# loicland/superpoint_graph

Measured on NVIDIA H100. Metric: spg_train_step_edges_plus_points_per_sec, higher is better.
Workload: dtype f32

## Files before the change

include/spg_b200.h:

```cpp
#ifndef SPG_B200_H_
#define SPG_B200_H_

#include <stdint.h>

#ifdef __cplusplus
extern "C" {
#endif

typedef void* spg_stream_t;

#define SPG_OK 0
#define SPG_E_BADARG (-1)
#define SPG_E_UNSUPPORTED (-2)
#define SPG_E_ALIGN (-3)

#define SPG_F32 0
#define SPG_F64 1

int spg_version(void);
const char* spg_error_string(int code);
int spg_set_pdl(int enabled);
int spg_zero(void* ptr, int64_t bytes, spg_stream_t stream);

int spg_prof_enable(int on);
int spg_prof_reset(void);
int spg_prof_collect(void);
int spg_prof_num_kernels(void);
const char* spg_prof_kernel_name(int kernel_id);
int spg_prof_kernel_stats(int kernel_id, int64_t* launches, double* total_ms);
int64_t spg_prof_total_launches(void);


int spg_ecc_fwd(const void* x, const void* w, const int32_t* tgt_rowptr, const int32_t* idxn,
                const int32_t* idxe, void* out, int64_t n_out, int64_t n_edges, int c_in,
                int c_out, int w_is_matrix, int dtype, spg_stream_t stream);

int spg_ecc_bwd_w(const void* xs, const void* gs, int64_t x_iter_stride, int64_t g_iter_stride,
                  int n_iter, const int32_t* tgt_rowptr, const int32_t* idxn,
                  const int32_t* idxe, const int32_t* edge_tgt, void* grad_w, int64_t n_out,
                  int64_t n_edges, int c_in, int c_out, int w_is_matrix, int accumulate,
                  int dtype, spg_stream_t stream);

int spg_ecc_bwd_x(const void* w, const void* g, const int32_t* tgt_rowptr,
                  const int32_t* src_rowptr, const int32_t* src_perm, const int32_t* edge_tgt,
                  const int32_t* idxe, const void* add0, const void* add1, void* grad_x,
                  int64_t n_in, int64_t n_edges, int c_in, int c_out, int w_is_matrix,
                  int dtype, spg_stream_t stream);


int spg_crf_softmax(const float* x, const float* g, float* out, int64_t n, int C,
                    spg_stream_t stream);

int spg_crf_fwd_step(const float* u, const float* q_prev, const float* w, const int32_t* tgt_rowptr,
                     const int32_t* idxn, float* out, int64_t n, int64_t n_edges, int C,
                     int do_softmax, spg_stream_t stream);

int spg_crf_bwd_step(const float* w, const float* gp, const float* q_prev,
                     const float* du_in, float* du_out, float* gp_out, const int32_t* tgt_rowptr,
                     const int32_t* src_rowptr, const int32_t* src_perm, const int32_t* edge_tgt,
                     int64_t n, int64_t n_edges, int C, spg_stream_t stream);


#define SPG_GRU_LAYERNORM 1
#define SPG_GRU_INGATE 2
#define SPG_GRU_BIAS 4
int spg_gru_fwd(const float* x, const float* h, const float* weight_ih, const float* weight_hh,
                const float* bias_ih, const float* bias_hh, const float* ig_weight,
                const float* ig_bias, float* hy, int64_t n_rows, int hidden, int flags,
                spg_stream_t stream);
int spg_gru_bwd(const float* x, const float* h, const float* grad_hy, const float* weight_ih,
                const float* weight_hh, const float* bias_ih, const float* bias_hh,
                const float* ig_weight, const float* ig_bias, float* d_x, float* d_h,
                float* d_gi, float* d_gh, float* d_q, float* xprime, float* dpre,
                int64_t n_rows, int hidden, int flags, spg_stream_t stream);

int spg_rnn_vv_supported(int64_t n_nodes, int hidden);
int spg_rnn_vv_fwd(float* hs, float* inps, const float* w, const int32_t* tgt_rowptr,
                   const int32_t* idxn, const float* weight_ih, const float* weight_hh,
                   const float* bias_ih, const float* bias_hh, const float* ig_weight,
                   const float* ig_bias, int64_t n_nodes, int hidden, int n_repeats, int flags,
                   void* barrier_ws, spg_stream_t stream);
int spg_rnn_vv_bwd(const float* hs, const float* inps, const float* w, const float* grad_top,
                   const float* grad_cat, const int32_t* tgt_rowptr, const int32_t* src_rowptr,
                   const int32_t* src_perm, const int32_t* edge_tgt, const float* weight_ih,
                   const float* weight_hh, const float* bias_ih, const float* bias_hh,
                   const float* ig_weight, const float* ig_bias, float* grad_inp, float* d_h_ws,
                   float* grad_h0, float* d_gi, float* d_gh, float* d_q, float* xprime,
                   float* dpre, int64_t n_nodes, int hidden, int n_repeats, int flags,
                   void* barrier_ws, spg_stream_t stream);

int spg_lstm_fwd(const float* x, const float* h, const float* c, const float* weight_ih,
                 const float* weight_hh, const float* bias_ih, const float* bias_hh,
                 const float* ig_weight, const float* ig_bias, float* hy, float* cy,
                 int64_t n_rows, int hidden, int flags, spg_stream_t stream);
int spg_lstm_bwd(const float* x, const float* h, const float* c, const float* grad_hy,
                 const float* grad_cy, const float* weight_ih, const float* weight_hh,
                 const float* bias_ih, const float* bias_hh, const float* ig_weight,
                 const float* ig_bias, float* d_x, float* d_h, float* d_c, float* d_gi,
                 float* d_gh, float* d_q, float* xprime, int64_t n_rows, int hidden, int flags,
                 spg_stream_t stream);
int spg_rnn_vv_lstm_fwd(float* hs, float* cs, float* inps, const float* w,
                        const int32_t* tgt_rowptr, const int32_t* idxn, const float* weight_ih,
                        const float* weight_hh, const float* bias_ih, const float* bias_hh,
                        const float* ig_weight, const float* ig_bias, int64_t n_nodes, int hidden,
                        int n_repeats, int flags, void* barrier_ws, spg_stream_t stream);
int spg_rnn_vv_lstm_bwd(const float* hs, const float* cs, const float* inps, const float* w,
                        const float* grad_top, const float* grad_cat, const int32_t* tgt_rowptr,
                        const int32_t* src_rowptr, const int32_t* src_perm,
                        const int32_t* edge_tgt, const float* weight_ih, const float* weight_hh,
                        const float* bias_ih, const float* bias_hh, const float* ig_weight,
                        const float* ig_bias, float* grad_inp, float* d_h_ws, float* d_c_ws,
                        float* grad_h0, float* d_gi, float* d_gh, float* d_q, float* xprime,
                        int64_t n_nodes, int hidden, int n_repeats, int flags, void* barrier_ws,
                        spg_stream_t stream);

int spg_gemm(const float* A, int64_t lda, int a_kmajor, const float* B, int64_t ldb, int b_kmajor,
             const float* bias, float* C, int64_t ldc, int64_t M, int64_t N, int64_t K,
             const float* a_scale, const float* a_shift, int a_relu, const float* b_scale,
             const float* b_shift, int b_relu, int split_k, float* workspace, float* stats_ws,
             spg_stream_t stream);
int64_t spg_gemm_stats_tiles(int64_t M);
int spg_colstats_merge(float* partials, int64_t n_partials, int C, float* mean, float* var,
                       spg_stream_t stream);
int spg_colstats_merge_fold(float* partials, int64_t n_partials, int C, float* mean, float* var,
                            const float* gamma, const float* beta, float eps, float* scale,
                            float* shift, float* running_mean, float* running_var,
                            int64_t* num_batches_tracked, float momentum, int64_t M,
                            spg_stream_t stream);

int64_t spg_tc_weight_image_floats(int N, int K);
int spg_tc_pack_weights(const float* W, int64_t ldw, int transpose, int N, int K, int k_valid,
                        float* image, spg_stream_t stream);
int spg_tc_pack_weights_scaled(const float* W, int64_t ldw, const float* row_scale, int N, int K, int k_valid,
                               float* image, spg_stream_t stream);
int spg_tc_pack_weights_multi(const int64_t* table, int n_jobs, int64_t total, spg_stream_t stream);
int spg_tc_gemm_supported(int64_t M, int N, int K);
int spg_tc_gemm(const float* A, int64_t lda, const float* weight_image, const float* bias, float* C,
                int64_t ldc, int64_t M, int N, int K, const float* a_scale, const float* a_shift,
                int a_relu, spg_stream_t stream);
int spg_tc_gemm_max_partials(void);
int spg_tc_gemm_ex(const float* A, int64_t lda, const float* weight_image, const float* bias, float* C,
                   int64_t ldc, int64_t M, int N, int K,
                   const float* a_scale, const float* a_shift, int a_relu,
                   const float* a2, int64_t lda2, const float* a_mean, const float* a_var,
                   const float* a_s12, float a_eps, float* dy_out, int64_t lddy,
                   int epilogue, float* partials_ws,
                   float* mean_out, float* var_out, const float* gamma, const float* beta, float eps,
                   float* scale_out, float* shift_out, float* running_mean, float* running_var,
                   int64_t* num_batches_tracked, float momentum,
                   const float* e_y, int64_t e_ldy, const float* e_scale, const float* e_shift,
                   const float* e_mean, const float* e_var, float e_eps, int e_relu, float* e_s12,
                   spg_stream_t stream);

int spg_tc_dw_supported(int64_t M, int co, int ci);
int spg_tc_dw_ctas(int64_t M);
int spg_tc_dw(const float* dY, int64_t lddy, const float* P, int64_t ldp, const float* p_scale,
              const float* p_shift, int p_relu, float* dW, float* workspace, int64_t M, int co, int ci,
              spg_stream_t stream);
int spg_splitk_reduce(const float* partials, int split, int64_t M, int64_t N, const float* bias,
                      float* C, int64_t ldc, spg_stream_t stream);

int64_t spg_colstats_chunks(int64_t M);
int spg_bn_fold(const float* mean, const float* var, const float* gamma, const float* beta,
                float eps, float* scale, float* shift, float* running_mean, float* running_var,
                int64_t* num_batches_tracked, float momentum, int64_t M, int C,
                spg_stream_t stream);
int spg_affine_act(const float* Y, int64_t ldy, const float* scale, const float* shift, int relu,
                   float* out, int64_t ldo, int64_t M, int C, float p, const int64_t* drop_slot,
                   spg_stream_t stream);
int spg_colsum(const float* X, int64_t ldx, int64_t M, int C, float* out, float* workspace,
               spg_stream_t stream);
int spg_act_bwd_reduce(const float* G, int64_t ldg, const float* Y, int64_t ldy,
                       const float* scale, const float* shift, const float* mean,
                       const float* var, float eps, int relu, float* s12, float* workspace,
                       int64_t M, int C, float p, const int64_t* drop_slot, spg_stream_t stream);
int spg_act_bwd_apply(const float* G, int64_t ldg, const float* Y, int64_t ldy,
                      const float* scale, const float* shift, const float* mean,
                      const float* var, float eps, int relu, int has_bn, const float* s1,
                      const float* s2, float* dY, int64_t lddy, int64_t M, int C, float p,
                      const int64_t* drop_slot, spg_stream_t stream);

int spg_dropout_rng_next(int64_t* state, int64_t* slot, int64_t key_xor, spg_stream_t stream);
int spg_dropout_mask(const int64_t* slot, float p, int64_t M, int C, uint8_t* mask, spg_stream_t stream);

int spg_cloud_rows(const float* clouds, const float* T, int add_eye, float* rows, int64_t ld,
                   int64_t B, int F, int L, spg_stream_t stream);
int spg_segmax_fwd(const float* Y, int64_t ldy, const float* scale, const float* shift, int relu,
                   float* pooled, int64_t ldp, int32_t* argmax, int64_t B, int L, const int64_t* offsets,
                   int C, spg_stream_t stream);
int spg_segmax_bwd(const float* g_pooled, int64_t ldg, const int32_t* argmax, float* G,
                   int64_t ldG, int64_t B, int L, const int64_t* offsets, const int32_t* row_seg,
                   int64_t rows, int C, spg_stream_t stream);
int spg_segmax_bn_bwd(const float* g_pooled, int64_t ldg, const int32_t* argmax, const float* Y,
                      int64_t ldy, const float* scale, const float* shift, const float* mean,
                      const float* var, float eps, int relu, float* s12, float* dY, int64_t lddy,
                      float* workspace, int64_t B, int L, const int64_t* offsets, const int32_t* row_seg,
                      int64_t rows, int C, spg_stream_t stream);
int64_t spg_group_norm_partials(int64_t B);
int spg_group_norm_fwd(const float* Y, int64_t ldy, const float* gamma, const float* beta, float eps, int relu,
                       float* out, int64_t ldo, float* mean, float* rstd, int64_t B, int L,
                       const int64_t* offsets, int C, int groups, float p, const int64_t* drop_slot,
                       spg_stream_t stream);
int spg_group_norm_bwd(const float* G, int64_t ldg, const float* Y, int64_t ldy, const float* mean,
                       const float* rstd, const float* gamma, const float* beta, int relu, float* dY,
                       int64_t lddy, float* dbg, float* workspace, int64_t B, int L, const int64_t* offsets,
                       int C, int groups, float p, const int64_t* drop_slot, spg_stream_t stream);
int spg_stn_apply_bwd(const float* clouds, const float* dXrows, int64_t ld, float* dT, int64_t B,
                      int F, int L, spg_stream_t stream);
int spg_rows_scatter(const float* src, const int64_t* idx, float* dst, int64_t n_src, int C,
                     spg_stream_t stream);
int spg_rows_gather(const float* src, const int64_t* idx, float* dst, int64_t n_dst, int C,
                    spg_stream_t stream);

int spg_ce_loss(const float* logits, const int64_t* target, const float* class_weight,
                int64_t ignore_index, float* loss_out, float* d_logits, float* workspace,
                int64_t n_rows, int C, spg_stream_t stream);
int spg_clamp_adam(float* param, const float* grad, float* exp_avg, float* exp_avg_sq,
                   int64_t n, float lr, float beta1, float beta2, float eps, float weight_decay,
                   float grad_clip, float grad_scale, int64_t step, spg_stream_t stream);

int spg_clamp_adam_dev(float* param, const float* grad, float* exp_avg, float* exp_avg_sq, int64_t n,
                       float lr, float beta1, float beta2, float eps, float weight_decay,
                       float grad_clip, float grad_scale, int64_t* step_counter,
                       spg_stream_t stream);

int spg_cloud_build(const float* points, int64_t ldp, const int64_t* sp_start,
                    const int32_t* sp_count, const int32_t* sample_idx, const int32_t* columns,
                    int n_attribs, int n_points, int normalize, const double* xform,
                    const float* jitter, float jitter_sigma, float jitter_clip, int64_t seed,
                    float* clouds, float* diameters, int64_t n_clouds, spg_stream_t stream);
int spg_graph_build_workspace(int64_t n_out, int64_t n_in, int64_t n_edges, int64_t* bytes);
int spg_graph_build(const int64_t* idxn, const int64_t* degs, int64_t n_out, int64_t n_in, int64_t n_edges,
                    int32_t* idxn32, int32_t* tgt_rowptr, int32_t* edge_tgt, int32_t* src_rowptr,
                    int32_t* src_perm, int32_t* status, void* workspace, int64_t workspace_bytes,
                    spg_stream_t stream);
int spg_confusion_count(const float* logits, int64_t ld_logits, const int64_t* label_mode,
                        const int64_t* label_vec, int64_t ld_vec, int64_t* confusion,
                        int64_t* counters, int64_t* pred_out, int64_t n_nodes, int n_classes,
                        spg_stream_t stream);
int spg_allreduce_flag_words(int world);
int64_t spg_allreduce_stage_floats(int64_t n);
int spg_allreduce_clamp_adam(const float* grad, float* const* peer_stage, uint32_t* const* peer_flags, int rank,
                             int world, float* param, float* exp_avg, float* exp_avg_sq, int64_t n, float lr,
                             float beta1, float beta2, float eps, float weight_decay, float grad_clip,
                             float grad_scale, int64_t* step_counter, uint32_t* local_state, spg_stream_t stream);
int spg_pointnet_fused_supported(int n_features, int n_points, int n_layers, const int32_t* widths);
int64_t spg_pointnet_fused_image_rows(int n_features, int n_layers, const int32_t* widths);
int spg_pointnet_fused_eval(const float* clouds, int64_t n_clouds, int n_features, int n_points, const float* T,
                            int add_eye, const float* weight_image, const float* bias, int n_layers,
                            const int32_t* widths, float* pooled, int64_t ldp, spg_stream_t stream);
int64_t spg_pointnet_fused_bf16_image_rows(int n_features, int n_layers, const int32_t* widths);
int spg_tc_pack_weights_bf16(const float* W, int64_t ldw, const float* row_scale, int N, int K, int k_valid,
                             void* image, spg_stream_t stream);
int spg_pointnet_fused_eval_bf16(const float* clouds, int64_t n_clouds, int n_features, int n_points, const float* T,
                                 int add_eye, const void* weight_image, const float* bias, int n_layers,
                                 const int32_t* widths, float* pooled, int64_t ldp, spg_stream_t stream);
int spg_rows_to_clouds(const float* rows, int64_t ld, float* clouds, int64_t B, int F, int L,
                       spg_stream_t stream);
int spg_rows_xy_transform(const float* rows_in, const float* T, int add_eye, const int32_t* row_seg,
                          float* rows_out, int64_t P, int64_t ld, spg_stream_t stream);
int spg_rows_xy_transform_bwd(const float* rows_in, int64_t ld, const float* d_rows_out, int64_t ld_d,
                              const int64_t* offsets, float* dT, int64_t B, spg_stream_t stream);
int spg_labels_to_points(const int64_t* labels_red, const int64_t* comp_ptr, const int64_t* point_ids,
                         int64_t n_components, uint8_t* labels_full, int64_t n_ver, spg_stream_t stream);
int spg_nn1_interpolate(const float* xyz_ref, int64_t n_ref, const float* xyz_query, int64_t n_query,
                        const int64_t* labels_ref, int64_t* labels_out, int32_t* nn_index_out,
                        spg_stream_t stream);

int spg_lp_sort_workspace(int64_t n, int64_t* bytes);
int spg_lp_incidence(const int64_t* src, const int64_t* tgt, int64_t n_ver, int64_t n_edges, int32_t* rowptr,
                     int32_t* entry, int32_t* keys_tmp, int32_t* keys_sorted, int32_t* vals_tmp, void* workspace,
                     int64_t workspace_bytes, spg_stream_t stream);
int spg_lp_dist_fwd(const float* emb, int64_t n_ver, int D, const int64_t* src, const int64_t* tgt, int64_t n_edges,
                    int dist_type, float* diff, float* coef, spg_stream_t stream);
int spg_lp_dist_bwd(const float* emb, int64_t n_ver, int D, const int64_t* src, const int64_t* tgt, int64_t n_edges,
                    int dist_type, const float* coef, const float* gdiff, const int32_t* rowptr, const int32_t* entry,
                    float* gemb, spg_stream_t stream);
int64_t spg_lp_loss_partials(void);
int spg_lp_loss_fwd(const float* diff, const float* weights, const uint8_t* is_transition, int64_t n_edges,
                    int intra, int inter, int dist_type, double* partials, float* loss, spg_stream_t stream);
int spg_lp_loss_bwd(const float* diff, const float* weights, const uint8_t* is_transition, int64_t n_edges,
                    int intra, int inter, int dist_type, const float* gloss, float* gdiff, spg_stream_t stream);
int spg_lp_xpart(const int64_t* src, const int64_t* tgt, const uint8_t* is_transition,
                 const int64_t* pred_in_component, int64_t n_ver, int64_t n_edges, double transition_factor,
                 float* weights, int32_t* in_component_x, int32_t* comp_size, int32_t* n_comp, int32_t* parent,
                 int32_t* is_root, int32_t* root_rank, uint64_t* keys_tmp, uint64_t* keys_sorted, int32_t* vals_tmp,
                 int32_t* vals_sorted, void* workspace, int64_t workspace_bytes, spg_stream_t stream);
int spg_lp_seal(const int64_t* src, const int64_t* tgt, const uint8_t* is_transition, const int64_t* pred_in_component,
                const int64_t* objects, int64_t n_ver, int64_t n_edges, int64_t n_comp, double transition_factor,
                float* weights, int32_t* w_per_component, int32_t* size_tmp, int32_t* maxfreq_tmp, uint64_t* keys_tmp,
                uint64_t* keys_sorted, void* workspace, int64_t workspace_bytes, spg_stream_t stream);
int spg_lp_fill_weights(const uint8_t* is_transition, int64_t n_edges, float w_other, float w_transition,
                        float* weights, spg_stream_t stream);
int spg_lp_count(const uint8_t* truth, const uint8_t* pred, int64_t n, int64_t* counts, spg_stream_t stream);
int spg_lp_edge_weight(const float* diff, int64_t n_edges, double threshold, double* edge_weight,
                       spg_stream_t stream);
int spg_lp_relax(uint8_t* relaxed, const int64_t* src, const int64_t* tgt, int64_t n_ver, int64_t n_edges,
                 int tolerance, uint8_t* vertex_mark, int32_t* hit, int32_t* status, spg_stream_t stream);
int spg_lp_perfect_prediction(const int64_t* comp_ptr, const int64_t* point_ids, int64_t n_comp,
                              const int64_t* labels, int64_t ld_labels, int n_classes, int64_t n_ver, int64_t* pred,
                              spg_stream_t stream);

int spg_lp_augment(const float* xyz, const float* rgb, int64_t n_ver, const float* rot, int64_t ref_index,
                   const float* noise_xyz, const float* noise_rgb, int device_noise, int rgb_jitter, float sigma,
                   float clip, int64_t seed, int64_t file_pos, float* xyz_out, float* rgb_out, spg_stream_t stream);
int spg_lp_subgraph_workspace(int64_t n_ver, int64_t n_edges, int64_t* bytes);
int spg_lp_subgraph_select(const uint8_t* mask, const int32_t* objects, int64_t n_ver, const int32_t* src,
                           const int32_t* tgt, int64_t n_edges, int32_t* new_index, int32_t* selected,
                           int32_t* edge_pos, uint32_t* object_max, void* workspace, int64_t workspace_bytes,
                           spg_stream_t stream);
int spg_lp_subgraph_edges(const int32_t* src, const int32_t* tgt, const uint8_t* is_transition, int64_t n_edges,
                          const int32_t* new_index, const int32_t* edge_pos, int64_t vertex_offset, int64_t* src_out,
                          int64_t* tgt_out, uint8_t* is_transition_out, spg_stream_t stream);
int spg_lp_object_offsets(const uint32_t* object_max, const int64_t* counts, int64_t n_files, int64_t* offsets,
                          spg_stream_t stream);
int spg_lp_local_clouds(const float* xyz, const float* rgb, int rgb_scale, const int32_t* local_geometry,
                        int64_t ld_geometry, int k, const int32_t* selected, int64_t n_sel, const float* elevation,
                        const float* xyn, const int32_t* labels, int64_t n_label_cols, const int32_t* objects,
                        const int64_t* object_offset, int use_rgb, int global_flags, float* clouds,
                        float* clouds_global, int64_t ld_global, float* xyz_out, int64_t* labels_out,
                        int64_t* objects_out, spg_stream_t stream);

int spg_knn_max_k(void);
int spg_knn_workspace(int64_t n, int64_t* bytes);
int spg_knn_bounds(const float* xyz, int64_t n, uint32_t* words, spg_stream_t stream);
int spg_knn_grid(const float* xyz, int64_t n, double ox, double oy, double oz, double cell, int64_t dim_x,
                 int64_t dim_y, int64_t dim_z, void* workspace, int64_t workspace_bytes, int32_t* n_cells,
                 spg_stream_t stream);
int spg_knn_query(int64_t n, int k, int k1, double ox, double oy, double oz, double cell, int64_t dim_x,
                  int64_t dim_y, int64_t dim_z, const void* workspace, int64_t workspace_bytes, int64_t* source,
                  int64_t* target, float* distances, int64_t* target2, spg_stream_t stream);
int spg_geof(const float* xyz, int64_t n, const int64_t* target, int k, float* geof, uint32_t* status,
             spg_stream_t stream);

#ifdef __cplusplus
}
#endif
#endif
```

superpoint_graph_b200/csrc/common.cuh:

```cuda
#pragma once
#include <cuda_runtime.h>
#include <stdint.h>

#include "../../include/spg_b200.h"

namespace spg {

enum KernelId {
    K_ECC_VV_FWD = 0,
    K_ECC_MAT_FWD,
    K_ECC_GEN_FWD,
    K_ECC_VV_BWD_W,
    K_ECC_MAT_BWD_W,
    K_ECC_GEN_BWD_W,
    K_ECC_VV_BWD_X,
    K_ECC_MAT_BWD_X,
    K_ECC_GEN_BWD_X,
    K_GRU_FWD,
    K_GRU_BWD,
    K_GEMM,
    K_GEMM_SPLITK_REDUCE,
    K_COLSTATS_FINAL,
    K_BN_FOLD,
    K_AFFINE_ACT,
    K_COLSUM_PARTIAL,
    K_COLSUM_FINAL,
    K_ACT_BWD_REDUCE,
    K_ACT_BWD_REDUCE_FINAL,
    K_ACT_BWD_APPLY,
    K_CLOUD_ROWS,
    K_SEGMAX_FWD,
    K_SEGMAX_BWD,
    K_STN_APPLY_BWD,
    K_ROWS_SCATTER,
    K_ROWS_GATHER,
    K_CE_LOSS,
    K_CE_LOSS_FINAL,
    K_CLAMP_ADAM,
    K_TC_GEMM,
    K_TC_PACK,
    K_TC_DW,
    K_RNN_FWD,
    K_RNN_BWD,
    K_CLOUD_BUILD,
    K_CONFUSION,
    K_TC_MERGE,
    K_POINTNET_FUSED,
    K_GRAPH_BUILD,
    K_DROPOUT_RNG_NEXT,
    K_DROPOUT_FWD,
    K_DROPOUT_MASK,
    K_DROPOUT_BWD_REDUCE,
    K_DROPOUT_BWD_REDUCE_FINAL,
    K_DROPOUT_BWD_APPLY,
    K_CRF_FWD,
    K_CRF_BWD,
    K_CRF_SOFTMAX,
    K_LSTM_FWD,
    K_LSTM_BWD,
    K_RNN_LSTM_FWD,
    K_RNN_LSTM_BWD,
    K_GN_FWD,
    K_GN_BWD,
    K_GN_BWD_FINAL,
    K_LP_INCIDENCE,
    K_LP_DIST_FWD,
    K_LP_DIST_BWD,
    K_LP_LOSS_FWD,
    K_LP_LOSS_BWD,
    K_LP_CC,
    K_LP_XPART,
    K_LP_SEAL,
    K_LP_WEIGHTS,
    K_LP_RELAX,
    K_LP_METRICS,
    K_LP_AUGMENT,
    K_LP_SUBGRAPH,
    K_LP_LOCAL_CLOUDS,
    K_GEO_BOUNDS,
    K_GEO_GRID,
    K_GEO_KNN,
    K_GEO_GEOF,
    K_COUNT
};

struct LaunchScope {
    int kid;
    cudaStream_t stream;
    int slot;
    LaunchScope(int kernel_id, cudaStream_t s);
    ~LaunchScope();
};

inline int launch_status() { return (int)cudaGetLastError(); }

constexpr int kNumSMs = 132;

__host__ __device__ inline int64_t ceil_div64(int64_t a, int64_t b) { return (a + b - 1) / b; }

__device__ __forceinline__ float warp_sum(float v) {
#pragma unroll
    for (int o = 16; o > 0; o >>= 1) v += __shfl_xor_sync(0xffffffffu, v, o);
    return v;
}

__device__ __forceinline__ float4 ld_stream4(const float4* p) { return __ldcs(p); }
__device__ __forceinline__ void st_stream4(float4* p, float4 v) { __stcs(p, v); }

__device__ __forceinline__ float sigmoidf_(float v) { return 1.f / (1.f + expf(-v)); }


__device__ __forceinline__ float relu_bwd(float g, float y, float sc, float sh) {
    return fmaf(y, sc, sh) > 0.f ? g : 0.f;
}

__device__ __forceinline__ float bn_bwd(float g, float y, float sc, float mu, float rstd, float m1, float m2) {
    return sc * (g - m1 - (y - mu) * rstd * m2);
}

struct FoldArgs {
    const float *gamma, *beta;
    float *scale, *shift, *rmean, *rvar;
    long long* nbt;
    float eps, momentum, unbias;
    int enabled;
};

inline FoldArgs fold_args(const float* gamma, const float* beta, float eps, float* scale, float* shift,
                          float* rmean, float* rvar, int64_t* nbt, float momentum, int64_t M) {
    FoldArgs f;
    f.gamma = gamma; f.beta = beta; f.scale = scale; f.shift = shift;
    f.rmean = rmean; f.rvar = rvar; f.nbt = (long long*)nbt;
    f.eps = eps; f.momentum = momentum;
    f.unbias = M > 1 ? (float)((double)M / (double)(M - 1)) : 1.f;
    f.enabled = scale != nullptr;
    return f;
}

__device__ __forceinline__ void bn_fold_col(const FoldArgs& f, int c, float mu, float var) {
    const float rstd = 1.f / sqrtf(var + f.eps);
    const float sc = (f.gamma ? f.gamma[c] : 1.f) * rstd;
    f.scale[c] = sc;
    f.shift[c] = (f.beta ? f.beta[c] : 0.f) - mu * sc;
    if (f.rmean) f.rmean[c] = (1.f - f.momentum) * f.rmean[c] + f.momentum * mu;
    if (f.rvar) f.rvar[c] = (1.f - f.momentum) * f.rvar[c] + f.momentum * var * f.unbias;
    if (c == 0 && f.nbt) f.nbt[0] += 1;
}

int colsum_merge(int kid, const float* ws, int64_t chunks, int C, float* out, cudaStream_t s);

}

#define SPG_PDL_ENTRY()                                          \
    do {                                                         \
        asm volatile("griddepcontrol.wait;" ::: "memory");       \
        asm volatile("griddepcontrol.launch_dependents;" :::);   \
    } while (0)

namespace spg {
bool pdl_enabled(int kernel_id);

template <typename... KArgs, typename... Args>
inline void launch_kernel(int kid, void (*kernel)(KArgs...), dim3 grid, dim3 block, size_t smem, cudaStream_t s,
                          Args&&... args) {
    cudaLaunchConfig_t cfg = {};
    cfg.gridDim = grid;
    cfg.blockDim = block;
    cfg.dynamicSmemBytes = smem;
    cfg.stream = s;
    cudaLaunchAttribute at[1];
    at[0].id = cudaLaunchAttributeProgrammaticStreamSerialization;
    at[0].val.programmaticStreamSerializationAllowed = 1;
    cfg.attrs = at;
    cfg.numAttrs = pdl_enabled(kid) ? 1 : 0;
    cudaLaunchKernelEx(&cfg, kernel, static_cast<KArgs>(args)...);
}
}

#define SPG_LAUNCH(kid, stream_, kernel, grid, block, smem, ...)                                  \
    do {                                                                                           \
        ::spg::LaunchScope _scope((kid), (stream_));                                               \
        ::spg::launch_kernel((kid), kernel, dim3(grid), dim3(block), (size_t)(smem), (stream_), __VA_ARGS__); \
    } while (0)
```

superpoint_graph_b200/csrc/pointnet.cu:

```cuda
#include <float.h>

#include "common.cuh"
#include "segs.cuh"

namespace spg {

constexpr int kPtChunk = 128;

__global__ void __launch_bounds__(kPtChunk)
cloud_rows_kernel(const float* __restrict__ clouds, const float* __restrict__ T, int add_eye,
                  float* __restrict__ rows, int64_t ld, int F, int L) {
    SPG_PDL_ENTRY();
    extern __shared__ float tile[];
    const int64_t b = blockIdx.x;
    const int l0 = blockIdx.y * kPtChunk;
    const int nl = min(kPtChunk, L - l0);
    const float* src = clouds + b * (int64_t)F * L;
    for (int f = 0; f < F; ++f)
        for (int l = threadIdx.x; l < nl; l += kPtChunk)
            tile[f * (kPtChunk + 1) + l] = src[(int64_t)f * L + l0 + l];
    __syncthreads();
    if (T && F >= 2) {
        const float eye = add_eye ? 1.f : 0.f;
        const float t00 = T[b * 4 + 0] + eye, t01 = T[b * 4 + 1], t10 = T[b * 4 + 2],
                    t11 = T[b * 4 + 3] + eye;
        for (int l = threadIdx.x; l < nl; l += kPtChunk) {
            const float x0 = tile[l], x1 = tile[(kPtChunk + 1) + l];
            tile[l] = fmaf(x0, t00, x1 * t10);
            tile[(kPtChunk + 1) + l] = fmaf(x0, t01, x1 * t11);
        }
        __syncthreads();
    }
    float* dst = rows + (b * L + l0) * ld;
    const int64_t total = (int64_t)nl * ld;
    for (int64_t i = threadIdx.x; i < total; i += kPtChunk) {
        const int l = (int)(i / ld), f = (int)(i % ld);
        dst[i] = f < F ? tile[f * (kPtChunk + 1) + l] : 0.f;
    }
}

template <class Segs>
__global__ void __launch_bounds__(256)
segmax_fwd_kernel(const float* __restrict__ Y, int64_t ldy, const float* __restrict__ scale,
                  const float* __restrict__ shift, int relu, float* __restrict__ pooled,
                  int64_t ldp, int* __restrict__ argmax, Segs segs, int C) {
    SPG_PDL_ENTRY();
    __shared__ float s_v[8][32];
    __shared__ int s_i[8][32];
    const int x = threadIdx.x & 31, y = threadIdx.x >> 5;
    const int c = blockIdx.x * 32 + x;
    const int64_t b = blockIdx.y;
    const int64_t r0 = segs.begin(b);
    const int L = (int)(segs.end(b) - r0);
    float best = -FLT_MAX;
    int bi = 0;
    if (c < C) {
        const float sc = scale ? scale[c] : 1.f, sh = shift ? shift[c] : 0.f;
        const float* src = Y + r0 * ldy + c;
        for (int l = y; l < L; l += 8) {
            float v = fmaf(__ldg(src + (int64_t)l * ldy), sc, sh);
            if (relu) v = fmaxf(v, 0.f);
            if (v > best || l == y) {
                best = v;
                bi = l;
            }
        }
    }
    s_v[y][x] = best;
    s_i[y][x] = (y < L) ? bi : -1;
    __syncthreads();
    if (y == 0 && c < C) {
        float bv = s_v[0][x];
        int bidx = s_i[0][x];
        for (int j = 1; j < 8; ++j) {
            const float v = s_v[j][x];
            const int i = s_i[j][x];
            if (i >= 0 && (v > bv || (v == bv && i < bidx))) {
                bv = v;
                bidx = i;
            }
        }
        pooled[b * ldp + c] = (Segs::kMayBeEmpty && bidx < 0) ? 0.f : bv;
        argmax[b * C + c] = bidx;
    }
}

template <class Segs>
__global__ void __launch_bounds__(256)
segmax_fwd_v4_kernel(const float* __restrict__ Y, int64_t ldy, const float* __restrict__ scale,
                     const float* __restrict__ shift, int relu, float* __restrict__ pooled,
                     int64_t ldp, int* __restrict__ argmax, Segs segs, int C) {
    SPG_PDL_ENTRY();
    __shared__ float4 s_v[8][32];
    __shared__ int4 s_i[8][32];
    const int x = threadIdx.x & 31, y = threadIdx.x >> 5;
    const int c = (blockIdx.x * 32 + x) * 4;
    const int64_t b = blockIdx.y;
    const int64_t r0 = segs.begin(b);
    const int L = (int)(segs.end(b) - r0);
    float best[4] = {-FLT_MAX, -FLT_MAX, -FLT_MAX, -FLT_MAX};
    int bi[4] = {-1, -1, -1, -1};
    if (c < C) {
        float sc[4] = {1.f, 1.f, 1.f, 1.f}, sh[4] = {0.f, 0.f, 0.f, 0.f};
#pragma unroll
        for (int j = 0; j < 4; ++j) {
            if (scale) sc[j] = scale[c + j];
            if (shift) sh[j] = shift[c + j];
        }
        const float* src = Y + r0 * ldy + c;
#pragma unroll 4
        for (int l = y; l < L; l += 8) {
            const float4 q = __ldg(reinterpret_cast<const float4*>(src + (int64_t)l * ldy));
            const float v[4] = {q.x, q.y, q.z, q.w};
#pragma unroll
            for (int j = 0; j < 4; ++j) {
                float t = fmaf(v[j], sc[j], sh[j]);
                if (relu) t = fmaxf(t, 0.f);
                if (bi[j] < 0 || t > best[j]) {
                    best[j] = t;
                    bi[j] = l;
                }
            }
        }
    }
    s_v[y][x] = make_float4(best[0], best[1], best[2], best[3]);
    s_i[y][x] = make_int4(bi[0], bi[1], bi[2], bi[3]);
    __syncthreads();
    if (y == 0 && c < C) {
        for (int j = 1; j < 8; ++j) {
            const float4 vq = s_v[j][x];
            const int4 iq = s_i[j][x];
            const float v[4] = {vq.x, vq.y, vq.z, vq.w};
            const int i[4] = {iq.x, iq.y, iq.z, iq.w};
#pragma unroll
            for (int k = 0; k < 4; ++k) {
                if (i[k] >= 0 && (bi[k] < 0 || v[k] > best[k] || (v[k] == best[k] && i[k] < bi[k]))) {
                    best[k] = v[k];
                    bi[k] = i[k];
                }
            }
        }
#pragma unroll
        for (int k = 0; k < 4; ++k) pooled[b * ldp + c + k] = (Segs::kMayBeEmpty && bi[k] < 0) ? 0.f : best[k];
        *reinterpret_cast<int4*>(argmax + b * C + c) = make_int4(bi[0], bi[1], bi[2], bi[3]);
    }
}

template <class Segs>
__global__ void __launch_bounds__(256)
segmax_bwd_kernel(const float* __restrict__ gp, int64_t ldg, const int* __restrict__ argmax,
                  float* __restrict__ G, int64_t ldG, int64_t rows, Segs segs, int C) {
    SPG_PDL_ENTRY();
    const int x = threadIdx.x & 31, y = threadIdx.x >> 5;
    const int c = blockIdx.x * 32 + x;
    if (c >= C) return;
    for (int64_t r = (int64_t)blockIdx.y * 8 + y; r < rows; r += (int64_t)gridDim.y * 8) {
        const int64_t b = segs.seg_of(r);
        const int l = (int)(r - segs.begin(b));
        G[r * ldG + c] = (argmax[b * C + c] == l) ? gp[b * ldg + c] : 0.f;
    }
}

__global__ void __launch_bounds__(128)
stn_apply_bwd_kernel(const float* __restrict__ clouds, const float* __restrict__ dX, int64_t ld,
                     float* __restrict__ dT, int F, int L) {
    SPG_PDL_ENTRY();
    __shared__ float red[4][4];
    const int64_t b = blockIdx.x;
    const float* xy = clouds + b * (int64_t)F * L;
    float a00 = 0.f, a01 = 0.f, a10 = 0.f, a11 = 0.f;
    for (int l = threadIdx.x; l < L; l += 128) {
        const float x0 = xy[l], x1 = xy[L + l];
        const float d0 = dX[(b * L + l) * ld], d1 = dX[(b * L + l) * ld + 1];
        a00 = fmaf(x0, d0, a00);
        a01 = fmaf(x0, d1, a01);
        a10 = fmaf(x1, d0, a10);
        a11 = fmaf(x1, d1, a11);
    }
    a00 = warp_sum(a00);
    a01 = warp_sum(a01);
    a10 = warp_sum(a10);
    a11 = warp_sum(a11);
    const int w = threadIdx.x >> 5;
    if ((threadIdx.x & 31) == 0) {
        red[w][0] = a00;
        red[w][1] = a01;
        red[w][2] = a10;
        red[w][3] = a11;
    }
    __syncthreads();
    if (threadIdx.x < 4)
        dT[b * 4 + threadIdx.x] = red[0][threadIdx.x] + red[1][threadIdx.x] + red[2][threadIdx.x] +
                                  red[3][threadIdx.x];
}

template <class Segs>
__global__ void __launch_bounds__(256)
segmax_bn_bwd_reduce_kernel(const float* __restrict__ gp, int64_t ldg, const int* __restrict__ argmax,
                            const float* __restrict__ Y, int64_t ldy, const float* __restrict__ scale,
                            const float* __restrict__ shift, const float* __restrict__ mean,
                            const float* __restrict__ var, float eps, int relu,
                            float* __restrict__ ws, int64_t B, Segs segs, int C) {
    SPG_PDL_ENTRY();
    __shared__ float s1[8][32], s2[8][32];
    const int x = threadIdx.x & 31, y = threadIdx.x >> 5;
    const int c = blockIdx.x * 32 + x;
    const int64_t b0 = (int64_t)blockIdx.y * 256, b1 = min(B, b0 + 256);
    float a1 = 0.f, a2 = 0.f;
    if (c < C) {
        const float sc = scale[c], sh = shift[c], mu = mean[c];
        const float rstd = 1.f / sqrtf(var[c] + eps);
        for (int64_t b = b0 + y; b < b1; b += 8) {
            const int l = argmax[b * C + c];
            if (Segs::kMayBeEmpty && l < 0) continue;
            const float yv = __ldg(Y + (segs.begin(b) + l) * ldy + c);
            float g = __ldg(gp + b * ldg + c);
            if (relu) g = relu_bwd(g, yv, sc, sh);
            a1 += g;
            a2 = fmaf(g, (yv - mu) * rstd, a2);
        }
    }
    s1[y][x] = a1;
    s2[y][x] = a2;
    __syncthreads();
    if (y == 0 && c < C) {
        float t1 = 0.f, t2 = 0.f;
        for (int j = 0; j < 8; ++j) {
            t1 += s1[j][x];
            t2 += s2[j][x];
        }
        ws[((int64_t)blockIdx.y * 2) * C + c] = t1;
        ws[((int64_t)blockIdx.y * 2 + 1) * C + c] = t2;
    }
}

template <class Segs>
__global__ void __launch_bounds__(256)
segmax_bn_bwd_apply_kernel(const float* __restrict__ gp, int64_t ldg, const int* __restrict__ argmax,
                           const float* __restrict__ Y, int64_t ldy, const float* __restrict__ scale,
                           const float* __restrict__ shift, const float* __restrict__ mean,
                           const float* __restrict__ var, float eps, int relu,
                           const float* __restrict__ s1, const float* __restrict__ s2,
                           float* __restrict__ dY, int64_t lddy, int64_t M, Segs segs, int C) {
    SPG_PDL_ENTRY();
    const int x = threadIdx.x & 31, y = threadIdx.x >> 5;
    const int c = (blockIdx.x * 32 + x) * 4;
    if (c >= C) return;
    float sc[4], sh[4], mu[4], rs[4], m1[4], m2[4];
#pragma unroll
    for (int j = 0; j < 4; ++j) {
        sc[j] = scale[c + j];
        sh[j] = shift[c + j];
        mu[j] = mean[c + j];
        rs[j] = 1.f / sqrtf(var[c + j] + eps);
        m1[j] = s1[c + j] / (float)M;
        m2[j] = s2[c + j] / (float)M;
    }
#pragma unroll 2
    for (int64_t r = (int64_t)blockIdx.y * 8 + y; r < M; r += (int64_t)gridDim.y * 8) {
        const int64_t b = segs.seg_of(r);
        const int l = (int)(r - segs.begin(b));
        const float4 yq = __ldg(reinterpret_cast<const float4*>(Y + r * ldy + c));
        const int4 am = __ldg(reinterpret_cast<const int4*>(argmax + b * C + c));
        const float* gr = gp + b * ldg + c;
        const float gv[4] = {__ldg(gr), __ldg(gr + 1), __ldg(gr + 2), __ldg(gr + 3)};
        const float yv[4] = {yq.x, yq.y, yq.z, yq.w};
        const int aq[4] = {am.x, am.y, am.z, am.w};
        float d[4];
#pragma unroll
        for (int j = 0; j < 4; ++j) {
            float g = (aq[j] == l) ? gv[j] : 0.f;
            if (relu) g = relu_bwd(g, yv[j], sc[j], sh[j]);
            d[j] = bn_bwd(g, yv[j], sc[j], mu[j], rs[j], m1[j], m2[j]);
        }
        *reinterpret_cast<float4*>(dY + r * lddy + c) = make_float4(d[0], d[1], d[2], d[3]);
    }
}

__global__ void rows_scatter_kernel(const float* __restrict__ src, const int64_t* __restrict__ idx,
                                    float* __restrict__ dst, int64_t n, int C) {
    SPG_PDL_ENTRY();
    const int64_t i = (int64_t)blockIdx.x * blockDim.x + threadIdx.x;
    if (i >= n * C) return;
    const int64_t r = i / C;
    dst[idx[r] * C + (i % C)] = src[i];
}

__global__ void rows_gather_kernel(const float* __restrict__ src, const int64_t* __restrict__ idx,
                                   float* __restrict__ dst, int64_t n, int C) {
    SPG_PDL_ENTRY();
    const int64_t i = (int64_t)blockIdx.x * blockDim.x + threadIdx.x;
    if (i >= n * C) return;
    const int64_t r = i / C;
    dst[i] = src[idx[r] * C + (i % C)];
}

__global__ void __launch_bounds__(kPtChunk)
rows_to_clouds_kernel(const float* __restrict__ rows, int64_t ld, float* __restrict__ clouds, int F, int L) {
    SPG_PDL_ENTRY();
    extern __shared__ float tile[];
    const int64_t b = blockIdx.x;
    const int l0 = blockIdx.y * kPtChunk;
    const int nl = min(kPtChunk, L - l0);
    const float* src = rows + (b * L + l0) * ld;
    for (int64_t i = threadIdx.x; i < (int64_t)nl * F; i += kPtChunk) {
        const int l = (int)(i / F), f = (int)(i % F);
        tile[f * (kPtChunk + 1) + l] = src[(int64_t)l * ld + f];
    }
    __syncthreads();
    float* dst = clouds + b * (int64_t)F * L;
    for (int f = 0; f < F; ++f)
        for (int l = threadIdx.x; l < nl; l += kPtChunk) dst[(int64_t)f * L + l0 + l] = tile[f * (kPtChunk + 1) + l];
}

__global__ void __launch_bounds__(256)
rows_xy_transform_kernel(const float* __restrict__ in, const float* __restrict__ T, int add_eye,
                         const int32_t* __restrict__ row_seg, float* __restrict__ out, int64_t P,
                         int64_t ld) {
    SPG_PDL_ENTRY();
    const int64_t i = (int64_t)blockIdx.x * blockDim.x + threadIdx.x;
    if (i >= P * ld) return;
    const int64_t r = i / ld;
    const int f = (int)(i % ld);
    float v = in[i];
    if (f < 2) {
        const int64_t b = row_seg[r];
        const float eye = add_eye ? 1.f : 0.f;
        const float x0 = in[r * ld], x1 = in[r * ld + 1];
        v = f == 0 ? fmaf(x0, T[b * 4 + 0] + eye, x1 * T[b * 4 + 2])
                   : fmaf(x0, T[b * 4 + 1], x1 * (T[b * 4 + 3] + eye));
    }
    out[i] = v;
}

__global__ void __launch_bounds__(256)
rows_xy_transform_bwd_kernel(const float* __restrict__ in, int64_t ld, const float* __restrict__ dOut,
                             int64_t ldd, const int64_t* __restrict__ offsets, float* __restrict__ dT,
                             int64_t B) {
    SPG_PDL_ENTRY();
    const int lane = threadIdx.x & 31;
    const int64_t b = ((int64_t)blockIdx.x * blockDim.x + threadIdx.x) >> 5;
    if (b >= B) return;
    float a00 = 0.f, a01 = 0.f, a10 = 0.f, a11 = 0.f;
    for (int64_t r = offsets[b] + lane; r < offsets[b + 1]; r += 32) {
        const float x0 = in[r * ld], x1 = in[r * ld + 1], d0 = dOut[r * ldd], d1 = dOut[r * ldd + 1];
        a00 = fmaf(x0, d0, a00);
        a01 = fmaf(x0, d1, a01);
        a10 = fmaf(x1, d0, a10);
        a11 = fmaf(x1, d1, a11);
    }
    a00 = warp_sum(a00);
    a01 = warp_sum(a01);
    a10 = warp_sum(a10);
    a11 = warp_sum(a11);
    if (lane == 0) {
        dT[b * 4 + 0] = a00;
        dT[b * 4 + 1] = a01;
        dT[b * 4 + 2] = a10;
        dT[b * 4 + 3] = a11;
    }
}

}

using namespace spg;

extern "C" {

int spg_cloud_rows(const float* clouds, const float* T, int add_eye, float* rows, int64_t ld,
                   int64_t B, int F, int L, spg_stream_t stream) {
    if (B < 0 || F <= 0 || L <= 0 || ld < F) return SPG_E_BADARG;
    if (B == 0) return SPG_OK;
    if (!clouds || !rows) return SPG_E_BADARG;
    if (F > 256 || B > 2147483647ll) return SPG_E_UNSUPPORTED;
    const size_t smem = sizeof(float) * (size_t)F * (kPtChunk + 1);
    if (smem > 200 * 1024) return SPG_E_UNSUPPORTED;
    if (smem > 48 * 1024) {
        cudaError_t e = cudaFuncSetAttribute(cloud_rows_kernel,
                                             cudaFuncAttributeMaxDynamicSharedMemorySize, (int)smem);
        if (e != cudaSuccess) return (int)e;
    }
    dim3 grid((unsigned)B, (unsigned)ceil_div64(L, kPtChunk));
    SPG_LAUNCH(K_CLOUD_ROWS, (cudaStream_t)stream, cloud_rows_kernel, grid, kPtChunk, smem, clouds,
               T, add_eye, rows, ld, F, L);
    return launch_status();
}

int spg_segmax_fwd(const float* Y, int64_t ldy, const float* scale, const float* shift, int relu,
                   float* pooled, int64_t ldp, int32_t* argmax, int64_t B, int L, const int64_t* offsets,
                   int C, spg_stream_t stream) {
    if (B < 0 || (!offsets && L <= 0) || C <= 0 || ldy < C || ldp < C) return SPG_E_BADARG;
    if (B == 0) return SPG_OK;
    if (!Y || !pooled || !argmax) return SPG_E_BADARG;
    if (B > 65535ll * 32768) return SPG_E_UNSUPPORTED;
    cudaStream_t s = (cudaStream_t)stream;
    const int64_t max_by = 65535;
    const bool vec = (C & 3) == 0 && (ldy & 3) == 0 && ((uintptr_t)Y & 15) == 0 &&
                     ((uintptr_t)argmax & 15) == 0;
    for (int64_t b0 = 0; b0 < B; b0 += max_by) {
        const int64_t nb = min(max_by, B - b0);
        const float* Yb = offsets ? Y : Y + b0 * L * ldy;
        const int rc = with_segs(L, offsets ? offsets + b0 : nullptr, nullptr, [&](auto segs) {
            if (vec) {
                dim3 grid((unsigned)ceil_div64(C, 128), (unsigned)nb);
                SPG_LAUNCH(K_SEGMAX_FWD, s, segmax_fwd_v4_kernel<decltype(segs)>, grid, 256, 0, Yb, ldy,
                           scale, shift, relu, pooled + b0 * ldp, ldp, argmax + b0 * C, segs, C);
            } else {
                dim3 grid((unsigned)ceil_div64(C, 32), (unsigned)nb);
                SPG_LAUNCH(K_SEGMAX_FWD, s, segmax_fwd_kernel<decltype(segs)>, grid, 256, 0, Yb, ldy,
                           scale, shift, relu, pooled + b0 * ldp, ldp, argmax + b0 * C, segs, C);
            }
            return launch_status();
        });
        if (rc) return rc;
    }
    return SPG_OK;
}

int spg_segmax_bwd(const float* g_pooled, int64_t ldg, const int32_t* argmax, float* G,
                   int64_t ldG, int64_t B, int L, const int64_t* offsets, const int32_t* row_seg,
                   int64_t rows, int C, spg_stream_t stream) {
    if (B < 0 || rows < 0 || C <= 0 || ldg < C || ldG < C) return SPG_E_BADARG;
    if (offsets ? !row_seg : (L <= 0 || rows != B * L)) return SPG_E_BADARG;
    if (rows == 0) return SPG_OK;
    if (!g_pooled || !argmax || !G) return SPG_E_BADARG;
    int64_t gy = ceil_div64(rows, 64);
    if (gy > 8 * kNumSMs) gy = 8 * kNumSMs;
    dim3 grid((unsigned)ceil_div64(C, 32), (unsigned)gy);
    return with_segs(L, offsets, row_seg, [&](auto segs) {
        SPG_LAUNCH(K_SEGMAX_BWD, (cudaStream_t)stream, segmax_bwd_kernel<decltype(segs)>, grid, 256, 0,
                   g_pooled, ldg, argmax, G, ldG, rows, segs, C);
        return launch_status();
    });
}

int spg_segmax_bn_bwd(const float* g_pooled, int64_t ldg, const int32_t* argmax, const float* Y,
                      int64_t ldy, const float* scale, const float* shift, const float* mean,
                      const float* var, float eps, int relu, float* s12, float* dY, int64_t lddy,
                      float* workspace, int64_t B, int L, const int64_t* offsets, const int32_t* row_seg,
                      int64_t rows, int C, spg_stream_t stream) {
    if (B <= 0 || rows <= 0 || C <= 0 || !g_pooled || !argmax || !Y || !scale || !shift || !mean || !var ||
        !s12 || !dY || !workspace)
        return SPG_E_BADARG;
    if (offsets ? !row_seg : (L <= 0 || rows != B * L)) return SPG_E_BADARG;
    if ((C & 3) || (ldy & 3) || (lddy & 3)) return SPG_E_UNSUPPORTED;
    if (((uintptr_t)argmax | (uintptr_t)Y | (uintptr_t)dY) & 15) return SPG_E_ALIGN;
    cudaStream_t s = (cudaStream_t)stream;
    const int64_t chunks = ceil_div64(B, 256);
    if (chunks > 65535) return SPG_E_UNSUPPORTED;
    return with_segs(L, offsets, row_seg, [&](auto segs) {
        dim3 g1((unsigned)ceil_div64(C, 32), (unsigned)chunks);
        SPG_LAUNCH(K_SEGMAX_BWD, s, segmax_bn_bwd_reduce_kernel<decltype(segs)>, g1, 256, 0, g_pooled, ldg,
                   argmax, Y, ldy, scale, shift, mean, var, eps, relu, workspace, B, segs, C);
        int rc = launch_status();
        if (rc) return rc;
        rc = colsum_merge(K_SEGMAX_BWD, workspace, chunks, 2 * C, s12, s);
        if (rc) return rc;
        int64_t gy = ceil_div64(rows, 32);
        if (gy > 16 * kNumSMs) gy = 16 * kNumSMs;
        dim3 g2((unsigned)ceil_div64(C, 128), (unsigned)gy);
        SPG_LAUNCH(K_SEGMAX_BWD, s, segmax_bn_bwd_apply_kernel<decltype(segs)>, g2, 256, 0, g_pooled, ldg,
                   argmax, Y, ldy, scale, shift, mean, var, eps, relu, s12, s12 + C, dY, lddy, rows, segs, C);
        return launch_status();
    });
}

int spg_stn_apply_bwd(const float* clouds, const float* dXrows, int64_t ld, float* dT, int64_t B,
                      int F, int L, spg_stream_t stream) {
    if (B < 0 || F < 2 || L <= 0 || ld < 2) return SPG_E_BADARG;
    if (B == 0) return SPG_OK;
    if (!clouds || !dXrows || !dT) return SPG_E_BADARG;
    if (B > 2147483647ll) return SPG_E_UNSUPPORTED;
    SPG_LAUNCH(K_STN_APPLY_BWD, (cudaStream_t)stream, stn_apply_bwd_kernel, (unsigned)B, 128, 0,
               clouds, dXrows, ld, dT, F, L);
    return launch_status();
}

int spg_rows_scatter(const float* src, const int64_t* idx, float* dst, int64_t n_src, int C,
                     spg_stream_t stream) {
    if (n_src < 0 || C <= 0) return SPG_E_BADARG;
    if (n_src == 0) return SPG_OK;
    if (!src || !idx || !dst) return SPG_E_BADARG;
    SPG_LAUNCH(K_ROWS_SCATTER, (cudaStream_t)stream, rows_scatter_kernel,
               (unsigned)ceil_div64(n_src * C, 256), 256, 0, src, idx, dst, n_src, C);
    return launch_status();
}

int spg_rows_gather(const float* src, const int64_t* idx, float* dst, int64_t n_dst, int C,
                    spg_stream_t stream) {
    if (n_dst < 0 || C <= 0) return SPG_E_BADARG;
    if (n_dst == 0) return SPG_OK;
    if (!src || !idx || !dst) return SPG_E_BADARG;
    SPG_LAUNCH(K_ROWS_GATHER, (cudaStream_t)stream, rows_gather_kernel,
               (unsigned)ceil_div64(n_dst * C, 256), 256, 0, src, idx, dst, n_dst, C);
    return launch_status();
}

int spg_rows_to_clouds(const float* rows, int64_t ld, float* clouds, int64_t B, int F, int L,
                       spg_stream_t stream) {
    if (B < 0 || F <= 0 || L <= 0 || ld < F) return SPG_E_BADARG;
    if (B == 0) return SPG_OK;
    if (!rows || !clouds) return SPG_E_BADARG;
    const size_t smem = sizeof(float) * (size_t)F * (kPtChunk + 1);
    if (smem > 48 * 1024 || B > 2147483647ll) return SPG_E_UNSUPPORTED;
    dim3 grid((unsigned)B, (unsigned)ceil_div64(L, kPtChunk));
    SPG_LAUNCH(K_CLOUD_ROWS, (cudaStream_t)stream, rows_to_clouds_kernel, grid, kPtChunk, smem, rows, ld, clouds, F,
               L);
    return launch_status();
}

int spg_rows_xy_transform(const float* rows_in, const float* T, int add_eye, const int32_t* row_seg,
                          float* rows_out, int64_t P, int64_t ld, spg_stream_t stream) {
    if (P < 0 || ld < 2) return SPG_E_BADARG;
    if (P == 0) return SPG_OK;
    if (!rows_in || !T || !row_seg || !rows_out) return SPG_E_BADARG;
    SPG_LAUNCH(K_CLOUD_ROWS, (cudaStream_t)stream, rows_xy_transform_kernel, (unsigned)ceil_div64(P * ld, 256),
               256, 0, rows_in, T, add_eye, row_seg, rows_out, P, ld);
    return launch_status();
}

int spg_rows_xy_transform_bwd(const float* rows_in, int64_t ld, const float* d_rows_out, int64_t ld_d,
                              const int64_t* offsets, float* dT, int64_t B, spg_stream_t stream) {
    if (B < 0 || ld < 2 || ld_d < 2) return SPG_E_BADARG;
    if (B == 0) return SPG_OK;
    if (!rows_in || !d_rows_out || !offsets || !dT) return SPG_E_BADARG;
    SPG_LAUNCH(K_STN_APPLY_BWD, (cudaStream_t)stream, rows_xy_transform_bwd_kernel,
               (unsigned)ceil_div64(B * 32, 256), 256, 0, rows_in, ld, d_rows_out, ld_d, offsets, dT, B);
    return launch_status();
}

}
```

superpoint_graph_b200/csrc/tc_dw.cu:

```cuda
#include "common.cuh"
#include "tc_common.cuh"

#include <type_traits>

namespace spg {

constexpr int DW_CONS_WARPS = 8, DW_PROD_WARPS = 4;
constexpr int DW_PROD_THREADS = DW_PROD_WARPS * 32;
constexpr int DW_THREADS = (DW_CONS_WARPS + DW_PROD_WARPS) * 32;
constexpr int DW_PTS = 32;
constexpr int DW_KSTEPS = DW_PTS / 8;
constexpr int DW_STAGES = 4;
constexpr int DW_SMEM_LIMIT = 232448;
constexpr int DW_STATIC_SMEM = 2048;

template <int CO, int CI>
struct DwCfg {
    static constexpr int WM = CO >= 128 ? CO / 2 : 64;
    static constexpr int WN = CO >= 128 ? CI : CI / 2;
    static constexpr int MSUB = WM / 64;
    static constexpr int B_BYTES = CI * DW_PTS * 4;
    static constexpr int STAGE_BYTES = 2 * B_BYTES;
    static constexpr int SMEM = DW_STAGES * STAGE_BYTES + 1024;
    static_assert(SMEM + DW_STATIC_SMEM <= DW_SMEM_LIMIT, "ring");
    static constexpr int B_F4 = CI * DW_PTS / 4 / DW_PROD_THREADS;
    static constexpr bool REG_SPLIT = WM * WN > 128 * 64;
    static constexpr int CONS_REGS = 224, PROD_REGS = 56;
    static constexpr int PF_FIT = REG_SPLIT ? 1 : 24 / B_F4;
    static constexpr int PF = PF_FIT < 1 ? 1 : (PF_FIT > 4 ? 4 : PF_FIT);
    static constexpr int HL = WN * MSUB <= 64 ? 4 : 2;
    static constexpr int RAW = MSUB == 1 ? 2 * DW_KSTEPS : 2;
    static_assert(DW_KSTEPS % HL == 0 && (DW_KSTEPS % RAW == 0 || RAW == 2 * DW_KSTEPS), "A fragment rings");
};

struct DwArgs {
    const float* dY;
    int64_t lddy;
    const float* P;
    int64_t ldp;
    const float *p_scale, *p_shift;
    int p_relu;
    float* partial;
    int64_t M;
    int64_t pts_per_cta;
};

template <int CO, int CI>
__global__ void __launch_bounds__(DW_THREADS, 1) tc_dw_kernel(const DwArgs p) {
    using Cfg = DwCfg<CO, CI>;
    constexpr int WM = Cfg::WM, WN = Cfg::WN, MSUB = Cfg::MSUB;
    constexpr int B_BYTES = Cfg::B_BYTES, STAGE_BYTES = Cfg::STAGE_BYTES;
    constexpr int PF = Cfg::PF, B_F4 = Cfg::B_F4, HL = Cfg::HL, RAW = Cfg::RAW;
    static_assert(CO % 64 == 0 && CI % 32 == 0 && CI <= 128 && CO <= 256, "shape");

    extern __shared__ __align__(1024) uint8_t smem_raw[];
    uint8_t* smem = reinterpret_cast<uint8_t*>((reinterpret_cast<uintptr_t>(smem_raw) + 1023) & ~(uintptr_t)1023);
    __shared__ __align__(8) uint64_t bars[2 * DW_STAGES];
    __shared__ __align__(16) float sc_s[128], sh_s[128];
    static_assert(sizeof(bars) + sizeof(sc_s) + sizeof(sh_s) <= DW_STATIC_SMEM, "static shared memory");

    const int t = threadIdx.x;
    const int warp = t >> 5, lane = t & 31;
    const uint32_t bars_u32 = smem_u32(&bars[0]);
    auto bar_full = [&](int s) { return bars_u32 + 8u * (uint32_t)s; };
    auto bar_empty = [&](int s) { return bars_u32 + 8u * (uint32_t)(DW_STAGES + s); };
    if (t == 0) {
#pragma unroll
        for (int s = 0; s < DW_STAGES; ++s) {
            mbar_init(bar_full(s), DW_PROD_WARPS);
            mbar_init(bar_empty(s), DW_CONS_WARPS);
        }
        asm volatile("fence.mbarrier_init.release.cluster;" ::: "memory");
    }
    SPG_PDL_ENTRY();

    const int64_t m_beg = (int64_t)blockIdx.x * p.pts_per_cta;
    const int64_t m_end = min(p.M, m_beg + p.pts_per_cta);
    const int nchunks = m_beg < m_end ? (int)((m_end - m_beg + DW_PTS - 1) / DW_PTS) : 0;

    const int ptid = t - DW_CONS_WARPS * 32;
    const int pt = (ptid >> 5) * 8 + (lane & 7), c40 = lane >> 3;
    float4 q[PF][B_F4];
    auto load_chunk = [&](int ch, float4 (&dst)[B_F4]) {
        const int64_t row = m_beg + (int64_t)ch * DW_PTS + pt;
        const bool ok = row < m_end;
        const float4* gb = reinterpret_cast<const float4*>(p.P + row * p.ldp) + c40;
#pragma unroll
        for (int j = 0; j < B_F4; ++j) dst[j] = ok ? __ldg(gb + 4 * j) : make_float4(0.f, 0.f, 0.f, 0.f);
    };
    const int g = warp >> 2, wl = warp & 3;
    const int a_co = (CO >= 128 ? g * WM : 0) + (wl * 8 + (lane >> 2)) * 2 * MSUB;
    float a_raw[RAW][MSUB][4];
    auto load_a = [&](int kstep, float (&dst)[MSUB][4]) {
        const int64_t i0 = m_beg + (int64_t)kstep * 8 + (lane & 3);
        const bool ok0 = i0 < m_end, ok1 = i0 + 4 < m_end;
        const float* y0 = p.dY + i0 * p.lddy + a_co;
        const float* y1 = y0 + 4 * p.lddy;
        if constexpr (MSUB == 1) {
            const float2 v0 = ok0 ? __ldg(reinterpret_cast<const float2*>(y0)) : make_float2(0.f, 0.f);
            const float2 v1 = ok1 ? __ldg(reinterpret_cast<const float2*>(y1)) : make_float2(0.f, 0.f);
            dst[0][0] = v0.x; dst[0][1] = v0.y; dst[0][2] = v1.x; dst[0][3] = v1.y;
        } else {
            static_assert(MSUB == 2, "A fragment loads");
            const float4 v0 = ok0 ? __ldg(reinterpret_cast<const float4*>(y0)) : make_float4(0.f, 0.f, 0.f, 0.f);
            const float4 v1 = ok1 ? __ldg(reinterpret_cast<const float4*>(y1)) : make_float4(0.f, 0.f, 0.f, 0.f);
            dst[0][0] = v0.x; dst[0][1] = v0.y; dst[1][0] = v0.z; dst[1][1] = v0.w;
            dst[0][2] = v1.x; dst[0][3] = v1.y; dst[1][2] = v1.z; dst[1][3] = v1.w;
        }
    };
    if (ptid >= 0) {
#pragma unroll
        for (int d = 0; d < PF; ++d) load_chunk(d, q[d]);
    } else {
#pragma unroll
        for (int j = 0; j < RAW; ++j) load_a(j, a_raw[j]);
    }
    if (t < CI) {
        sc_s[t] = p.p_scale ? p.p_scale[t] : 1.f;
        sh_s[t] = p.p_shift ? p.p_shift[t] : 0.f;
    }
    __syncthreads();

    if (warp >= DW_CONS_WARPS) {
        if constexpr (Cfg::REG_SPLIT) asm volatile("setmaxnreg.dec.sync.aligned.u32 %0;" ::"n"(Cfg::PROD_REGS));
        const bool pro = p.p_scale || p.p_shift || p.p_relu;
        uint32_t soff[4];
#pragma unroll
        for (int e = 0; e < 4; ++e) soff[e] = sw128_off(4 * c40 + e, pt >> 2) + (uint32_t)(pt & 3) * 4u;
        auto st_shared = [](uint32_t addr, uint32_t v) {
            asm volatile("st.shared.b32 [%0], %1;" ::"r"(addr), "r"(v) : "memory");
        };
        const uint32_t smem_u = smem_u32(smem);
        int ch = 0, s = 0;
        uint32_t use = 0;
        auto produce = [&](float4 (&cur)[B_F4]) {
            if (use > 0) mbar_wait(bar_empty(s), (use - 1) & 1);
            const uint32_t stage = smem_u + (uint32_t)s * STAGE_BYTES;
            const bool affine = pro && m_beg + (int64_t)ch * DW_PTS + pt < m_end;
#pragma unroll
            for (int j = 0; j < B_F4; ++j) {
                float4 v = cur[j];
                if (affine) {
                    const float4 sc = *reinterpret_cast<const float4*>(sc_s + (c40 + 4 * j) * 4);
                    const float4 sh = *reinterpret_cast<const float4*>(sh_s + (c40 + 4 * j) * 4);
                    v.x = fmaf(v.x, sc.x, sh.x);
                    v.y = fmaf(v.y, sc.y, sh.y);
                    v.z = fmaf(v.z, sc.z, sh.z);
                    v.w = fmaf(v.w, sc.w, sh.w);
                    if (p.p_relu) {
                        v.x = fmaxf(v.x, 0.f);
                        v.y = fmaxf(v.y, 0.f);
                        v.z = fmaxf(v.z, 0.f);
                        v.w = fmaxf(v.w, 0.f);
                    }
                }
                const float vv[4] = {v.x, v.y, v.z, v.w};
#pragma unroll
                for (int e = 0; e < 4; ++e) {
                    const uint32_t addr = stage + soff[e] + 2048u * (uint32_t)j;
                    const uint32_t hi = to_tf32(vv[e]);
                    st_shared(addr, hi);
                    st_shared(addr + B_BYTES, to_tf32(vv[e] - __uint_as_float(hi)));
                }
            }
            load_chunk(ch + PF, cur);
            asm volatile("fence.proxy.async.shared::cta;" ::: "memory");
            __syncwarp();
            if (lane == 0) mbar_arrive(bar_full(s));
            ++ch;
            if (++s == DW_STAGES) {
                s = 0;
                ++use;
            }
        };
        while (ch < nchunks) {
#pragma unroll
            for (int u = 0; u < PF; ++u) {
                produce(q[u]);
                if (ch >= nchunks) break;
            }
        }
    } else {
        if constexpr (Cfg::REG_SPLIT) asm volatile("setmaxnreg.inc.sync.aligned.u32 %0;" ::"n"(Cfg::CONS_REGS));
        float acc[MSUB][WN / 2];
#pragma unroll
        for (int m = 0; m < MSUB; ++m)
#pragma unroll
            for (int i = 0; i < WN / 2; ++i) acc[m][i] = 0.f;
        uint32_t a_hi[HL][MSUB][4], a_lo[HL][MSUB][4];
#pragma unroll
        for (int m = 0; m < MSUB; ++m) wg_reg_fence(acc[m]);
        const int col_g = CO >= 128 ? 0 : g * WN;
        const uint32_t smem_u = smem_u32(smem);

        int s = 0, s_prev = 0;
        uint32_t phase = 0;
        auto consume = [&](int ch, auto par) {
            constexpr int PAR = decltype(par)::value;
            mbar_wait(bar_full(s), phase);
            const uint32_t bh = smem_u + (uint32_t)s * STAGE_BYTES + (uint32_t)col_g * 128u, bl = bh + B_BYTES;
#pragma unroll
            for (int kb = 0; kb < DW_KSTEPS; ++kb) {
                const int h = kb % HL, r = (PAR * DW_KSTEPS + kb) % RAW;
                wg_wait<HL - 1>();
#pragma unroll
                for (int m = 0; m < MSUB; ++m) {
                    wg_reg_fence(a_hi[h][m]);
                    wg_reg_fence(a_lo[h][m]);
                }
                if (kb == HL - 1 && ch > 0) {
                    __syncwarp();
                    if (lane == 0) mbar_arrive(bar_empty(s_prev));
                }
#pragma unroll
                for (int m = 0; m < MSUB; ++m)
#pragma unroll
                    for (int e = 0; e < 4; ++e) {
                        const float v = a_raw[r][m][e];
                        const uint32_t hi = to_tf32(v);
                        a_hi[h][m][e] = hi;
                        a_lo[h][m][e] = to_tf32(v - __uint_as_float(hi));
                    }
                load_a(ch * DW_KSTEPS + kb + RAW, a_raw[r]);
                wg_fence();
                const uint64_t dbh = wg_desc_k_sw128(bh + kb * 32), dbl = wg_desc_k_sw128(bl + kb * 32);
#pragma unroll
                for (int m = 0; m < MSUB; ++m) {
                    wgmma_tf32<WN>(acc[m], a_hi[h][m], dbh, 1u);
                    wgmma_tf32<WN>(acc[m], a_lo[h][m], dbh, 1u);
                    wgmma_tf32<WN>(acc[m], a_hi[h][m], dbl, 1u);
                }
                wg_commit();
            }
            s_prev = s;
            if (++s == DW_STAGES) {
                s = 0;
                phase ^= 1u;
            }
        };
        if constexpr (RAW > DW_KSTEPS) {
            for (int ch = 0; ch < nchunks; ch += 2) {
                consume(ch, std::integral_constant<int, 0>());
                if (ch + 1 < nchunks) consume(ch + 1, std::integral_constant<int, 1>());
            }
        } else {
            for (int ch = 0; ch < nchunks; ++ch) consume(ch, std::integral_constant<int, 0>());
        }
        wg_wait<0>();
#pragma unroll
        for (int m = 0; m < MSUB; ++m) wg_reg_fence(acc[m]);
#pragma unroll
        for (int h = 0; h < HL; ++h)
#pragma unroll
            for (int m = 0; m < MSUB; ++m) {
                wg_reg_fence(a_hi[h][m]);
                wg_reg_fence(a_lo[h][m]);
            }

        float* out = p.partial + (int64_t)blockIdx.x * CO * CI;
        const int cq = 2 * (lane & 3);
#pragma unroll
        for (int m = 0; m < MSUB; ++m) {
            const int row = a_co + 2 * m;
#pragma unroll
            for (int j = 0; j < WN / 8; ++j) {
                const int col = col_g + 8 * j + cq;
                *reinterpret_cast<float2*>(out + (int64_t)row * CI + col) =
                    make_float2(acc[m][4 * j], acc[m][4 * j + 1]);
                *reinterpret_cast<float2*>(out + (int64_t)(row + 1) * CI + col) =
                    make_float2(acc[m][4 * j + 2], acc[m][4 * j + 3]);
            }
        }
    }
}

template <int CO, int CI>
static int launch_dw(const DwArgs& a, int ctas, cudaStream_t s) {
    constexpr int smem = DwCfg<CO, CI>::SMEM;
    cudaError_t e = cudaFuncSetAttribute(tc_dw_kernel<CO, CI>, cudaFuncAttributeMaxDynamicSharedMemorySize, smem);
    if (e != cudaSuccess) return (int)e;
    SPG_LAUNCH(K_TC_DW, s, (tc_dw_kernel<CO, CI>), (unsigned)ctas, DW_THREADS, smem, a);
    return launch_status();
}

}

using namespace spg;

extern "C" {

int spg_tc_dw_supported(int64_t M, int co, int ci) {
    const bool co_ok = (co == 64 || co == 128 || co == 256);
    const bool ci_ok = (ci == 32 || ci == 64 || ci == 128);
    return (M >= DW_PTS && co_ok && ci_ok) ? 1 : 0;
}

int spg_tc_dw_ctas(int64_t M) {
    int64_t chunks = ceil_div64(M, DW_PTS);
    int64_t ctas = chunks < kNumSMs ? chunks : kNumSMs;
    return (int)(ctas < 1 ? 1 : ctas);
}

int spg_tc_dw(const float* dY, int64_t lddy, const float* P, int64_t ldp, const float* p_scale,
              const float* p_shift, int p_relu, float* dW, float* workspace, int64_t M, int co, int ci,
              spg_stream_t stream) {
    if (!dY || !P || !dW || !workspace || M <= 0) return SPG_E_BADARG;
    if (!spg_tc_dw_supported(M, co, ci)) return SPG_E_UNSUPPORTED;
    if ((lddy & 3) || (ldp & 3) || lddy < co || ldp < ci) return SPG_E_ALIGN;
    if (((uintptr_t)dY | (uintptr_t)P | (uintptr_t)workspace | (uintptr_t)p_scale | (uintptr_t)p_shift) & 15)
        return SPG_E_ALIGN;
    const int ctas = spg_tc_dw_ctas(M);
    DwArgs a;
    a.dY = dY; a.lddy = lddy; a.P = P; a.ldp = ldp; a.p_scale = p_scale; a.p_shift = p_shift;
    a.p_relu = p_relu; a.partial = workspace; a.M = M;
    cudaStream_t s = (cudaStream_t)stream;
    a.pts_per_cta = ceil_div64(ceil_div64(M, ctas), DW_PTS) * DW_PTS;
    int rc;
#define SPG_DW_CASE(CO_, CI_) \
    if (co == CO_ && ci == CI_) rc = launch_dw<CO_, CI_>(a, ctas, s); else
    SPG_DW_CASE(64, 32) SPG_DW_CASE(64, 64) SPG_DW_CASE(64, 128) SPG_DW_CASE(128, 32)
    SPG_DW_CASE(128, 64) SPG_DW_CASE(128, 128) SPG_DW_CASE(256, 32) SPG_DW_CASE(256, 64)
    SPG_DW_CASE(256, 128) rc = SPG_E_UNSUPPORTED;
#undef SPG_DW_CASE
    if (rc) return rc;
    return spg_splitk_reduce(workspace, ctas, co, ci, nullptr, dW, ci, stream);
}

}
```

superpoint_graph_b200/csrc/tc_gemm2.cu:

```cuda
#include <cuda.h>
#include <stdlib.h>

#include <mutex>

#include "common.cuh"
#include "tc_common.cuh"

namespace spg {

constexpr int T2_BM = 128;
constexpr int T2_KC = 32;
constexpr int T2_MAX_STAGES = 4;
constexpr int T2_EPI_WARPS = 8, T2_PROD_WARPS = 8;
constexpr int T2_THREADS = (T2_EPI_WARPS + T2_PROD_WARPS) * 32;
constexpr int T2_A_BYTES = T2_BM * T2_KC * 4;
constexpr int T2_STAGE_BYTES = 2 * T2_A_BYTES;
constexpr int T2_HALF_A_BYTES = T2_A_BYTES / 2;
constexpr int T2_HALF_STAGE_BYTES = 2 * T2_HALF_A_BYTES;

enum { PRO_AFFINE = 0, PRO_BNBWD = 1 };
enum { EPI_NONE = 0, EPI_STATS = 1, EPI_BNRED = 2 };

struct Tc2Args {
    const float* A;
    int64_t lda;
    const float* A2;
    int64_t lda2;
    const float* bias;
    float* C;
    int64_t ldc;
    int64_t M;
    int N, K;
    const float *a_scale, *a_shift;
    int a_relu;
    const float *a_mean, *a_var, *a_s12;
    float a_eps;
    float* dy_out;
    int64_t lddy;
    int epi;
    float* part;
    float *mean_out, *var_out;
    FoldArgs fold;
    const float* e_y;
    int64_t e_ldy;
    const float *e_scale, *e_shift, *e_mean, *e_var;
    float e_eps;
    int e_relu;
    float* e_s12;
    int nstages;
};

constexpr int T2_TURN_BAR = 1;
constexpr int T2_TURN_THREADS = 2 * 128;
__device__ __forceinline__ void turn_wait(int id) {
    asm volatile("bar.sync %0, %1;" ::"r"(id), "n"(T2_TURN_THREADS) : "memory");
}
__device__ __forceinline__ void turn_pass(int id) {
    asm volatile("bar.arrive %0, %1;" ::"r"(id), "n"(T2_TURN_THREADS) : "memory");
}

__device__ __forceinline__ void st_global2(float* ptr, float2 v, bool pred) {
    asm volatile(
        "{\n\t.reg .pred p;\n\tsetp.ne.b32 p, %3, 0;\n\t@p st.global.v2.f32 [%0], {%1, %2};\n\t}" ::"l"(ptr),
        "f"(v.x), "f"(v.y), "r"((int)pred));
}
__device__ __forceinline__ void st_global4(float* ptr, float4 v, bool pred) {
    asm volatile(
        "{\n\t.reg .pred p;\n\tsetp.ne.b32 p, %5, 0;\n\t@p st.global.v4.f32 [%0], {%1, %2, %3, %4};\n\t}" ::"l"(ptr),
        "f"(v.x), "f"(v.y), "f"(v.z), "f"(v.w), "r"((int)pred));
}

__device__ __forceinline__ float reduce_scatter8(const float (&v)[8], int r) {
    const bool b0 = r & 1, b1 = r & 2, b2 = r & 4;
    float w[4], x[2];
#pragma unroll
    for (int i = 0; i < 4; ++i) {
        const float keep = b0 ? v[i + 4] : v[i], send = b0 ? v[i] : v[i + 4];
        w[i] = keep + __shfl_xor_sync(0xffffffffu, send, 4);
    }
#pragma unroll
    for (int i = 0; i < 2; ++i) {
        const float keep = b1 ? w[i + 2] : w[i], send = b1 ? w[i] : w[i + 2];
        x[i] = keep + __shfl_xor_sync(0xffffffffu, send, 8);
    }
    const float keep = b2 ? x[1] : x[0], send = b2 ? x[0] : x[1];
    return keep + __shfl_xor_sync(0xffffffffu, send, 16);
}

__device__ __forceinline__ void tma_load_2d(uint32_t dst, const CUtensorMap* map, int x, int y, uint32_t bar) {
    asm volatile(
        "cp.async.bulk.tensor.2d.shared::cluster.global.mbarrier::complete_tx::bytes [%0], [%1, {%2, %3}], [%4];"
        ::"r"(dst), "l"(map), "r"(x), "r"(y), "r"(bar)
        : "memory");
}

template <int NS, int PRO>
__global__ void __launch_bounds__(T2_THREADS, 1)
tc_gemm2_kernel(const Tc2Args p, const __grid_constant__ CUtensorMap wmap) {
    extern __shared__ __align__(1024) uint8_t smem_raw[];
    uint8_t* smem = smem_raw;
    if ((smem_u32(smem_raw) & 1023u) != 0u) __trap();
    __shared__ __align__(8) uint64_t bars[4 * T2_MAX_STAGES + 1];

    const int t = threadIdx.x;
    const int warp = t >> 5, lane = t & 31;
    const int nk = p.K / T2_KC;
    const int n0 = blockIdx.y * NS;
    const int64_t tiles = (p.M + T2_BM - 1) / T2_BM;
    const int nst = p.nstages;
    auto ring = [&](int h) { return smem_u32(smem) + (uint32_t)(h * nst) * T2_HALF_STAGE_BYTES; };
    uint8_t* wres = smem + (size_t)nst * T2_STAGE_BYTES;

    const uint32_t bars_u32 = smem_u32(&bars[0]);
    auto bar_full = [&](int h, int s) { return bars_u32 + 8u * (uint32_t)(h * T2_MAX_STAGES + s); };
    auto bar_empty = [&](int h, int s) { return bars_u32 + 8u * (uint32_t)((2 + h) * T2_MAX_STAGES + s); };
    const uint32_t bar_w = bars_u32 + 8u * (4 * T2_MAX_STAGES);

    if (t == 0) {
#pragma unroll
        for (int h = 0; h < 2; ++h)
#pragma unroll
            for (int s = 0; s < T2_MAX_STAGES; ++s) {
                mbar_init(bar_full(h, s), T2_PROD_WARPS / 2);
                mbar_init(bar_empty(h, s), T2_EPI_WARPS / 2);
            }
        mbar_init(bar_w, 1);
        asm volatile("fence.mbarrier_init.release.cluster;" ::: "memory");
        asm volatile("prefetch.tensormap [%0];" ::"l"(&wmap) : "memory");
    }
    SPG_PDL_ENTRY();
    if (t == 0) {
        mbar_expect_tx(bar_w, (uint32_t)(nk * 2 * NS * T2_KC * 4));
        const uint32_t wres_u = smem_u32(wres);
        for (int blk = 0; blk < nk * 2; ++blk)
            tma_load_2d(wres_u + (uint32_t)blk * (NS * T2_KC * 4), &wmap, 0, blk * p.N + n0, bar_w);
    }
    constexpr int PF = PRO == PRO_BNBWD ? 2 : 4;
    constexpr int NOPS = PRO == PRO_BNBWD ? 2 : 1;
    float4 q[PF][NOPS][4];
    const int pt = t - T2_EPI_WARPS * 32;
    const int ph = pt >> 7, pq = pt & 127;
    auto load = [&](int64_t tile, int kc, float4 (&dst)[NOPS][4]) {
        const int64_t m0 = tile * T2_BM;
#pragma unroll
        for (int j = 0; j < 4; ++j) {
            const int row = ph * 64 + (pq >> 3) + 16 * j, c16 = pq & 7;
            const bool ok = tile < tiles && m0 + row < p.M;
            dst[0][j] = ok ? __ldg(reinterpret_cast<const float4*>(p.A + (m0 + row) * p.lda + kc * T2_KC + c16 * 4))
                           : make_float4(0.f, 0.f, 0.f, 0.f);
            if (PRO == PRO_BNBWD)
                dst[NOPS - 1][j] =
                    ok ? __ldg(reinterpret_cast<const float4*>(p.A2 + (m0 + row) * p.lda2 + kc * T2_KC + c16 * 4))
                       : make_float4(0.f, 0.f, 0.f, 0.f);
        }
    };
    auto advance = [&](int64_t& tl, int& k) {
        if (++k == nk) {
            k = 0;
            tl += gridDim.x;
        }
    };
    int64_t ltile = blockIdx.x;
    int lkc = 0;
    if (pt >= 0) {
#pragma unroll
        for (int d = 0; d < PF - 1; ++d) {
            load(ltile, lkc, q[d]);
            advance(ltile, lkc);
        }
    }
    float* sc_s = reinterpret_cast<float*>(wres + (size_t)nk * 2 * NS * T2_KC * 4);
    float* sh_s = sc_s + p.K;
    float* cy_s = sh_s + p.K;
    float* c0_s = cy_s + p.K;
    float* bias_s = c0_s + p.K;
    float* ev_s = bias_s + NS;
    float* acc_s = ev_s + 4 * NS;
    for (int i = t; i < p.K; i += T2_THREADS) {
        const float sc = p.a_scale ? p.a_scale[i] : 1.f;
        sc_s[i] = sc;
        sh_s[i] = p.a_shift ? p.a_shift[i] : 0.f;
        if (PRO == PRO_BNBWD) {
            const float mu = p.a_mean[i], rstd = 1.f / sqrtf(p.a_var[i] + p.a_eps);
            const float m1 = p.a_s12[i] / (float)p.M, m2 = p.a_s12[p.K + i] / (float)p.M;
            cy_s[i] = -sc * rstd * m2;
            c0_s[i] = sc * (rstd * m2 * mu - m1);
        }
    }
    for (int i = t; i < NS; i += T2_THREADS) {
        bias_s[i] = p.bias ? p.bias[n0 + i] : 0.f;
        if (p.epi == EPI_BNRED) {
            ev_s[i] = p.e_scale ? p.e_scale[n0 + i] : 1.f;
            ev_s[NS + i] = p.e_shift ? p.e_shift[n0 + i] : 0.f;
            ev_s[2 * NS + i] = p.e_mean[n0 + i];
            ev_s[3 * NS + i] = 1.f / sqrtf(p.e_var[n0 + i] + p.e_eps);
        }
    }
    for (int i = t; i < T2_EPI_WARPS * NS * 4; i += T2_THREADS) acc_s[i] = 0.f;
    __syncthreads();

    if (warp >= T2_EPI_WARPS) {
        const bool pro = PRO == PRO_BNBWD || p.a_scale || p.a_shift || p.a_relu;
        int64_t tile = blockIdx.x;
        int kc = 0;
        uint32_t it = 0;
        const int c16 = pq & 7;
        uint32_t soff[4];
#pragma unroll
        for (int j = 0; j < 4; ++j) soff[j] = sw128_off((pq >> 3) + 16 * j, c16);
        const uint32_t ring_u = ring(ph);
        const bool side_store = PRO == PRO_BNBWD && p.dy_out != nullptr && blockIdx.y == 0;
        auto st_shared4 = [](uint32_t addr, uint4 v) {
            asm volatile("st.shared.v4.b32 [%0], {%1, %2, %3, %4};" ::"r"(addr), "r"(v.x), "r"(v.y),
                         "r"(v.z), "r"(v.w)
                         : "memory");
        };
        auto consume = [&](float4 (&cur)[NOPS][4], float4 (&far)[NOPS][4]) {
            const int s = it % nst;
            const uint32_t use = it / nst;
            load(ltile, lkc, far);
            advance(ltile, lkc);
            const int col = kc * T2_KC + c16 * 4;
            const float4 sc = *reinterpret_cast<const float4*>(sc_s + col);
            const float4 sh = *reinterpret_cast<const float4*>(sh_s + col);
            float4 cy = make_float4(0.f, 0.f, 0.f, 0.f), c0 = cy;
            if (PRO == PRO_BNBWD) {
                cy = *reinterpret_cast<const float4*>(cy_s + col);
                c0 = *reinterpret_cast<const float4*>(c0_s + col);
            }
            if (use > 0) mbar_wait(bar_empty(ph, s), (use - 1) & 1);
            const uint32_t stage = ring_u + (uint32_t)s * T2_HALF_STAGE_BYTES;
            const int64_t m0 = tile * T2_BM + ph * 64;
#pragma unroll
            for (int j = 0; j < 4; ++j) {
                float4 v = cur[0][j];
                const int64_t row = m0 + (pq >> 3) + 16 * j;
                if (pro && row < p.M) {
                    if (PRO == PRO_BNBWD) {
                        const float4 y = cur[NOPS - 1][j];
                        if (p.a_relu) {
                            if (!(fmaf(y.x, sc.x, sh.x) > 0.f)) v.x = 0.f;
                            if (!(fmaf(y.y, sc.y, sh.y) > 0.f)) v.y = 0.f;
                            if (!(fmaf(y.z, sc.z, sh.z) > 0.f)) v.z = 0.f;
                            if (!(fmaf(y.w, sc.w, sh.w) > 0.f)) v.w = 0.f;
                        }
                        v.x = fmaf(sc.x, v.x, fmaf(cy.x, y.x, c0.x));
                        v.y = fmaf(sc.y, v.y, fmaf(cy.y, y.y, c0.y));
                        v.z = fmaf(sc.z, v.z, fmaf(cy.z, y.z, c0.z));
                        v.w = fmaf(sc.w, v.w, fmaf(cy.w, y.w, c0.w));
                        st_global4(p.dy_out + row * p.lddy + col, v, side_store);
                    } else {
                        v.x = fmaf(v.x, sc.x, sh.x);
                        v.y = fmaf(v.y, sc.y, sh.y);
                        v.z = fmaf(v.z, sc.z, sh.z);
                        v.w = fmaf(v.w, sc.w, sh.w);
                        if (p.a_relu) {
                            v.x = fmaxf(v.x, 0.f);
                            v.y = fmaxf(v.y, 0.f);
                            v.z = fmaxf(v.z, 0.f);
                            v.w = fmaxf(v.w, 0.f);
                        }
                    }
                }
                uint4 hi, lo;
                hi.x = to_tf32(v.x);
                hi.y = to_tf32(v.y);
                hi.z = to_tf32(v.z);
                hi.w = to_tf32(v.w);
                lo.x = to_tf32(v.x - __uint_as_float(hi.x));
                lo.y = to_tf32(v.y - __uint_as_float(hi.y));
                lo.z = to_tf32(v.z - __uint_as_float(hi.z));
                lo.w = to_tf32(v.w - __uint_as_float(hi.w));
                st_shared4(stage + soff[j], hi);
                st_shared4(stage + T2_HALF_A_BYTES + soff[j], lo);
            }
            asm volatile("fence.proxy.async.shared::cta;" ::: "memory");
            __syncwarp();
            if (lane == 0) mbar_arrive(bar_full(ph, s));
            advance(tile, kc);
            ++it;
        };
        while (tile < tiles) {
#pragma unroll
            for (int u = 0; u < PF; ++u) {
                consume(q[u], q[(u + PF - 1) % PF]);
                if (tile >= tiles) break;
            }
        }
    } else {
        const int g = warp >> 2, wl = warp & 3;
        const int r = lane >> 2, cq = 2 * (lane & 3);
        float* acc_w = acc_s + warp * (NS * 4);
        const uint32_t wres_u32 = smem_u32(wres);
        const uint32_t ring_u = ring(g);
        float acc[NS / 2];
        float n_w = 0.f;
        uint32_t it = 0;
        mbar_wait(bar_w, 0);
        for (int64_t tile = blockIdx.x; tile < tiles; tile += gridDim.x) {
            if (g == 1 || tile != blockIdx.x) turn_wait(T2_TURN_BAR + g);
            for (int kc = 0; kc < nk; ++kc, ++it) {
                const int s = it % nst;
                mbar_wait(bar_full(g, s), (it / nst) & 1);
                const uint32_t a_hi = ring_u + (uint32_t)s * T2_HALF_STAGE_BYTES;
                const uint32_t a_lo = a_hi + T2_HALF_A_BYTES;
                const uint32_t b_hi = wres_u32 + (uint32_t)(kc * 2) * (NS * T2_KC * 4);
                const uint32_t b_lo = b_hi + NS * T2_KC * 4;
                wg_reg_fence(acc);
                wg_fence();
#pragma unroll
                for (int ks = 0; ks < T2_KC / 8; ++ks) {
                    const uint32_t ko = ks * 32;
                    const uint64_t dah = wg_desc_k_sw128(a_hi + ko), dal = wg_desc_k_sw128(a_lo + ko);
                    const uint64_t dbh = wg_desc_k_sw128(b_hi + ko), dbl = wg_desc_k_sw128(b_lo + ko);
                    wgmma_tf32<NS>(acc, dah, dbh, (kc | ks) ? 1u : 0u);
                    wgmma_tf32<NS>(acc, dal, dbh, 1u);
                    wgmma_tf32<NS>(acc, dah, dbl, 1u);
                }
                wg_commit();
                wg_wait<0>();
                wg_reg_fence(acc);
                __syncwarp();
                if (lane == 0) mbar_arrive(bar_empty(g, s));
            }
            if (g == 0 || tile + gridDim.x < tiles) turn_pass(T2_TURN_BAR + (g ^ 1));
            const int64_t row0 = tile * T2_BM + g * 64 + wl * 16;
            const int nv = (int)max((int64_t)0, min((int64_t)16, p.M - row0));
            const bool va = r < nv, vb = r + 8 < nv;
            float* ca = p.C + (row0 + r) * p.ldc + n0;
            float* cb = ca + 8 * p.ldc;
            const bool have_pivot = n_w > 0.f;
            if (p.epi == EPI_STATS) __syncwarp();
            const bool reduce = p.epi == EPI_BNRED || (p.epi == EPI_STATS && nv > 0);
            const int vr = 4 * (r & 1) + 2 * ((r >> 1) & 1) + (r >> 2);
            constexpr int YB = NS == 128 ? 2 : 4;
#pragma unroll
            for (int j1 = 0; j1 < NS / 8; j1 += YB) {
                float2 ya[YB], yb[YB];
                if (p.epi == EPI_BNRED) {
#pragma unroll
                    for (int u = 0; u < YB; ++u) {
                        const int64_t col = n0 + 8 * (j1 + u) + cq;
                        ya[u] = va ? __ldg(reinterpret_cast<const float2*>(p.e_y + (row0 + r) * p.e_ldy + col))
                                   : make_float2(0.f, 0.f);
                        yb[u] = vb ? __ldg(reinterpret_cast<const float2*>(p.e_y + (row0 + r + 8) * p.e_ldy + col))
                                   : make_float2(0.f, 0.f);
                    }
                }
#pragma unroll
                for (int j0 = j1; j0 < j1 + YB; j0 += 2) {
                    float v[8];
                    float piv[4];
#pragma unroll
                    for (int u = 0; u < 2; ++u) {
                        const int j = j0 + u;
                        const int c = 8 * j + cq;
                        const float2 oa = make_float2(acc[4 * j] + bias_s[c], acc[4 * j + 1] + bias_s[c + 1]);
                        const float2 ob = make_float2(acc[4 * j + 2] + bias_s[c], acc[4 * j + 3] + bias_s[c + 1]);
                        st_global2(ca + c, oa, va);
                        st_global2(cb + c, ob, vb);
#pragma unroll
                        for (int e = 0; e < 2; ++e) {
                            const int k = 2 * u + e;
                            if (p.epi == EPI_BNRED) {
                                const float esc = ev_s[c + e], esh = ev_s[NS + c + e];
                                const float emu = ev_s[2 * NS + c + e], ers = ev_s[3 * NS + c + e];
                                const float2 y0p = ya[j - j1], y1p = yb[j - j1];
                                const float y0 = e ? y0p.y : y0p.x, y1 = e ? y1p.y : y1p.x;
                                float g0 = va ? (e ? oa.y : oa.x) : 0.f, g1 = vb ? (e ? ob.y : ob.x) : 0.f;
                                if (p.e_relu) {
                                    if (!(fmaf(y0, esc, esh) > 0.f)) g0 = 0.f;
                                    if (!(fmaf(y1, esc, esh) > 0.f)) g1 = 0.f;
                                }
                                v[2 * k] = g0 + g1;
                                v[2 * k + 1] = fmaf(g1, (y1 - emu) * ers, g0 * ((y0 - emu) * ers));
                            } else if (p.epi == EPI_STATS && nv > 0) {
                                const float x0 = e ? oa.y : oa.x, x1 = e ? ob.y : ob.x;
                                const float first = __shfl_sync(0xffffffffu, x0, lane & 3);
                                piv[k] = have_pivot ? acc_w[(c + e) * 4 + 3] : first;
                                const float d0 = va ? x0 - piv[k] : 0.f;
                                const float d1 = vb ? x1 - piv[k] : 0.f;
                                v[2 * k] = d0 + d1;
                                v[2 * k + 1] = fmaf(d1, d1, d0 * d0);
                            }
                        }
                    }
                    if (reduce) {
                        const float sum = reduce_scatter8(v, r);
                        const int k = vr >> 1;
                        acc_w[(8 * (j0 + (k >> 1)) + cq + (k & 1)) * 4 + (p.epi == EPI_STATS) + (vr & 1)] += sum;
                        if (p.epi == EPI_STATS && r == 0 && !have_pivot) {
#pragma unroll
                            for (int q = 0; q < 4; ++q) acc_w[(8 * (j0 + (q >> 1)) + cq + (q & 1)) * 4 + 3] = piv[q];
                        }
                    }
                }
            }
            if (p.epi == EPI_STATS && nv > 0) n_w += (float)nv;
        }
        if (p.epi == EPI_STATS && r == 0) {
#pragma unroll
            for (int j = 0; j < NS / 8; ++j) {
                acc_w[(8 * j + cq) * 4] = n_w;
                acc_w[(8 * j + cq + 1) * 4] = n_w;
            }
        }
    }

    __syncthreads();
    if (p.epi == EPI_NONE) return;

    if (t < NS) {
        if (p.epi == EPI_STATS) {
            double n = 0.0, mean = 0.0, m2 = 0.0;
#pragma unroll
            for (int wq = 0; wq < T2_EPI_WARPS; ++wq) {
                const float* o = acc_s + wq * (NS * 4) + t * 4;
                const double nb = (double)o[0];
                if (nb > 0.0) {
                    const double mb = (double)o[3] + (double)o[1] / nb;
                    const double qb = fmax((double)o[2] - (double)o[1] * (double)o[1] / nb, 0.0);
                    const double tot = n + nb, delta = mb - mean;
                    m2 += qb + delta * delta * n * nb / tot;
                    mean += delta * nb / tot;
                    n = tot;
                }
            }
            float* o = p.part + ((int64_t)blockIdx.x * p.N + n0 + t) * 3;
            o[0] = (float)n;
            o[1] = (float)mean;
            o[2] = (float)m2;
        } else {
            float a1 = 0.f, a2 = 0.f;
#pragma unroll
            for (int wq = 0; wq < T2_EPI_WARPS; ++wq) {
                a1 += acc_s[wq * (NS * 4) + t * 4];
                a2 += acc_s[wq * (NS * 4) + t * 4 + 1];
            }
            float* o = p.part + ((int64_t)blockIdx.x * p.N + n0 + t) * 2;
            o[0] = a1;
            o[1] = a2;
        }
    }
}

__global__ void __launch_bounds__(256) tc_merge_kernel(const Tc2Args p, int P) {
    SPG_PDL_ENTRY();
    const int warp = threadIdx.x >> 5, lane = threadIdx.x & 31;
    const int c = blockIdx.x * 8 + warp;
    if (c >= p.N) return;
    {
        if (p.epi == EPI_STATS) {
            double sn = 0.0, snm = 0.0;
            float pn[5], pm[5], pq[5];
#pragma unroll
            for (int u = 0; u < 5; ++u) {
                const int k = lane + 32 * u;
                pn[u] = pm[u] = pq[u] = 0.f;
                if (k < P) {
                    const float* o = p.part + ((int64_t)k * p.N + c) * 3;
                    pn[u] = __ldcg(o);
                    pm[u] = __ldcg(o + 1);
                    pq[u] = __ldcg(o + 2);
                }
                sn += (double)pn[u];
                snm += (double)pn[u] * (double)pm[u];
            }
#pragma unroll
            for (int o = 16; o > 0; o >>= 1) {
                sn += __shfl_xor_sync(0xffffffffu, sn, o);
                snm += __shfl_xor_sync(0xffffffffu, snm, o);
            }
            const double mu = sn > 0.0 ? snm / sn : 0.0;
            double qq = 0.0;
#pragma unroll
            for (int u = 0; u < 5; ++u) {
                const double d = (double)pm[u] - mu;
                qq += (double)pq[u] + (double)pn[u] * d * d;
            }
#pragma unroll
            for (int o = 16; o > 0; o >>= 1) qq += __shfl_xor_sync(0xffffffffu, qq, o);
            if (lane == 0) {
                const float mu_f = (float)mu;
                const float var_f = sn > 0.0 ? (float)(qq / sn) : 0.f;
                p.mean_out[c] = mu_f;
                p.var_out[c] = var_f;
                if (p.fold.enabled) bn_fold_col(p.fold, c, mu_f, var_f);
            }
        } else {
            double a1 = 0.0, a2 = 0.0;
            for (int k = lane; k < P; k += 32) {
                const float* o = p.part + ((int64_t)k * p.N + c) * 2;
                a1 += (double)__ldcg(o);
                a2 += (double)__ldcg(o + 1);
            }
#pragma unroll
            for (int o = 16; o > 0; o >>= 1) {
                a1 += __shfl_xor_sync(0xffffffffu, a1, o);
                a2 += __shfl_xor_sync(0xffffffffu, a2, o);
            }
            if (lane == 0) {
                p.e_s12[c] = (float)a1;
                p.e_s12[p.N + c] = (float)a2;
            }
        }
    }
}

typedef CUresult (*EncodeTiledFn)(CUtensorMap*, CUtensorMapDataType, cuuint32_t, void*, const cuuint64_t*,
                                  const cuuint64_t*, const cuuint32_t*, const cuuint32_t*,
                                  CUtensorMapInterleave, CUtensorMapSwizzle, CUtensorMapL2promotion,
                                  CUtensorMapFloatOOBfill);

static EncodeTiledFn encode_tiled() {
    static EncodeTiledFn fn = nullptr;
    static std::once_flag once;
    std::call_once(once, [] {
        void* ptr = nullptr;
        cudaDriverEntryPointQueryResult qres;
        if (cudaGetDriverEntryPoint("cuTensorMapEncodeTiled", &ptr, cudaEnableDefault, &qres) == cudaSuccess &&
            qres == cudaDriverEntryPointSuccess)
            fn = reinterpret_cast<EncodeTiledFn>(ptr);
    });
    return fn;
}

static int make_weight_map(CUtensorMap* map, const float* image, int N, int K, int NS) {
    EncodeTiledFn fn = encode_tiled();
    if (!fn) return SPG_E_UNSUPPORTED;
    const cuuint64_t dims[2] = {(cuuint64_t)T2_KC, (cuuint64_t)(K / T2_KC) * 2 * (cuuint64_t)N};
    const cuuint64_t strides[1] = {(cuuint64_t)T2_KC * 4};
    const cuuint32_t box[2] = {(cuuint32_t)T2_KC, (cuuint32_t)NS};
    const cuuint32_t estr[2] = {1, 1};
    const CUresult r = fn(map, CU_TENSOR_MAP_DATA_TYPE_FLOAT32, 2, const_cast<float*>(image), dims, strides, box,
                          estr, CU_TENSOR_MAP_INTERLEAVE_NONE, CU_TENSOR_MAP_SWIZZLE_NONE,
                          CU_TENSOR_MAP_L2_PROMOTION_L2_128B, CU_TENSOR_MAP_FLOAT_OOB_FILL_NONE);
    return r == CUDA_SUCCESS ? SPG_OK : SPG_E_BADARG;
}

static inline int fixed_smem(int NS, int K) {
    return (K / T2_KC) * 2 * NS * T2_KC * 4 + (4 * K + NS + 4 * NS + T2_EPI_WARPS * NS * 4) * 4;
}

static inline int stages_for(int NS, int K) {
    int nst = (232448 - 1024 - fixed_smem(NS, K)) / T2_STAGE_BYTES;
    return nst > T2_MAX_STAGES ? T2_MAX_STAGES : nst;
}

template <int NS, int PRO>
static int launch_tc2(Tc2Args& a, const float* image, cudaStream_t s) {
    const int slices = a.N / NS;
    const int64_t tiles = ceil_div64(a.M, T2_BM);
    int64_t gx = kNumSMs / slices;
    if (gx > tiles) gx = tiles;
    if (gx < 1) gx = 1;
    const int nst = stages_for(NS, a.K);
    if (nst < 2) return SPG_E_UNSUPPORTED;
    a.nstages = nst;
    CUtensorMap map;
    int rc = make_weight_map(&map, image, a.N, a.K, NS);
    if (rc) return rc;
    const int smem = nst * T2_STAGE_BYTES + fixed_smem(NS, a.K);
    cudaError_t e = cudaFuncSetAttribute(tc_gemm2_kernel<NS, PRO>, cudaFuncAttributeMaxDynamicSharedMemorySize, smem);
    if (e != cudaSuccess) return (int)e;
    dim3 grid((unsigned)gx, (unsigned)slices);
    SPG_LAUNCH(K_TC_GEMM, s, (tc_gemm2_kernel<NS, PRO>), grid, T2_THREADS, smem, a, map);
    rc = launch_status();
    if (rc || a.epi == EPI_NONE) return rc;
    SPG_LAUNCH(K_TC_MERGE, s, tc_merge_kernel, (unsigned)ceil_div64(a.N, 8), 256, 0, a, (int)gx);
    return launch_status();
}

static inline int pick_ns(int N, int K) {
    if (N % 128 == 0 && stages_for(128, K) >= 2) return 128;
    if (N % 64 == 0 && stages_for(64, K) >= 2) return 64;
    if (N % 32 == 0 && N <= 64 && stages_for(32, K) >= 2) return 32;
    return 0;
}

}

using namespace spg;

extern "C" {

int spg_tc_gemm_supported(int64_t M, int N, int K) {
    return (M > 0 && N > 0 && N <= 256 && K >= T2_KC && K % T2_KC == 0 && pick_ns(N, K) != 0) ? 1 : 0;
}

int spg_tc_gemm_max_partials(void) { return kNumSMs; }

int spg_tc_gemm_ex(const float* A, int64_t lda, const float* weight_image, const float* bias, float* C,
                   int64_t ldc, int64_t M, int N, int K,
                   const float* a_scale, const float* a_shift, int a_relu,
                   const float* a2, int64_t lda2, const float* a_mean, const float* a_var,
                   const float* a_s12, float a_eps, float* dy_out, int64_t lddy,
                   int epilogue, float* partials_ws,
                   float* mean_out, float* var_out, const float* gamma, const float* beta, float eps,
                   float* scale_out, float* shift_out, float* running_mean, float* running_var,
                   int64_t* num_batches_tracked, float momentum,
                   const float* e_y, int64_t e_ldy, const float* e_scale, const float* e_shift,
                   const float* e_mean, const float* e_var, float e_eps, int e_relu, float* e_s12,
                   spg_stream_t stream) {
    if (M < 0 || !A || !weight_image || !C) return SPG_E_BADARG;
    if (M == 0) return SPG_OK;
    if (!spg_tc_gemm_supported(M, N, K)) return SPG_E_UNSUPPORTED;
    if ((lda & 3) || (ldc & 3) || lda < K || ldc < N) return SPG_E_ALIGN;
    if (((uintptr_t)A | (uintptr_t)C | (uintptr_t)weight_image | (uintptr_t)a2 | (uintptr_t)dy_out |
         (uintptr_t)e_y) & 15)
        return SPG_E_ALIGN;
    if (ceil_div64(M, T2_BM) > 2147483647ll) return SPG_E_UNSUPPORTED;
    Tc2Args a;
    a.A = A; a.lda = lda; a.A2 = a2; a.lda2 = lda2; a.bias = bias; a.C = C; a.ldc = ldc; a.M = M;
    a.N = N; a.K = K; a.a_scale = a_scale; a.a_shift = a_shift; a.a_relu = a_relu;
    a.a_mean = a_mean; a.a_var = a_var; a.a_s12 = a_s12; a.a_eps = a_eps;
    a.dy_out = dy_out; a.lddy = lddy;
    a.epi = epilogue; a.part = partials_ws;
    a.mean_out = mean_out; a.var_out = var_out;
    a.fold = fold_args(gamma, beta, eps, scale_out, shift_out, running_mean, running_var, num_batches_tracked,
                       momentum, M);
    a.e_y = e_y; a.e_ldy = e_ldy; a.e_scale = e_scale; a.e_shift = e_shift; a.e_mean = e_mean;
    a.e_var = e_var; a.e_eps = e_eps; a.e_relu = e_relu; a.e_s12 = e_s12; a.nstages = 0;
    const bool bnbwd = a2 != nullptr;
    if (bnbwd && (!a_scale || !a_shift || !a_mean || !a_var || !a_s12 || (lda2 & 3) || lda2 < K))
        return SPG_E_BADARG;
    if (dy_out && (!bnbwd || (lddy & 3) || lddy < K)) return SPG_E_BADARG;
    if (epilogue == EPI_STATS) {
        if (!partials_ws || !mean_out || !var_out) return SPG_E_BADARG;
        if (a.fold.enabled && !shift_out) return SPG_E_BADARG;
    } else if (epilogue == EPI_BNRED) {
        if (!partials_ws || !e_y || !e_mean || !e_var || !e_s12 || (e_ldy & 3) || e_ldy < N) return SPG_E_BADARG;
    } else if (epilogue != EPI_NONE) {
        return SPG_E_BADARG;
    }
    cudaStream_t s = (cudaStream_t)stream;
    const int ns = pick_ns(N, K);
#define SPG_TC2_CASE(NS_)                                                                  \
    if (ns == NS_) return bnbwd ? launch_tc2<NS_, PRO_BNBWD>(a, weight_image, s)          \
                                : launch_tc2<NS_, PRO_AFFINE>(a, weight_image, s);
    SPG_TC2_CASE(128)
    SPG_TC2_CASE(64)
    SPG_TC2_CASE(32)
#undef SPG_TC2_CASE
    return SPG_E_UNSUPPORTED;
}

int spg_tc_gemm(const float* A, int64_t lda, const float* weight_image, const float* bias, float* C,
                int64_t ldc, int64_t M, int N, int K, const float* a_scale, const float* a_shift,
                int a_relu, spg_stream_t stream) {
    return spg_tc_gemm_ex(A, lda, weight_image, bias, C, ldc, M, N, K, a_scale, a_shift, a_relu, nullptr, 0,
                          nullptr, nullptr, nullptr, 0.f, nullptr, 0, EPI_NONE, nullptr, nullptr, nullptr,
                          nullptr, nullptr, 0.f, nullptr, nullptr, nullptr, nullptr, nullptr, 0.f, nullptr, 0,
                          nullptr, nullptr, nullptr, nullptr, 0.f, 0, nullptr, stream);
}

}
```

superpoint_graph_b200/dense.py:

```python
import torch
import torch.nn as nn

from . import ops


class LayerSpec(object):

    __slots__ = ("w", "b", "gamma", "beta", "bn", "relu", "cin", "cout", "drop", "gn")

    def __init__(self, w, b, gamma, beta, bn, relu, cin, cout, drop=0.0, gn=None):
        self.w, self.b, self.gamma, self.beta = w, b, gamma, beta
        self.bn, self.relu, self.cin, self.cout = bn, relu, cin, cout
        self.drop = drop
        self.gn = gn


def parse_sequential(seq, training, params=None):
    specs = []
    params = [] if params is None else params
    mods = list(seq.children()) if isinstance(seq, nn.Sequential) else list(seq)
    i = 0
    while i < len(mods):
        m = mods[i]
        if isinstance(m, nn.Conv1d):
            if m.kernel_size != (1,) or m.stride != (1,) or m.padding != (0,) or m.groups != 1:
                raise NotImplementedError("only 1x1 Conv1d layers are on the SPG path")
            cout, cin = m.weight.shape[0], m.weight.shape[1]
        elif isinstance(m, nn.Linear):
            cout, cin = m.weight.shape
        elif isinstance(m, nn.Dropout):
            if training and m.p > 0:
                raise NotImplementedError(
                    "training-mode dropout is supported only directly after a layer's activation, in the "
                    "order Linear|Conv1d, [BatchNorm1d], [ReLU], Dropout (got %r at position %d)" % (m, i))
            i += 1
            continue
        else:
            raise NotImplementedError("unsupported module in fused chain: %r" % (m,))
        w = len(params)
        params.append(m.weight)
        b = None
        if m.bias is not None:
            b = len(params)
            params.append(m.bias)
        i += 1
        bn, gn, gamma, beta, relu = None, None, None, None, False
        if i < len(mods) and isinstance(mods[i], nn.BatchNorm1d):
            bn = mods[i]
            if bn.affine:
                gamma = len(params)
                params.append(bn.weight)
                beta = len(params)
                params.append(bn.bias)
            i += 1
        elif i < len(mods) and isinstance(mods[i], nn.GroupNorm):
            gn = mods[i]
            if not gn.affine:
                raise NotImplementedError("GroupNorm(affine=False) is not on the fused path (no PointNet of the "
                                          "reference builds one)")
            gamma = len(params)
            params.append(gn.weight)
            beta = len(params)
            params.append(gn.bias)
            i += 1
        if i < len(mods) and isinstance(mods[i], nn.ReLU):
            relu = True
            i += 1
        drop = 0.0
        if i < len(mods) and isinstance(mods[i], nn.Dropout):
            if training and mods[i].p > 0:
                drop = float(mods[i].p)
            i += 1
        specs.append(LayerSpec(w, b, gamma, beta, bn, relu, cin, cout, drop, gn))
    return specs, params


class Deferred(object):

    __slots__ = ("raw", "ld", "C", "scale", "shift", "relu", "drop")

    def __init__(self, raw, ld, C, scale=None, shift=None, relu=False):
        self.raw, self.ld, self.C = raw, ld, C
        self.scale, self.shift, self.relu = scale, shift, relu
        self.drop = None

    @property
    def pending(self):
        return self.scale is not None or self.shift is not None or self.relu

    def aff(self):
        return (self.scale, self.shift, self.relu) if self.pending else None

    def materialise(self, M):
        if not self.pending and self.ld == self.C:
            return self.raw
        return ops.affine_act(self.raw, self.ld, M, self.C, self.scale, self.shift, self.relu)


_ZEROS = {}


def _zeros(n, device):
    key = (n, device.index)
    z = _ZEROS.get(key)
    if z is None:
        z = torch.zeros(n, dtype=torch.float32, device=device)
        _ZEROS[key] = z
    return z


def _padded_k(cin, ld):
    kp = (cin + 31) // 32 * 32
    return kp if kp <= ld else cin


def _w2d(w):
    return w.view(w.shape[0], w.shape[1]) if w.dim() == 3 else w


def chain_forward(inp, M, specs, params, training, saved=None, bn_repeats=1, seg=None):
    cur = inp
    for sp in specs:
        W = _w2d(params[sp.w])
        bias = params[sp.b] if sp.b is not None else None
        bn = sp.bn
        batch_stats = bn is not None and (training or not bn.track_running_stats)
        fold = None
        if batch_stats:
            rm = rv = nbt = None
            mom = 0.0
            if training and bn.track_running_stats:
                rm, rv, nbt = bn.running_mean, bn.running_var, bn.num_batches_tracked
                if bn.momentum is None:
                    raise NotImplementedError("BatchNorm momentum=None (cumulative average)")
                mom = bn.momentum
                if bn_repeats != 1:
                    mom = 1.0 - (1.0 - mom) ** bn_repeats
            fold = (params[sp.gamma] if sp.gamma is not None else None,
                    params[sp.beta] if sp.beta is not None else None, bn.eps, rm, rv, nbt, mom)
        kpad = _padded_k(sp.cin, cur.ld)
        if ops.tc_supported(M, sp.cout, kpad, cur.ld, sp.cout) and (kpad == sp.cin or not cur.pending):
            res = ops.tc_gemm(cur.raw, cur.ld, W, sp.cin, False, M, sp.cout, kpad, bias=bias,
                              a_aff=cur.aff(), stats=batch_stats, k_valid=sp.cin, fold=fold)
        else:
            res = ops.gemm(cur.raw, cur.ld, True, W, sp.cin, True, M, sp.cout, sp.cin, bias=bias,
                           a_aff=cur.aff(), stats=batch_stats, fold=fold)
        mean = var = scale = shift = None
        y = res
        if bn is not None:
            gamma = params[sp.gamma] if sp.gamma is not None else None
            beta = params[sp.beta] if sp.beta is not None else None
            if batch_stats:
                y, mean, var, scale, shift = res
                if bn_repeats != 1 and fold[5] is not None:
                    fold[5].add_(bn_repeats - 1)
            else:
                mean, var = bn.running_mean, bn.running_var
                scale, shift = ops.bn_fold(mean, var, gamma, beta, bn.eps)
        if sp.gn is not None:
            drop = (sp.drop, ops.dropout_slot(y.device)) if (sp.drop > 0 and training) else None
            a, mean, var = ops.group_norm_fwd(y, sp.cout, ops.row_segs(M) if seg is None else seg, sp.cout,
                                              sp.gn.num_groups, params[sp.gamma], params[sp.beta], sp.gn.eps,
                                              sp.relu, drop=drop)
            nxt = Deferred(y, sp.cout, sp.cout)
            nxt.drop = drop
            act = Deferred(a, sp.cout, sp.cout)
        else:
            nxt = act = Deferred(y, sp.cout, sp.cout, scale, shift, sp.relu)
            if sp.drop > 0 and training:
                nxt.drop = (sp.drop, ops.dropout_slot(y.device))
                act = Deferred(ops.affine_act(y, sp.cout, M, sp.cout, scale, shift, sp.relu, drop=nxt.drop),
                               sp.cout, sp.cout)
        if saved is not None:
            saved.append((cur, nxt, mean, var))
        cur = act
    return cur


def _accumulate_grad(prm, g):
    if prm.requires_grad:
        prm.grad = g if prm.grad is None else prm.grad + g


def chain_backward(G, ldg, M, specs, params, saved, need_input_grad, grads, own_g=False, pooled=None, seg=None):
    red = None
    for li in range(len(specs) - 1, -1, -1):
        sp = specs[li]
        cur, nxt, mean, var = saved[li]
        C = sp.cout
        Wp = params[sp.w]
        want_dx = li > 0 or need_input_grad
        drop = nxt.drop
        fused_pool = (pooled is not None and li == len(specs) - 1 and sp.bn is not None
                      and mean is not None and C % 4 == 0 and drop is None)
        if G is None and not fused_pool:
            gp, ldgp, argmax, seg = pooled
            G, ldg, own_g = ops.segmax_bwd(gp, ldgp, argmax, seg, C), C, True
        lazy = None
        dY, ldy = None, C
        if fused_pool:
            gp, ldgp, argmax, seg = pooled
            s1, s2, dY = ops.segmax_bn_bwd(gp, ldgp, argmax, nxt.raw, nxt.ld, nxt.scale, nxt.shift,
                                           mean, var, sp.bn.eps, nxt.relu, seg, C)
            if sp.gamma is not None:
                grads[sp.gamma] = s2
                grads[sp.beta] = s1
        elif sp.gn is not None:
            dY, grads[sp.gamma], grads[sp.beta] = ops.group_norm_bwd(
                G, ldg, nxt.raw, nxt.ld, mean, var, params[sp.gamma], params[sp.beta],
                ops.row_segs(M) if seg is None else seg, C, sp.gn.num_groups, sp.relu, drop=drop)
        elif sp.bn is not None:
            eps = sp.bn.eps
            assert drop is None or red is None
            s12 = red if red is not None else ops.act_bwd_reduce(
                G, ldg, nxt.raw, nxt.ld, nxt.scale, nxt.shift, mean, var, eps, nxt.relu, M, C, drop=drop)
            s1, s2 = s12[:C], s12[C:]
            if sp.gamma is not None:
                grads[sp.gamma] = s2
                grads[sp.beta] = s1
            if (ops.USE_FUSED_BNBWD[0] and want_dx and ldg % 4 == 0 and nxt.ld % 4 == 0 and mean is not None
                    and drop is None and ops.tc_supported(M, sp.cin, sp.cout, ldg, sp.cin)):
                lazy = (nxt.raw, nxt.ld, nxt.scale, nxt.shift, nxt.relu, mean, var, s12, eps, True)
            else:
                out = G if (own_g and ldg == C) else None
                dY = ops.act_bwd_apply(G, ldg, nxt.raw, nxt.ld, nxt.scale, nxt.shift, mean, var, eps,
                                       nxt.relu, True, s1, s2, M, C, out=out, ldo=C, drop=drop)
        elif sp.relu or drop is not None:
            out = G if (own_g and ldg == C) else None
            dY = ops.act_bwd_apply(G, ldg, nxt.raw if sp.relu else None, nxt.ld, None, None, None, None, 0.0,
                                   sp.relu, False, None, None, M, C, out=out, ldo=C, drop=drop)
        else:
            dY, ldy = G, ldg
        red = None

        def weight_grads(dY, ldy, cur=cur, nxt=nxt, mean=mean, sp=sp, Wp=Wp, C=C):
            kpad = _padded_k(sp.cin, cur.ld)
            if ops.tc_dw_supported(M, sp.cout, kpad, ldy, cur.ld) and (kpad == sp.cin or not cur.pending):
                dW = ops.tc_dw(dY, ldy, cur.raw, cur.ld, M, sp.cout, kpad, p_aff=cur.aff())
                if kpad != sp.cin:
                    dW = dW[:, :sp.cin].contiguous()
            else:
                dW = ops.gemm(dY, ldy, False, cur.raw, cur.ld, False, sp.cout, sp.cin, M, b_aff=cur.aff())
            db = None
            if sp.b is not None:
                if sp.bn is not None and nxt.scale is not None and mean is not None:
                    db = _zeros(C, dY.device)
                else:
                    db = ops.colsum(dY, ldy, M, C)
            return dW.view(Wp.shape), db

        def run_weight_grads(dY, ldy):
            side = ops.SIDE[0]
            if side is None:
                grads[sp.w], db = weight_grads(dY, ldy)
                if sp.b is not None:
                    grads[sp.b] = db
            else:
                with side.fork(dY, saved[li]):
                    dW, db = weight_grads(dY, ldy)
                    _accumulate_grad(Wp, dW)
                    if sp.b is not None:
                        if db is _ZEROS.get((C, dY.device.index)):
                            db = db.clone()
                        _accumulate_grad(params[sp.b], db)

        if lazy is None:
            run_weight_grads(dY, ldy)
        Gn = None
        if want_dx:
            if lazy is not None or ops.tc_supported(M, sp.cin, sp.cout, ldy, sp.cin):
                bnred = None
                if (ops.USE_FUSED_BNBWD[0] and li > 0 and specs[li - 1].bn is not None
                        and saved[li - 1][2] is not None and saved[li - 1][1].drop is None and cur.ld % 4 == 0):
                    bnred = (cur.raw, cur.ld, cur.scale, cur.shift, saved[li - 1][2], saved[li - 1][3],
                             specs[li - 1].bn.eps, cur.relu)
                res = ops.tc_gemm(G if lazy is not None else dY, ldg if lazy is not None else ldy,
                                  _w2d(Wp), sp.cin, True, M, sp.cin, sp.cout, bnbwd=lazy, bnred=bnred)
                res = list(res) if isinstance(res, tuple) else [res]
                Gn = res.pop(0)
                if lazy is not None:
                    dY, ldy = res.pop(0), C
                if bnred is not None:
                    red = res.pop(0)
            else:
                Gn = ops.gemm(dY, ldy, True, _w2d(Wp), sp.cin, False, M, sp.cin, sp.cout)
        elif lazy is not None:
            raise AssertionError
        if lazy is not None:
            run_weight_grads(dY, ldy)
        if want_dx:
            G, ldg, own_g = Gn, sp.cin, True
        else:
            G = None
    return G


def pack_jobs(specs, params, M, ld_in, need_input_grad):
    jobs = []
    ld = ld_in
    for li, sp in enumerate(specs):
        W = _w2d(params[sp.w])
        kpad = _padded_k(sp.cin, ld)
        if ops.tc_supported(M, sp.cout, kpad, ld, sp.cout):
            jobs.append((W, sp.cin, False, sp.cout, kpad, sp.cin))
        if (li > 0 or need_input_grad) and ops.tc_supported(M, sp.cin, sp.cout, sp.cout, sp.cin):
            jobs.append((W, sp.cin, True, sp.cin, sp.cout, sp.cout))
        ld = sp.cout
    return jobs


class ChainFunction(torch.autograd.Function):

    @staticmethod
    def forward(ctx, x, specs, training, *params):
        x = x.contiguous()
        M, K = x.shape
        saved = [] if training else None
        out = chain_forward(Deferred(x, K, K), M, specs, params, training, saved)
        y = out.materialise(M)
        ctx.specs, ctx.saved, ctx.M = specs, saved, M
        ctx.nparams = len(params)
        ctx.params = params
        return y

    @staticmethod
    def backward(ctx, gy):
        if ctx.saved is None:
            raise RuntimeError("backward through an eval-mode forward is not supported "
                               "(the reference never does it: learning/main.py:229-311)")
        gy = gy.contiguous()
        grads = [None] * ctx.nparams
        gx = chain_backward(gy, gy.shape[1], ctx.M, ctx.specs, ctx.params, ctx.saved,
                            ctx.needs_input_grad[0], grads)
        ctx.saved = None
        return (gx, None, None) + tuple(grads)


def run_sequential(seq, x, training):
    specs, params = parse_sequential(seq, training)
    return ChainFunction.apply(x, specs, training, *params)
```

superpoint_graph_b200/ops.py:

```python
import os

import numpy as np
import torch

from . import _lib

F32, F64 = 0, 1
GRU_LAYERNORM, GRU_INGATE, GRU_BIAS = 1, 2, 4


def _need_cuda(*tensors):
    for t in tensors:
        if t is not None and not t.is_cuda:
            raise RuntimeError(
                "superpoint_graph_b200 ops run on sm_90a CUDA tensors only (got a CPU tensor); "
                "there is no CPU fallback")


def _dt(t):
    if t.dtype == torch.float32:
        return F32
    if t.dtype == torch.float64:
        return F64
    raise TypeError("unsupported dtype %s" % t.dtype)


def _c(t):
    return t if t.is_contiguous() else t.contiguous()


_workspaces = {}
_retired_workspaces = []


def workspace(nfloats, device, slot=0):
    key = (device.index, _lib.current_stream(), slot)
    buf = _workspaces.get(key)
    if buf is None or buf.numel() < nfloats:
        grow = 0 if buf is None else 2 * buf.numel()
        if buf is not None:
            _retired_workspaces.append(buf)
        buf = torch.empty(max(int(nfloats), grow, 1 << 16), dtype=torch.float32, device=device)
        _workspaces[key] = buf
    return buf


def zero_(t):
    _need_cuda(t)
    assert t.is_contiguous()
    _lib.call("spg_zero", t, t.numel() * t.element_size(), _lib.current_stream())
    return t


class EccGraph(object):

    def __init__(self, idxn, idxe, degs, n_in=None):
        idxn_np = idxn.detach().cpu().numpy().astype(np.int64, copy=False)
        degs_np = degs.detach().cpu().numpy().astype(np.int64, copy=False)
        self.n_out = int(degs_np.shape[0])
        self.n_edges = int(idxn_np.shape[0])
        if int(degs_np.sum()) != self.n_edges:
            raise ValueError("sum(degs)=%d does not match the number of edges %d"
                             % (int(degs_np.sum()), self.n_edges))
        if n_in is None:
            n_in = max(self.n_out, int(idxn_np.max()) + 1 if self.n_edges else 0)
        self.n_in = int(n_in)
        if self.n_edges and (idxn_np.min() < 0 or idxn_np.max() >= self.n_in):
            raise ValueError("idxn out of range")
        host = build_csr_host(idxn_np, degs_np, self.n_in)
        self.host = host
        self.idxe_host = None if idxe is None else idxe.detach().cpu().numpy().astype(np.int32)
        self._dev = {}

    GRAPH_FIELDS = ("tgt_rowptr", "idxn", "edge_tgt", "src_rowptr", "src_perm")

    @classmethod
    def from_device(cls, idxn, degs, n_in=None, check=True, idxe=None):
        _need_cuda(idxn, degs)
        g = cls.__new__(cls)
        g.n_out, g.n_edges = int(degs.numel()), int(idxn.numel())
        g.n_in = int(n_in if n_in is not None else g.n_out)
        g.host, g.idxe_host = None, None
        dev = graph_build_alloc(g.n_out, g.n_in, g.n_edges, idxn.device)
        graph_build_into(dev, idxn, degs, g.n_in)
        if idxe is not None:
            dev["idxe"] = idxe.to(device=idxn.device, dtype=torch.int32)
        if check:
            st = int(dev["status"].item())
            if st:
                raise ValueError("graph build rejected the arrays (status %d: 1 = idxn out of range, "
                                 "2 = bad degree, 4 = sum(degs) != number of edges)" % st)
        g._dev = {(idxn.device.type, idxn.device.index): dev}
        return g

    def to(self, device):
        device = torch.device(device)
        key = (device.type, device.index)
        if key not in self._dev:
            if self.host is None:
                raise RuntimeError("this graph was built on %s; it has no host copy to move" % (list(self._dev),))
            d = {k: torch.from_numpy(v).to(device) for k, v in self.host.items()}
            d["idxe"] = None if self.idxe_host is None else torch.from_numpy(self.idxe_host).to(device)
            self._dev[key] = d
        return self._dev[key]


def graph_build_alloc(n_out, n_in, n_edges, device):
    nbytes = torch.zeros(1, dtype=torch.int64)
    _lib.call("spg_graph_build_workspace", n_out, n_in, n_edges, nbytes)
    i32 = dict(dtype=torch.int32, device=device)
    return {"tgt_rowptr": torch.empty(n_out + 1, **i32), "idxn": torch.empty(n_edges, **i32),
            "edge_tgt": torch.empty(n_edges, **i32), "src_rowptr": torch.empty(n_in + 1, **i32),
            "src_perm": torch.empty(n_edges, **i32), "idxe": None, "status": torch.zeros(1, **i32),
            "_ws": torch.empty(int(nbytes[0]) + 256, dtype=torch.uint8, device=device)}


def graph_build_into(dev, idxn, degs, n_in):
    _need_cuda(idxn, degs)
    assert idxn.dtype == torch.int64 and degs.dtype == torch.int64 and idxn.is_contiguous() and degs.is_contiguous()
    ws = dev["_ws"]
    off = (-ws.data_ptr()) % 256
    _lib.call("spg_graph_build", idxn, degs, degs.numel(), int(n_in), idxn.numel(), dev["idxn"], dev["tgt_rowptr"],
              dev["edge_tgt"], dev["src_rowptr"], dev["src_perm"], dev["status"], ws.data_ptr() + off,
              ws.numel() - off, _lib.current_stream())


def build_csr_host(idxn, degs, n_in):
    n_edges = idxn.shape[0]
    tgt_rowptr = np.zeros(degs.shape[0] + 1, dtype=np.int64)
    np.cumsum(degs, out=tgt_rowptr[1:])
    edge_tgt = np.repeat(np.arange(degs.shape[0], dtype=np.int64), degs)
    src_perm = np.argsort(idxn, kind="stable")
    src_counts = np.bincount(idxn, minlength=n_in) if n_edges else np.zeros(n_in, dtype=np.int64)
    src_rowptr = np.zeros(n_in + 1, dtype=np.int64)
    np.cumsum(src_counts, out=src_rowptr[1:])
    if n_edges >= 2 ** 31 or n_in >= 2 ** 31:
        raise ValueError("graph too large for int32 indices")
    return {
        "tgt_rowptr": tgt_rowptr.astype(np.int32),
        "idxn": idxn.astype(np.int32),
        "edge_tgt": edge_tgt.astype(np.int32),
        "src_rowptr": src_rowptr.astype(np.int32),
        "src_perm": src_perm.astype(np.int32),
    }


def ecc_fwd(x, w, graph, c_out, out=None):
    _need_cuda(x, w)
    x, w = _c(x), _c(w)
    g = graph.to(x.device)
    is_mat = int(w.dim() == 3)
    c_in = x.shape[1]
    if x.shape[0] != graph.n_in:
        raise ValueError("input has %d rows, graph has %d nodes" % (x.shape[0], graph.n_in))
    n_w = g["idxe"].max().item() + 1 if g["idxe"] is not None else graph.n_edges
    if w.shape[0] < n_w:
        raise ValueError("weights has %d rows, graph needs %d" % (w.shape[0], n_w))
    if out is None:
        out = torch.empty((graph.n_out, c_out), dtype=x.dtype, device=x.device)
    _lib.call("spg_ecc_fwd", x, w, g["tgt_rowptr"], g["idxn"], g["idxe"], out, graph.n_out,
              graph.n_edges, c_in, c_out, is_mat, _dt(x), _lib.current_stream())
    return out


def ecc_bwd_w(xs, gs, graph, w_shape, n_iter=1, out=None, accumulate=False):
    _need_cuda(xs, gs)
    xs, gs = _c(xs), _c(gs)
    g = graph.to(xs.device)
    is_mat = int(len(w_shape) == 3)
    c_in, c_out = xs.shape[-1], gs.shape[-1]
    if out is None:
        if g["idxe"] is not None:
            out = torch.zeros(w_shape, dtype=xs.dtype, device=xs.device)
        else:
            out = torch.empty(w_shape, dtype=xs.dtype, device=xs.device)
    x_stride = xs.shape[-2] * c_in if xs.dim() == 3 else 0
    g_stride = gs.shape[-2] * c_out if gs.dim() == 3 else 0
    _lib.call("spg_ecc_bwd_w", xs, gs, x_stride, g_stride, n_iter, g["tgt_rowptr"], g["idxn"],
              g["idxe"], g["edge_tgt"], out, graph.n_out, graph.n_edges, c_in, c_out, is_mat,
              int(accumulate), _dt(xs), _lib.current_stream())
    return out


def ecc_bwd_x(w, g_out, graph, c_in, add0=None, add1=None):
    _need_cuda(w, g_out, add0, add1)
    w, g_out = _c(w), _c(g_out)
    add0 = None if add0 is None else _c(add0)
    add1 = None if add1 is None else _c(add1)
    g = graph.to(w.device)
    is_mat = int(w.dim() == 3)
    c_out = g_out.shape[1]
    gx = torch.empty((graph.n_in, c_in), dtype=w.dtype, device=w.device)
    _lib.call("spg_ecc_bwd_x", w, g_out, g["tgt_rowptr"], g["src_rowptr"], g["src_perm"],
              g["edge_tgt"], g["idxe"], add0, add1, gx, graph.n_in, graph.n_edges, c_in, c_out,
              is_mat, _dt(w), _lib.current_stream())
    return gx


CRF_MAX_C = 32


def _crf_graph(graph, n, device):
    if graph.idxe_host is not None or graph.n_in != n or graph.n_out != n:
        raise ValueError("the CRF kernels need a square graph of %d nodes without idxe" % n)
    return graph.to(device)


def crf_softmax(x, g=None, out=None):
    _need_cuda(x, g)
    x = _c(x)
    n, C = x.shape
    if out is None:
        out = torch.empty_like(x)
    _lib.call("spg_crf_softmax", x, None if g is None else _c(g), out, n, C, _lib.current_stream())
    return out


def crf_fwd_step(u, q_prev, w, graph, out, softmax):
    _need_cuda(u, q_prev, w, out)
    n, C = u.shape
    g = _crf_graph(graph, n, u.device)
    _lib.call("spg_crf_fwd_step", u, q_prev, w, g["tgt_rowptr"], g["idxn"], out, n, graph.n_edges, C,
              int(softmax), _lib.current_stream())
    return out


def crf_bwd_step(w, gp, q_prev, du_in, du_out, gp_out, graph):
    _need_cuda(w, gp, q_prev, du_in, du_out, gp_out)
    n, C = q_prev.shape
    g = _crf_graph(graph, n, w.device)
    _lib.call("spg_crf_bwd_step", w, gp, q_prev, du_in, du_out, gp_out, g["tgt_rowptr"], g["src_rowptr"],
              g["src_perm"], g["edge_tgt"], n, graph.n_edges, C, _lib.current_stream())
    return du_out


def gru_fwd(x, h, w_ih, w_hh, b_ih, b_hh, w_ig, b_ig, flags, out=None):
    _need_cuda(x, h, w_ih, w_hh)
    x, h = _c(x), _c(h)
    n, H = h.shape
    assert x.shape == h.shape and w_ih.shape == (3 * H, H) and w_hh.shape == (3 * H, H)
    if out is None:
        out = torch.empty_like(h)
    _lib.call("spg_gru_fwd", x, h, _c(w_ih), _c(w_hh), b_ih, b_hh,
              None if w_ig is None else _c(w_ig), b_ig, out, n, H, flags, _lib.current_stream())
    return out


def gru_bwd(x, h, gy, w_ih, w_hh, b_ih, b_hh, w_ig, b_ig, flags, d_gi, d_gh, d_q, xprime, dpre,
            d_x=None, d_h=None):
    _need_cuda(x, h, gy)
    x, h, gy = _c(x), _c(h), _c(gy)
    n, H = h.shape
    if d_x is None:
        d_x = torch.empty_like(h)
    if d_h is None:
        d_h = torch.empty_like(h)
    _lib.call("spg_gru_bwd", x, h, gy, _c(w_ih), _c(w_hh), b_ih, b_hh,
              None if w_ig is None else _c(w_ig), b_ig, d_x, d_h, d_gi, d_gh, d_q, xprime, dpre,
              n, H, flags, _lib.current_stream())
    return d_x, d_h


def lstm_fwd(x, h, c, w_ih, w_hh, b_ih, b_hh, w_ig, b_ig, flags, out=None, out_c=None):
    _need_cuda(x, h, c, w_ih, w_hh)
    x, h, c = _c(x), _c(h), _c(c)
    n, H = h.shape
    assert x.shape == h.shape == c.shape and w_ih.shape == (4 * H, H) and w_hh.shape == (4 * H, H)
    if out is None:
        out = torch.empty_like(h)
    if out_c is None:
        out_c = torch.empty_like(h)
    _lib.call("spg_lstm_fwd", x, h, c, _c(w_ih), _c(w_hh), b_ih, b_hh,
              None if w_ig is None else _c(w_ig), b_ig, out, out_c, n, H, flags, _lib.current_stream())
    return out, out_c


def lstm_bwd(x, h, c, gy, gc, w_ih, w_hh, b_ih, b_hh, w_ig, b_ig, flags, d_gi, d_gh, d_q, xprime,
             d_x=None, d_h=None, d_c=None):
    _need_cuda(x, h, c, gy, gc)
    x, h, c, gy = _c(x), _c(h), _c(c), _c(gy)
    n, H = h.shape
    d_x = torch.empty_like(h) if d_x is None else d_x
    d_h = torch.empty_like(h) if d_h is None else d_h
    d_c = torch.empty_like(h) if d_c is None else d_c
    _lib.call("spg_lstm_bwd", x, h, c, gy, None if gc is None else _c(gc), _c(w_ih), _c(w_hh), b_ih, b_hh,
              None if w_ig is None else _c(w_ig), b_ig, d_x, d_h, d_c, d_gi, d_gh, d_q, xprime,
              n, H, flags, _lib.current_stream())
    return d_x, d_h, d_c


def rnn_vv_supported(weights, graph, n, H):
    return (USE_FUSED_RNN[0] and weights.dim() == 2 and weights.dtype == torch.float32
            and graph.idxe_host is None and graph.n_in == n and graph.n_out == n
            and bool(_lib.lib().spg_rnn_vv_supported(n, H)))


def rnn_vv_fwd(hs, inps, weights, graph, cell, flags, cs=None):
    _need_cuda(hs, inps, weights, cs)
    R, n, H = inps.shape
    g = graph.to(hs.device)
    w_ih, w_hh, b_ih, b_hh, w_ig, b_ig = cell
    bar = torch.empty(4, dtype=torch.int32, device=hs.device)
    w = (_c(weights), g["tgt_rowptr"], g["idxn"], _c(w_ih), _c(w_hh), b_ih, b_hh,
         None if w_ig is None else _c(w_ig), b_ig, n, H, R, flags, bar, _lib.current_stream())
    if cs is None:
        _lib.call("spg_rnn_vv_fwd", hs, inps, *w)
    else:
        _lib.call("spg_rnn_vv_lstm_fwd", hs, cs, inps, *w)


def rnn_vv_bwd(hs, inps, weights, graph, cell, flags, gtop, gcat, ginp, d_gi, d_gh, d_q, xp, dpre, cs=None):
    _need_cuda(hs, inps, weights, gtop, cs)
    R, n, H = inps.shape
    g = graph.to(hs.device)
    w_ih, w_hh, b_ih, b_hh, w_ig, b_ig = cell
    bar = torch.empty(4, dtype=torch.int32, device=hs.device)
    dh = torch.empty((n, H), dtype=torch.float32, device=hs.device)
    gh0 = torch.empty((n, H), dtype=torch.float32, device=hs.device)
    head = (_c(weights), gtop, gcat, g["tgt_rowptr"], g["src_rowptr"], g["src_perm"], g["edge_tgt"],
            _c(w_ih), _c(w_hh), b_ih, b_hh, None if w_ig is None else _c(w_ig), b_ig, ginp, dh)
    tail = (n, H, R, flags, bar, _lib.current_stream())
    if cs is None:
        _lib.call("spg_rnn_vv_bwd", hs, inps, *head, gh0, d_gi, d_gh, d_q, xp, dpre, *tail)
    else:
        dc = torch.empty((n, H), dtype=torch.float32, device=hs.device)
        _lib.call("spg_rnn_vv_lstm_bwd", hs, cs, inps, *head, dc, gh0, d_gi, d_gh, d_q, xp, *tail)
    return gh0


GEMM_TRACE = None
GEMM_FLOPS = [0]


def _auto_split(M, N, K):
    tiles = ((M + 127) // 128) * ((N + 63) // 64)
    if tiles >= 132 or K < 256:
        return 1
    split = min((2 * 132 + tiles - 1) // tiles, max(1, K // 64))
    return max(1, split)


def _merge_stats(sws, tiles, N, M, dev, fold):
    mean = torch.empty(N, dtype=torch.float32, device=dev)
    var = torch.empty(N, dtype=torch.float32, device=dev)
    if fold is None:
        _lib.call("spg_colstats_merge", sws, tiles, N, mean, var, _lib.current_stream())
        return mean, var
    gamma, beta, eps, rm, rv, nbt, mom = fold
    scale = torch.empty(N, dtype=torch.float32, device=dev)
    shift = torch.empty(N, dtype=torch.float32, device=dev)
    _lib.call("spg_colstats_merge_fold", sws, tiles, N, mean, var, gamma, beta, float(eps), scale, shift,
              rm, rv, nbt, float(mom), int(M), _lib.current_stream())
    return mean, var, scale, shift


def gemm(A, lda, a_kmajor, B, ldb, b_kmajor, M, N, K, bias=None, out=None, ldc=None,
         a_aff=None, b_aff=None, split_k=None, stats=False, fold=None):
    _need_cuda(A, B)
    dev = A.device
    if out is None:
        out = torch.empty((M, N), dtype=torch.float32, device=dev)
        ldc = N
    elif ldc is None:
        ldc = out.stride(0)
    a_s, a_t, a_r = a_aff if a_aff is not None else (None, None, False)
    b_s, b_t, b_r = b_aff if b_aff is not None else (None, None, False)
    GEMM_FLOPS[0] += 2 * M * N * K
    if GEMM_TRACE is not None:
        ev0 = torch.cuda.Event(enable_timing=True)
        ev0.record()
    if split_k is None:
        split_k = 1 if stats else _auto_split(M, N, K)
    ws = workspace(split_k * M * N, dev) if split_k > 1 else None
    tiles = (M + 127) // 128
    sws = workspace((tiles + tiles // 256 + 2) * N * 3, dev, slot=1) if stats else None
    _lib.call("spg_gemm", A, lda, int(a_kmajor), B, ldb, int(b_kmajor), bias, out, ldc, M, N, K,
              a_s, a_t, int(bool(a_r)), b_s, b_t, int(bool(b_r)), split_k, ws, sws,
              _lib.current_stream())
    if GEMM_TRACE is not None:
        ev1 = torch.cuda.Event(enable_timing=True)
        ev1.record()
        GEMM_TRACE.append(("M=%d N=%d K=%d a%d b%d split=%d" % (M, N, K, int(a_kmajor), int(b_kmajor), split_k),
                           ev0, ev1))
    if stats:
        return (out,) + _merge_stats(sws, tiles, N, M, dev, fold)
    return out


USE_TC = [os.environ.get("SPG_TC", "1") != "0"]
USE_FUSED_RNN = [os.environ.get("SPG_FUSED_RNN", "1") != "0"]
USE_FUSED_BNBWD = [os.environ.get("SPG_FUSED_BNBWD", "1") != "0"]
USE_FUSED_EVAL = [os.environ.get("SPG_FUSED_EVAL", "1") != "0"]
def set_pdl(mode):
    if "SPG_PDL" not in os.environ:
        _lib.call("spg_set_pdl", int(mode))


USE_SIDE_STREAM = [os.environ.get("SPG_SIDE_STREAM", "1") != "0"]


def tc_supported(M, N, K, lda=0, ldc=0):
    return (USE_TC[0] and M >= 512 and lda % 4 == 0 and ldc % 4 == 0
            and bool(_lib.lib().spg_tc_gemm_supported(int(M), int(N), int(K))))


PACK_CACHE = {}
_PACK_TABLES = {}
PACK_LEARN = [None]


def prepack(jobs):
    if not jobs:
        return
    keys = tuple((W.data_ptr(), int(ldw), int(bool(tr)), int(N), int(K), int(kv)) for W, ldw, tr, N, K, kv in jobs)
    ent = _PACK_TABLES.get(keys)
    dev = jobs[0][0].device
    if ent is None:
        rows, imgs, total = [], [], 0
        for (ptr, ldw, tr, N, K, kv) in keys:
            img = torch.empty(2 * N * K, dtype=torch.float32, device=dev)
            imgs.append(img)
            rows.append([ptr, ldw, tr, N, K, kv, img.data_ptr(), total])
            total += N * K
        table = torch.tensor(rows, dtype=torch.int64).to(dev)
        ent = _PACK_TABLES[keys] = (table, imgs, total)
    table, imgs, total = ent
    _lib.call("spg_tc_pack_weights_multi", table, len(keys), total, _lib.current_stream())
    for k, img in zip(keys, imgs):
        PACK_CACHE[k] = img


def _weight_image(W, ldw, transpose, N, K, kv, dev):
    key = (W.data_ptr(), int(ldw), int(bool(transpose)), int(N), int(K), int(kv))
    img = PACK_CACHE.get(key)
    if img is None:
        img = torch.empty(2 * N * K, dtype=torch.float32, device=dev)
        _lib.call("spg_tc_pack_weights", W, ldw, int(bool(transpose)), N, K, kv, img, _lib.current_stream())
        if PACK_LEARN[0] is not None:
            PACK_LEARN[0][key] = (W, int(ldw), bool(transpose), int(N), int(K), kv)
    return img


def tc_gemm(A, lda, W, ldw, transpose, M, N, K, bias=None, a_aff=None, stats=False, k_valid=None,
            fold=None, bnbwd=None, bnred=None):
    _need_cuda(A, W)
    dev = A.device
    kv = int(K if k_valid is None else k_valid)
    img = _weight_image(W, ldw, transpose, N, K, kv, dev)
    out = torch.empty((M, N), dtype=torch.float32, device=dev)
    a_s, a_t, a_r = a_aff if a_aff is not None else (None, None, False)
    a2 = a_mean = a_var = a_s12 = dy = None
    lda2 = lddy = 0
    a_eps = 0.0
    if bnbwd is not None:
        a2, lda2, a_s, a_t, a_r, a_mean, a_var, a_s12, a_eps, want_dy = bnbwd
        if want_dy:
            dy = torch.empty((M, K), dtype=torch.float32, device=dev)
            lddy = K
    epi, ws = 0, None
    mean = var = scale = shift = gamma = beta = rm = rv = nbt = None
    eps = mom = 0.0
    e = (None, 0, None, None, None, None, 0.0, False)
    s12 = None
    if stats:
        epi = 1
        mean = torch.empty(N, dtype=torch.float32, device=dev)
        var = torch.empty(N, dtype=torch.float32, device=dev)
        if fold is not None:
            gamma, beta, eps, rm, rv, nbt, mom = fold
            scale = torch.empty(N, dtype=torch.float32, device=dev)
            shift = torch.empty(N, dtype=torch.float32, device=dev)
    elif bnred is not None:
        epi = 2
        e = bnred
        s12 = torch.empty(2 * N, dtype=torch.float32, device=dev)
    if epi:
        ws = workspace(MAX_TC_PARTIALS[0] * N * 3, dev, slot=1)
    GEMM_FLOPS[0] += 2 * M * N * K
    TC_FLOPS[0] += 2 * M * N * K
    _lib.call("spg_tc_gemm_ex", A, lda, img, bias, out, N, M, N, K, a_s, a_t, int(bool(a_r)),
              a2, lda2, a_mean, a_var, a_s12, float(a_eps), dy, lddy, epi, ws,
              mean, var, gamma, beta, float(eps), scale, shift, rm, rv, nbt, float(mom),
              e[0], e[1], e[2], e[3], e[4], e[5], float(e[6]), int(bool(e[7])), s12,
              _lib.current_stream())
    res = [out]
    if stats:
        res += [mean, var] + ([scale, shift] if fold is not None else [])
    if dy is not None:
        res.append(dy)
    if s12 is not None:
        res.append(s12)
    return res[0] if len(res) == 1 else tuple(res)


MAX_TC_PARTIALS = [132]

TC_FLOPS = [0]
DW_FLOPS = [0]


def tc_dw_supported(M, co, ci, lddy, ldp):
    return (USE_TC[0] and M >= 2048 and lddy % 4 == 0 and ldp % 4 == 0
            and bool(_lib.lib().spg_tc_dw_supported(int(M), int(co), int(ci))))


def tc_dw(dY, lddy, P, ldp, M, co, ci, p_aff=None):
    _need_cuda(dY, P)
    dev = dY.device
    ctas = int(_lib.lib().spg_tc_dw_ctas(int(M)))
    ws = workspace(ctas * co * ci, dev)
    out = torch.empty((co, ci), dtype=torch.float32, device=dev)
    p_s, p_t, p_r = p_aff if p_aff is not None else (None, None, False)
    GEMM_FLOPS[0] += 2 * M * co * ci
    DW_FLOPS[0] += 2 * M * co * ci
    _lib.call("spg_tc_dw", dY, lddy, P, ldp, p_s, p_t, int(bool(p_r)), out, ws, M, co, ci,
              _lib.current_stream())
    return out


def _chunks(M):
    return max(1, (M + 255) // 256)


def bn_fold(mean, var, gamma, beta, eps, running_mean=None, running_var=None, momentum=0.1, M=0,
            num_batches_tracked=None):
    _need_cuda(mean, var)
    C = mean.numel()
    scale = torch.empty(C, dtype=torch.float32, device=mean.device)
    shift = torch.empty(C, dtype=torch.float32, device=mean.device)
    _lib.call("spg_bn_fold", mean, var, gamma, beta, float(eps), scale, shift, running_mean,
              running_var, num_batches_tracked, float(momentum), int(M), C, _lib.current_stream())
    return scale, shift


def _drop(drop):
    if drop is None:
        return 0.0, None
    _need_cuda(drop[1])
    return float(drop[0]), drop[1]


def affine_act(Y, ldy, M, C, scale=None, shift=None, relu=False, out=None, ldo=None, drop=None):
    _need_cuda(Y)
    if out is None:
        out = torch.empty((M, C), dtype=torch.float32, device=Y.device)
        ldo = C
    _lib.call("spg_affine_act", Y, ldy, scale, shift, int(bool(relu)), out, ldo, M, C, *_drop(drop),
              _lib.current_stream())
    return out


def colsum(X, ldx, M, C):
    _need_cuda(X)
    out = torch.empty(C, dtype=torch.float32, device=X.device)
    ws = workspace(C * _chunks(M), X.device)
    _lib.call("spg_colsum", X, ldx, M, C, out, ws, _lib.current_stream())
    return out


def act_bwd_reduce(G, ldg, Y, ldy, scale, shift, mean, var, eps, relu, M, C, drop=None):
    _need_cuda(G, Y)
    s12 = torch.empty(2 * C, dtype=torch.float32, device=G.device)
    ws = workspace(2 * C * _chunks(M), G.device)
    _lib.call("spg_act_bwd_reduce", G, ldg, Y, ldy, scale, shift, mean, var, float(eps),
              int(bool(relu)), s12, ws, M, C, *_drop(drop), _lib.current_stream())
    return s12


def act_bwd_apply(G, ldg, Y, ldy, scale, shift, mean, var, eps, relu, has_bn, s1, s2, M, C,
                  out=None, ldo=None, drop=None):
    _need_cuda(G)
    if out is None:
        out = torch.empty((M, C), dtype=torch.float32, device=G.device)
        ldo = C
    _lib.call("spg_act_bwd_apply", G, ldg, Y, ldy, scale, shift, mean, var, float(eps),
              int(bool(relu)), int(bool(has_bn)), s1, s2, out, ldo, M, C, *_drop(drop),
              _lib.current_stream())
    return out


_DROPOUT_RNG = {}
DROPOUT_KEY_XOR = {}


def _device(device):
    if device is None:
        return torch.device("cuda", torch.cuda.current_device())
    device = torch.device(device)
    return torch.device("cuda", device.index if device.index is not None else torch.cuda.current_device())


def dropout_rng_state(device=None, create=True):
    dev = _device(device)
    st = _DROPOUT_RNG.get(dev.index)
    if st is None and create:
        seed = int(torch.randint(-2 ** 63, 2 ** 63 - 1, (1,), dtype=torch.int64))
        st = torch.tensor([seed, 0], dtype=torch.int64).to(dev)
        _DROPOUT_RNG[dev.index] = st
    return st


def _int64(v):
    v = int(v) & (2 ** 64 - 1)
    return v - 2 ** 64 if v >= 2 ** 63 else v


def dropout_manual_seed(seed, device=None):
    dev = _device(device)
    st = _DROPOUT_RNG.get(dev.index)
    if st is None:
        _DROPOUT_RNG[dev.index] = torch.tensor([_int64(seed), 0], dtype=torch.int64).to(dev)
    else:
        st[0].fill_(_int64(seed))
        st[1].zero_()


def dropout_slot(device):
    dev = _device(device)
    st = dropout_rng_state(dev)
    slot = torch.empty(2, dtype=torch.int64, device=dev)
    _lib.call("spg_dropout_rng_next", st, slot, _int64(DROPOUT_KEY_XOR.get(dev.index, 0)), _lib.current_stream())
    return slot


def dropout_fwd(Y, ldy, M, C, scale, shift, relu, p, slot):
    return affine_act(Y, ldy, M, C, scale, shift, relu, drop=(p, slot))


def dropout_mask(slot, p, M, C):
    _need_cuda(slot)
    mask = torch.empty((M, C), dtype=torch.uint8, device=slot.device)
    _lib.call("spg_dropout_mask", _c(slot), float(p), M, C, mask, _lib.current_stream())
    return mask


def cloud_rows(clouds, T, ld, add_eye=False):
    _need_cuda(clouds, T)
    clouds = _c(clouds)
    B, F, L = clouds.shape
    rows = torch.empty((B * L, ld), dtype=torch.float32, device=clouds.device)
    _lib.call("spg_cloud_rows", clouds, None if T is None else _c(T), int(bool(add_eye)), rows, ld,
              B, F, L, _lib.current_stream())
    return rows


def rows_to_clouds(rows, ld, B, F, L):
    _need_cuda(rows)
    out = torch.empty((B, F, L), dtype=torch.float32, device=rows.device)
    _lib.call("spg_rows_to_clouds", rows, ld, out, B, F, L, _lib.current_stream())
    return out


def _seg_rows(seg):
    B, L, offsets, row_seg = seg
    if offsets is None:
        return B * L
    assert offsets.dtype == torch.int64 and offsets.is_contiguous() and row_seg.dtype == torch.int32
    return row_seg.numel()


def segmax_fwd(Y, ldy, seg, C, scale, shift, relu, pooled, ldp):
    B, L, offsets, _ = seg
    _need_cuda(Y, pooled, offsets)
    assert offsets is None or (offsets.dtype == torch.int64 and offsets.is_contiguous())
    argmax = torch.empty((B, C), dtype=torch.int32, device=Y.device)
    _lib.call("spg_segmax_fwd", Y, ldy, scale, shift, int(bool(relu)), pooled, ldp, argmax, B, L, offsets, C,
              _lib.current_stream())
    return argmax


def segmax_bwd(g_pooled, ldg, argmax, seg, C):
    _need_cuda(g_pooled, argmax)
    B, L, offsets, row_seg = seg
    M = _seg_rows(seg)
    G = torch.empty((M, C), dtype=torch.float32, device=g_pooled.device)
    _lib.call("spg_segmax_bwd", g_pooled, ldg, argmax, G, C, B, L, offsets, row_seg, M, C, _lib.current_stream())
    return G


def segmax_bn_bwd(g_pooled, ldg, argmax, Y, ldy, scale, shift, mean, var, eps, relu, seg, C):
    _need_cuda(g_pooled, argmax, Y)
    dev = Y.device
    B, L, offsets, row_seg = seg
    M = _seg_rows(seg)
    s12 = torch.empty(2 * C, dtype=torch.float32, device=dev)
    dY = torch.empty((M, C), dtype=torch.float32, device=dev)
    ws = workspace(2 * C * ((B + 255) // 256), dev)
    _lib.call("spg_segmax_bn_bwd", g_pooled, ldg, argmax, Y, ldy, scale, shift, mean, var, float(eps),
              int(bool(relu)), s12, dY, C, ws, B, L, offsets, row_seg, M, C, _lib.current_stream())
    return s12[:C], s12[C:], dY


def row_segs(M):
    return (M, 1, None, None)


def group_norm_fwd(Y, ldy, seg, C, groups, gamma, beta, eps, relu, drop=None, out=None, ldo=None):
    B, L, offsets, _ = seg
    _need_cuda(Y, gamma, beta, offsets)
    M = _seg_rows(seg)
    dev = Y.device
    if out is None:
        out = torch.empty((M, C), dtype=torch.float32, device=dev)
        ldo = C
    mean = torch.empty((B, groups, 2), dtype=torch.float32, device=dev)
    rstd = torch.empty((B, groups), dtype=torch.float32, device=dev)
    _lib.call("spg_group_norm_fwd", Y, ldy, _c(gamma), _c(beta), float(eps), int(bool(relu)), out, ldo, mean, rstd,
              B, L, offsets, C, groups, *_drop(drop), _lib.current_stream())
    return out, mean, rstd


def group_norm_bwd(G, ldg, Y, ldy, mean, rstd, gamma, beta, seg, C, groups, relu, drop=None):
    B, L, offsets, _ = seg
    _need_cuda(G, Y, gamma, beta, offsets)
    M = _seg_rows(seg)
    dev = G.device
    dY = torch.empty((M, C), dtype=torch.float32, device=dev)
    dbg = torch.empty(2 * C, dtype=torch.float32, device=dev)
    ws = workspace(2 * C * int(_lib.lib().spg_group_norm_partials(int(B))), dev)
    _lib.call("spg_group_norm_bwd", G, ldg, Y, ldy, mean, rstd, _c(gamma), _c(beta), int(bool(relu)), dY, C, dbg,
              ws, B, L, offsets, C, groups, *_drop(drop), _lib.current_stream())
    return dY, dbg[C:], dbg[:C]


def stn_apply_bwd(clouds, dXrows, ld):
    _need_cuda(clouds, dXrows)
    clouds = _c(clouds)
    B, F, L = clouds.shape
    dT = torch.empty((B, 4), dtype=torch.float32, device=clouds.device)
    _lib.call("spg_stn_apply_bwd", clouds, dXrows, ld, dT, B, F, L, _lib.current_stream())
    return dT


def rows_scatter(src, idx, n_rows_out):
    _need_cuda(src, idx)
    src = _c(src)
    n, C = src.shape
    dst = torch.empty((n_rows_out, C), dtype=torch.float32, device=src.device)
    zero_(dst)
    _lib.call("spg_rows_scatter", src, idx, dst, n, C, _lib.current_stream())
    return dst


def rows_gather(src, idx):
    _need_cuda(src, idx)
    src = _c(src)
    n = idx.numel()
    C = src.shape[1]
    dst = torch.empty((n, C), dtype=torch.float32, device=src.device)
    _lib.call("spg_rows_gather", src, idx, dst, n, C, _lib.current_stream())
    return dst


def ce_loss(logits, target, class_weight=None, ignore_index=-100, need_grad=True):
    _need_cuda(logits, target, class_weight)
    logits = _c(logits)
    n, C = logits.shape
    loss = torch.empty(1, dtype=torch.float32, device=logits.device)
    d_logits = torch.empty_like(logits) if need_grad else None
    ws = torch.empty(2, dtype=torch.float64, device=logits.device)
    _lib.call("spg_ce_loss", logits, _c(target), class_weight, int(ignore_index), loss, d_logits,
              ws, n, C, _lib.current_stream())
    return loss, d_logits


def clamp_adam_(param, grad, exp_avg, exp_avg_sq, step, lr, beta1=0.9, beta2=0.999, eps=1e-8,
                weight_decay=0.0, grad_clip=0.0, grad_scale=1.0):
    _need_cuda(param, grad, exp_avg, exp_avg_sq)
    _lib.call("spg_clamp_adam", param, grad, exp_avg, exp_avg_sq, param.numel(), float(lr),
              float(beta1), float(beta2), float(eps), float(weight_decay), float(grad_clip),
              float(grad_scale), int(step), _lib.current_stream())


def clamp_adam_dev_(param, grad, exp_avg, exp_avg_sq, step_counter, lr, beta1=0.9, beta2=0.999,
                    eps=1e-8, weight_decay=0.0, grad_clip=0.0, grad_scale=1.0):
    _need_cuda(param, grad, exp_avg, exp_avg_sq, step_counter)
    _lib.call("spg_clamp_adam_dev", param, grad, exp_avg, exp_avg_sq, param.numel(), float(lr),
              float(beta1), float(beta2), float(eps), float(weight_decay), float(grad_clip),
              float(grad_scale), step_counter, _lib.current_stream())


class FusedAllreduce(object):

    def __init__(self, n, device, group):
        import torch.distributed as dist
        import torch.distributed._symmetric_memory as symm_mem
        self.world = dist.get_world_size(group)
        self.rank = dist.get_rank(group)
        self.grad = torch.zeros(n, dtype=torch.float32, device=device)
        self.stage = symm_mem.empty(int(_lib.lib().spg_allreduce_stage_floats(int(n))), dtype=torch.float32,
                                    device=device)
        self.stage.zero_()
        words = int(_lib.lib().spg_allreduce_flag_words(self.world))
        self.flags = symm_mem.empty(words, dtype=torch.int32, device=device)
        self.flags.zero_()
        self._h_stage = symm_mem.rendezvous(self.stage, group)
        self._h_flags = symm_mem.rendezvous(self.flags, group)
        self.stage_ptrs = int(self._h_stage.buffer_ptrs_dev)
        self.flag_ptrs = int(self._h_flags.buffer_ptrs_dev)
        self.state = torch.zeros(2, dtype=torch.int32, device=device)
        torch.cuda.synchronize(device)
        dist.barrier(group=group)

    def step_(self, param, exp_avg, exp_avg_sq, step_counter, lr, beta1=0.9, beta2=0.999, eps=1e-8,
              weight_decay=0.0, grad_clip=0.0):
        _need_cuda(param, exp_avg, exp_avg_sq, step_counter)
        _lib.call("spg_allreduce_clamp_adam", self.grad, self.stage_ptrs, self.flag_ptrs, self.rank, self.world,
                  param, exp_avg, exp_avg_sq, param.numel(), float(lr), float(beta1), float(beta2), float(eps),
                  float(weight_decay), float(grad_clip), 1.0 / self.world, step_counter, self.state,
                  _lib.current_stream())


USE_FUSED_ALLREDUCE = [os.environ.get("SPG_FUSED_ALLREDUCE", "1") != "0"]


def prof_enable(on):
    _lib.lib().spg_prof_enable(int(on))


def prof_reset():
    _lib.lib().spg_prof_reset()


def prof_collect():
    import ctypes

    L = _lib.lib()
    L.spg_prof_collect()
    out = {}
    for k in range(L.spg_prof_num_kernels()):
        n = ctypes.c_int64(0)
        ms = ctypes.c_double(0.0)
        L.spg_prof_kernel_stats(k, ctypes.byref(n), ctypes.byref(ms))
        if n.value:
            out[L.spg_prof_kernel_name(k).decode()] = (int(n.value), float(ms.value))
    return out


def total_launches():
    return int(_lib.lib().spg_prof_total_launches())


class SideStream(object):

    def __init__(self, device):
        self.stream = torch.cuda.Stream(device=device)
        self.keep = []
        self.active = False

    def fork(self, *keep):
        self.stream.wait_stream(torch.cuda.current_stream())
        self.keep.append(keep)
        self.active = True
        return torch.cuda.stream(self.stream)

    def join(self):
        if self.active:
            torch.cuda.current_stream().wait_stream(self.stream)
            self.active = False
        self.keep = []


SIDE = [None]


def cloud_build(points, sp_start, sp_count, sample_idx, columns, n_points, normalize, xform, jitter,
                jitter_sigma, jitter_clip, seed, clouds, diameters):
    _need_cuda(points, sp_start, sp_count, sample_idx, columns, xform, jitter, clouds, diameters)
    assert points.dtype == torch.float32 and points.is_contiguous()
    assert sp_start.dtype == torch.int64 and sp_count.dtype == torch.int32 and columns.dtype == torch.int32
    assert sample_idx is None or (sample_idx.dtype == torch.int32 and sample_idx.is_contiguous())
    assert xform is None or (xform.dtype == torch.float64 and xform.is_contiguous())
    assert jitter is None or (jitter.dtype == torch.float32 and jitter.is_contiguous())
    nv, F, L = clouds.shape
    assert L == n_points and columns.numel() == F
    _lib.call("spg_cloud_build", points, points.shape[1], sp_start, sp_count, sample_idx, columns, F,
              L, int(bool(normalize)), xform, jitter, float(jitter_sigma), float(jitter_clip),
              int(seed), clouds, diameters, nv, _lib.current_stream())
    return clouds, diameters


def confusion_count(logits, label_mode, label_vec, confusion, counters, want_predictions=False):
    _need_cuda(logits, label_mode, label_vec, confusion, counters)
    logits = _c(logits)
    label_mode, label_vec = _c(label_mode), _c(label_vec)
    n, C = logits.shape
    assert logits.dtype == torch.float32 and label_mode.dtype == torch.int64
    assert label_vec.dtype == torch.int64 and label_vec.shape == (n, C)
    assert confusion.dtype == torch.int64 and confusion.shape == (C, C) and confusion.is_contiguous()
    pred = torch.empty(n, dtype=torch.int64, device=logits.device) if want_predictions else None
    _lib.call("spg_confusion_count", logits, C, label_mode, label_vec, C, confusion, counters, pred,
              n, C, _lib.current_stream())
    return pred


def labels_to_points(labels_red, comp_ptr, point_ids, n_ver):
    _need_cuda(labels_red, comp_ptr, point_ids)
    assert labels_red.dtype == torch.int64 and comp_ptr.dtype == torch.int64 and point_ids.dtype == torch.int64
    out = torch.empty(n_ver, dtype=torch.uint8, device=labels_red.device)
    _lib.call("spg_labels_to_points", _c(labels_red), _c(comp_ptr), _c(point_ids), comp_ptr.numel() - 1, out,
              n_ver, _lib.current_stream())
    return out


def nn1_interpolate(xyz_ref, xyz_query, labels_ref=None, want_index=False):
    _need_cuda(xyz_ref, xyz_query, labels_ref)
    assert xyz_ref.dtype == torch.float32 and xyz_query.dtype == torch.float32
    assert xyz_ref.shape[1] == 3 and xyz_query.shape[1] == 3
    xyz_ref, xyz_query = _c(xyz_ref), _c(xyz_query)
    m = xyz_query.shape[0]
    lab = torch.empty(m, dtype=torch.int64, device=xyz_ref.device) if labels_ref is not None else None
    idx = torch.empty(m, dtype=torch.int32, device=xyz_ref.device) if (want_index or labels_ref is None) else None
    _lib.call("spg_nn1_interpolate", xyz_ref, xyz_ref.shape[0], xyz_query, m,
              None if labels_ref is None else _c(labels_ref), lab, idx, _lib.current_stream())
    return lab, idx


def rows_xy_transform(rows, T, row_seg, add_eye=True):
    _need_cuda(rows, T, row_seg)
    assert rows.is_contiguous() and row_seg.dtype == torch.int32
    out = torch.empty_like(rows)
    _lib.call("spg_rows_xy_transform", rows, _c(T), int(bool(add_eye)), row_seg, out, rows.shape[0], rows.shape[1],
              _lib.current_stream())
    return out


def rows_xy_transform_bwd(rows, d_out, offsets):
    _need_cuda(rows, d_out, offsets)
    B = offsets.numel() - 1
    dT = torch.empty((B, 4), dtype=torch.float32, device=rows.device)
    d_out = _c(d_out)
    _lib.call("spg_rows_xy_transform_bwd", rows, rows.shape[1], d_out, d_out.shape[1], offsets, dT, B,
              _lib.current_stream())
    return dT


def pointnet_fused_supported(F, L, widths):
    w = torch.tensor(list(widths), dtype=torch.int32)
    return USE_FUSED_EVAL[0] and bool(_lib.lib().spg_pointnet_fused_supported(int(F), int(L), len(widths), w.data_ptr()))


_FUSED_IMAGES = {}
EVAL_BF16 = [False]


def pointnet_fused_image(layers, F, bf16=False):
    key = []
    for W, b, bn in layers:
        ts = [W, b] + ([bn.running_mean, bn.running_var, bn.weight, bn.bias] if bn is not None else [])
        key += [(x.data_ptr(), x._version) for x in ts if x is not None]
    key = (int(F), bool(bf16)) + tuple(key)
    ent = _FUSED_IMAGES.get(key)
    if ent is not None:
        return ent
    dev = layers[0][0].device
    L = _lib.lib()
    widths = torch.tensor([int(W.shape[0]) for W, _, _ in layers], dtype=torch.int32)
    if bf16:
        rows = int(L.spg_pointnet_fused_bf16_image_rows(int(F), len(layers), widths.data_ptr()))
        image = torch.empty(rows * 64, dtype=torch.bfloat16, device=dev)
        kc = 64
    else:
        rows = int(L.spg_pointnet_fused_image_rows(int(F), len(layers), widths.data_ptr()))
        image = torch.empty(rows * 32, dtype=torch.float32, device=dev)
        kc = 32
    bias = torch.empty(int(widths.sum()), dtype=torch.float32, device=dev)
    row, boff, K = 0, 0, kc
    for W, b, bn in layers:
        N, kv = int(W.shape[0]), int(W.shape[1])
        scale = shift = None
        if bn is not None:
            scale, shift = bn_fold(bn.running_mean, bn.running_var, bn.weight, bn.bias, bn.eps)
        if bf16:
            _lib.call("spg_tc_pack_weights_bf16", W, W.stride(0), scale, N, K, kv, image[row * 64:],
                      _lib.current_stream())
            row += (K // 64) * N
        else:
            _lib.call("spg_tc_pack_weights_scaled", W, W.stride(0), scale, N, K, kv, image[row * 32:],
                      _lib.current_stream())
            row += (K // 32) * 2 * N
        bsl = bias[boff:boff + N]
        if b is not None:
            affine_act(b.detach().reshape(1, N), N, 1, N, scale, shift, False, out=bsl, ldo=N)
        elif shift is not None:
            bsl.copy_(shift)
        else:
            zero_(bsl)
        boff += N
        K = max(N, kc) if bf16 else N
    if len(_FUSED_IMAGES) > 64:
        _FUSED_IMAGES.clear()
    _FUSED_IMAGES[key] = (image, bias, widths)
    return image, bias, widths


def pointnet_fused_eval(clouds, T, image, bias, widths, pooled, ldp):
    _need_cuda(clouds, image, bias, pooled, T)
    B, F, L = clouds.shape
    name = "spg_pointnet_fused_eval_bf16" if image.dtype == torch.bfloat16 else "spg_pointnet_fused_eval"
    _lib.call(name, clouds, B, F, L, None if T is None else _c(T), 1, image, bias,
              int(widths.numel()), widths.data_ptr(), pooled, ldp, _lib.current_stream())
    k = int(F)
    for n in widths.tolist():
        FUSED_FLOPS[0] += 2 * B * L * k * int(n)
        k = int(n)
    return pooled


FUSED_FLOPS = [0]


LP_DIST = {"euclidian": 0, "intrinsic": 1, "scalar": 2}
LP_INTRA = {"tv": 0, "laplacian": 1, "TVH": 2}
LP_INTER = {None: -1, "zhang": 0, "TVminus": 1}


def _lp_sort_ws(n, dev):
    nbytes = torch.zeros(1, dtype=torch.int64)
    _lib.call("spg_lp_sort_workspace", int(n), nbytes)
    ws = torch.empty(int(nbytes[0]), dtype=torch.uint8, device=dev)
    return ws, ws.numel()


def lp_incidence(src, tgt, n_ver):
    _need_cuda(src, tgt)
    dev, E = src.device, src.numel()
    i32 = dict(dtype=torch.int32, device=dev)
    rowptr, entry = torch.empty(n_ver + 1, **i32), torch.empty(2 * E, **i32)
    k0, k1, v0 = torch.empty(2 * E, **i32), torch.empty(2 * E, **i32), torch.empty(2 * E, **i32)
    ws, nb = _lp_sort_ws(2 * E, dev)
    _lib.call("spg_lp_incidence", src, tgt, n_ver, E, rowptr, entry, k0, k1, v0, ws, nb, _lib.current_stream())
    return rowptr, entry


def lp_dist_fwd(emb, src, tgt, dist_type):
    _need_cuda(emb, src, tgt)
    assert emb.dtype == torch.float32 and emb.dim() == 2 and emb.is_contiguous()
    assert src.dtype == torch.int64 and tgt.dtype == torch.int64
    E, dev = src.numel(), emb.device
    dt = LP_DIST[dist_type]
    diff = torch.empty(E, dtype=torch.float32, device=dev)
    coef = None if dt == 0 else torch.empty(E, dtype=torch.float32, device=dev)
    _lib.call("spg_lp_dist_fwd", emb, emb.shape[0], emb.shape[1], src, tgt, E, dt, diff, coef, _lib.current_stream())
    return diff, coef


def lp_dist_bwd(emb, src, tgt, dist_type, coef, gdiff, incidence):
    _need_cuda(emb, src, tgt, coef, gdiff)
    rowptr, entry = incidence
    gemb = torch.empty_like(emb)
    _lib.call("spg_lp_dist_bwd", emb, emb.shape[0], emb.shape[1], src, tgt, src.numel(), LP_DIST[dist_type], coef,
              _c(gdiff), rowptr, entry, gemb, _lib.current_stream())
    return gemb


def lp_loss_fwd(diff, weights, is_transition, intra, inter, dist_type):
    _need_cuda(diff, weights, is_transition)
    assert diff.dtype == torch.float32 and weights.dtype == torch.float32 and is_transition.dtype == torch.uint8
    dev = diff.device
    part = torch.empty(2 * int(_lib.lib().spg_lp_loss_partials()), dtype=torch.float64, device=dev)
    loss = torch.empty(2, dtype=torch.float32, device=dev)
    _lib.call("spg_lp_loss_fwd", _c(diff), _c(weights), _c(is_transition), diff.numel(), LP_INTRA[intra],
              LP_INTER[inter], LP_DIST[dist_type], part, loss, _lib.current_stream())
    return loss


def lp_loss_bwd(diff, weights, is_transition, intra, inter, dist_type, gloss):
    _need_cuda(diff, weights, is_transition, gloss)
    gdiff = torch.empty_like(diff)
    _lib.call("spg_lp_loss_bwd", _c(diff), _c(weights), _c(is_transition), diff.numel(), LP_INTRA[intra],
              LP_INTER[inter], LP_DIST[dist_type], _c(gloss), gdiff, _lib.current_stream())
    return gdiff


def lp_xpart(src, tgt, is_transition, pred_in_component, n_ver, transition_factor):
    _need_cuda(src, tgt, is_transition, pred_in_component)
    dev, E = src.device, src.numel()
    i32 = dict(dtype=torch.int32, device=dev)
    w = torch.empty(E, dtype=torch.float32, device=dev)
    inx, size, ncomp = torch.empty(n_ver, **i32), torch.empty(n_ver, **i32), torch.empty(1, **i32)
    par, root, rank = torch.empty(n_ver, **i32), torch.empty(n_ver, **i32), torch.empty(n_ver, **i32)
    k0 = torch.empty(E, dtype=torch.int64, device=dev)
    k1 = torch.empty(E, dtype=torch.int64, device=dev)
    v0, v1 = torch.empty(E, **i32), torch.empty(E, **i32)
    ws, nb = _lp_sort_ws(max(n_ver, E), dev)
    _lib.call("spg_lp_xpart", src, tgt, is_transition, pred_in_component, n_ver, E, float(transition_factor), w, inx,
              size, ncomp, par, root, rank, k0, k1, v0, v1, ws, nb, _lib.current_stream())
    return w, inx, size, ncomp


def lp_seal(src, tgt, is_transition, pred_in_component, objects, n_comp, transition_factor):
    _need_cuda(src, tgt, is_transition, pred_in_component, objects)
    dev, E, V = src.device, src.numel(), pred_in_component.numel()
    i32 = dict(dtype=torch.int32, device=dev)
    w, wc = torch.empty(E, dtype=torch.float32, device=dev), torch.empty(n_comp, **i32)
    st, mt = torch.empty(n_comp, **i32), torch.empty(n_comp, **i32)
    k0, k1 = torch.empty(V, dtype=torch.int64, device=dev), torch.empty(V, dtype=torch.int64, device=dev)
    ws, nb = _lp_sort_ws(V, dev)
    _lib.call("spg_lp_seal", src, tgt, is_transition, pred_in_component, objects, V, E, n_comp,
              float(transition_factor), w, wc, st, mt, k0, k1, ws, nb, _lib.current_stream())
    return w, wc


def lp_fill_weights(is_transition, w_other, w_transition):
    _need_cuda(is_transition)
    w = torch.empty(is_transition.numel(), dtype=torch.float32, device=is_transition.device)
    _lib.call("spg_lp_fill_weights", is_transition, is_transition.numel(), float(w_other), float(w_transition), w,
              _lib.current_stream())
    return w


def lp_count(truth, pred=None):
    _need_cuda(truth, pred)
    counts = torch.empty(2, dtype=torch.int64, device=truth.device)
    _lib.call("spg_lp_count", _c(truth), None if pred is None else _c(pred), truth.numel(), counts,
              _lib.current_stream())
    return counts


def lp_edge_weight(diff, threshold):
    _need_cuda(diff)
    out = torch.empty(diff.numel(), dtype=torch.float64, device=diff.device)
    _lib.call("spg_lp_edge_weight", _c(diff), diff.numel(), float(threshold), out, _lib.current_stream())
    return out


def lp_relax(relaxed, src, tgt, n_ver, tolerance):
    _need_cuda(relaxed, src, tgt)
    assert relaxed.dtype == torch.uint8 and relaxed.is_contiguous()
    dev = relaxed.device
    mark = torch.empty(max(n_ver, 1), dtype=torch.uint8, device=dev)
    hit, status = torch.empty(1, dtype=torch.int32, device=dev), torch.empty(1, dtype=torch.int32, device=dev)
    _lib.call("spg_lp_relax", relaxed, src, tgt, n_ver, relaxed.numel(), int(tolerance), mark, hit, status,
              _lib.current_stream())
    return status


def lp_perfect_prediction(comp_ptr, point_ids, labels, n_ver):
    _need_cuda(comp_ptr, point_ids, labels)
    assert labels.dtype == torch.int64 and labels.dim() == 2
    labels = _c(labels)
    pred = torch.empty(n_ver, dtype=torch.int64, device=labels.device)
    _lib.call("spg_lp_perfect_prediction", comp_ptr, point_ids, comp_ptr.numel() - 1, labels, labels.shape[1],
              labels.shape[1] - 1, n_ver, pred, _lib.current_stream())
    return pred


LPL_GLOBAL_E, LPL_GLOBAL_RGB, LPL_GLOBAL_XYN, LPL_GLOBAL_XY = 1, 2, 4, 8


def lp_augment(xyz, rgb, rot, ref_index, noise_xyz, noise_rgb, device_noise, rgb_jitter, sigma, clip, seed,
               file_pos, xyz_out, rgb_out):
    _need_cuda(xyz, rgb, rot, noise_xyz, noise_rgb, xyz_out, rgb_out)
    assert xyz.dtype == torch.float32 and rgb.dtype == torch.float32 and xyz.is_contiguous() and rgb.is_contiguous()
    assert rot is None or (rot.dtype == torch.float32 and rot.numel() == 9 and rot.is_contiguous())
    _lib.call("spg_lp_augment", xyz, rgb, xyz.shape[0], rot, int(ref_index), noise_xyz, noise_rgb,
              int(bool(device_noise)), int(bool(rgb_jitter)), float(sigma), float(clip), int(seed), int(file_pos),
              xyz_out, rgb_out, _lib.current_stream())


def lp_subgraph_select(mask, objects, src, tgt, new_index, selected, edge_pos, object_max):
    _need_cuda(mask, objects, src, tgt, new_index, selected, edge_pos, object_max)
    n, E = objects.numel(), src.numel()
    ws, nb = None, 0
    if mask is not None:
        nbytes = torch.zeros(1, dtype=torch.int64)
        _lib.call("spg_lp_subgraph_workspace", n, E, nbytes)
        ws = torch.empty(int(nbytes[0]), dtype=torch.uint8, device=objects.device)
        nb = ws.numel()
    _lib.call("spg_lp_subgraph_select", mask, objects, n, src, tgt, E, new_index, selected, edge_pos, object_max, ws,
              nb, _lib.current_stream())


def lp_subgraph_edges(src, tgt, is_transition, new_index, edge_pos, vertex_offset, src_out, tgt_out, tr_out):
    _need_cuda(src, tgt, is_transition, new_index, edge_pos, src_out, tgt_out, tr_out)
    _lib.call("spg_lp_subgraph_edges", src, tgt, is_transition, src.numel(), new_index, edge_pos, int(vertex_offset),
              src_out, tgt_out, tr_out, _lib.current_stream())


def lp_object_offsets(object_max, counts, offsets):
    _need_cuda(object_max, counts, offsets)
    assert counts.dtype == torch.int64 and offsets.dtype == torch.int64
    _lib.call("spg_lp_object_offsets", object_max, counts, counts.numel(), offsets, _lib.current_stream())


def lp_local_clouds(xyz, rgb, rgb_scale, local_geometry, k, selected, n_sel, elevation, xyn, labels, objects,
                    object_offset, use_rgb, global_flags, clouds, clouds_global, xyz_out, labels_out, objects_out):
    _need_cuda(xyz, rgb, local_geometry, selected, elevation, xyn, labels, objects, object_offset, clouds,
               clouds_global, xyz_out, labels_out, objects_out)
    assert local_geometry.dtype == torch.int32 and local_geometry.is_contiguous()
    assert clouds.dtype == torch.float32 and clouds.is_contiguous() and clouds_global.is_contiguous()
    _lib.call("spg_lp_local_clouds", xyz, rgb, int(bool(rgb_scale)), local_geometry, local_geometry.shape[1], int(k),
              selected, int(n_sel), elevation, xyn, labels, labels.shape[1], objects, object_offset,
              int(bool(use_rgb)), int(global_flags), clouds, clouds_global, clouds_global.shape[1], xyz_out,
              labels_out, objects_out, _lib.current_stream())


def knn_max_k():
    return int(_lib.lib().spg_knn_max_k())


def knn_bounds(xyz):
    _need_cuda(xyz)
    assert xyz.dtype == torch.float32 and xyz.is_contiguous()
    words = torch.empty(8, dtype=torch.int32, device=xyz.device)
    _lib.call("spg_knn_bounds", xyz, xyz.shape[0], words, _lib.current_stream())
    return words


def knn_workspace(n, device):
    nbytes = torch.zeros(1, dtype=torch.int64)
    _lib.call("spg_knn_workspace", int(n), nbytes)
    return torch.empty(int(nbytes[0]), dtype=torch.uint8, device=device)


def knn_grid(xyz, grid, ws):
    _need_cuda(xyz, ws)
    n_cells = torch.empty(1, dtype=torch.int32, device=xyz.device)
    ox, oy, oz, cell, dx, dy, dz = grid
    _lib.call("spg_knn_grid", xyz, xyz.shape[0], float(ox), float(oy), float(oz), float(cell), int(dx), int(dy),
              int(dz), ws, ws.numel(), n_cells, _lib.current_stream())
    return n_cells


def knn_query(n, k, k1, grid, ws, want_target2):
    _need_cuda(ws)
    dev = ws.device
    source = torch.empty(n * k1, dtype=torch.int64, device=dev)
    target = torch.empty(n * k1, dtype=torch.int64, device=dev)
    distances = torch.empty(n * k1, dtype=torch.float32, device=dev)
    target2 = torch.empty(n * k, dtype=torch.int64, device=dev) if want_target2 else None
    ox, oy, oz, cell, dx, dy, dz = grid
    _lib.call("spg_knn_query", int(n), int(k), int(k1), float(ox), float(oy), float(oz), float(cell), int(dx),
              int(dy), int(dz), ws, ws.numel(), source, target, distances, target2, _lib.current_stream())
    return source, target, distances, target2


def geof(xyz, target, k):
    _need_cuda(xyz, target)
    assert xyz.dtype == torch.float32 and xyz.is_contiguous()
    assert target.dtype == torch.int64 and target.is_contiguous()
    n = xyz.shape[0]
    out = torch.empty((n, 4), dtype=torch.float32, device=xyz.device)
    status = torch.empty(1, dtype=torch.int32, device=xyz.device)
    _lib.call("spg_geof", xyz, n, target, int(k), out, status, _lib.current_stream())
    return out, status
```

Baseline: 50.59 million.

## Fuse segment-max pooling backward into TC GEMM prologue and weight-grad kernel

Adds a pool-backward prologue to the tensor-core GEMM and the dW kernel, so the dense dY after max-pooling is rebuilt on the fly from the pooled gradient, argmax and BN stats instead of being written out by segmax_bn_bwd. segmax_bn_bwd gains a sums-only mode that skips the dY write. The segmax stats reduction loop is also unrolled with batched loads. The fused path is gated by SPG_FUSED_POOLBWD, which defaults to off, so only the unrolled reduction and the apply-loop unroll change run by default.

```diff
diff --git a/include/spg_b200.h b/include/spg_b200.h
--- a/include/spg_b200.h
+++ b/include/spg_b200.h
@@ -151,6 +151,15 @@
                    const float* e_y, int64_t e_ldy, const float* e_scale, const float* e_shift,
                    const float* e_mean, const float* e_var, float e_eps, int e_relu, float* e_s12,
                    spg_stream_t stream);
+int spg_tc_gemm_poolbwd_supported(int64_t M, int N, int K);
+int spg_tc_gemm_poolbwd(const float* Y, int64_t ldy, const float* weight_image, const float* bias, float* C,
+                        int64_t ldc, int64_t M, int N, int K, const float* g_pooled, int64_t ldg,
+                        const int32_t* argmax, int L, const float* scale, const float* shift, int relu,
+                        const float* mean, const float* var, const float* s12, float eps, float* dy_out,
+                        int64_t lddy, int epilogue, float* partials_ws,
+                        const float* e_y, int64_t e_ldy, const float* e_scale, const float* e_shift,
+                        const float* e_mean, const float* e_var, float e_eps, int e_relu, float* e_s12,
+                        spg_stream_t stream);
 
 int spg_tc_dw_supported(int64_t M, int co, int ci);
 int spg_tc_dw_ctas(int64_t M);
@@ -159,6 +168,12 @@
               spg_stream_t stream);
 int spg_splitk_reduce(const float* partials, int split, int64_t M, int64_t N, const float* bias,
                       float* C, int64_t ldc, spg_stream_t stream);
+int spg_tc_dw_pool_supported(int64_t M, int co, int ci);
+int spg_tc_dw_pool(const float* Y, int64_t ldy, const float* g_pooled, int64_t ldg, const int32_t* argmax, int L,
+                   const float* y_scale, const float* y_shift, int y_relu, const float* y_mean,
+                   const float* y_var, const float* y_s12, float y_eps, const float* P, int64_t ldp,
+                   const float* p_scale, const float* p_shift, int p_relu, float* dW, float* workspace,
+                   int64_t M, int co, int ci, spg_stream_t stream);
 
 int64_t spg_colstats_chunks(int64_t M);
 int spg_bn_fold(const float* mean, const float* var, const float* gamma, const float* beta,
diff --git a/superpoint_graph_b200/csrc/common.cuh b/superpoint_graph_b200/csrc/common.cuh
--- a/superpoint_graph_b200/csrc/common.cuh
+++ b/superpoint_graph_b200/csrc/common.cuh
@@ -118,6 +118,12 @@
     return sc * (g - m1 - (y - mu) * rstd * m2);
 }
 
+__device__ __forceinline__ float pool_bn_bwd(float g, float y, float sc, float sh, float mu, float rstd, float m1,
+                                             float m2, bool relu) {
+    if (relu) g = relu_bwd(g, y, sc, sh);
+    return __fmul_rn(sc, fmaf(-__fmul_rn(__fsub_rn(y, mu), rstd), m2, __fsub_rn(g, m1)));
+}
+
 struct FoldArgs {
     const float *gamma, *beta;
     float *scale, *shift, *rmean, *rvar;
diff --git a/superpoint_graph_b200/csrc/pointnet.cu b/superpoint_graph_b200/csrc/pointnet.cu
--- a/superpoint_graph_b200/csrc/pointnet.cu
+++ b/superpoint_graph_b200/csrc/pointnet.cu
@@ -210,14 +210,31 @@
     if (c < C) {
         const float sc = scale[c], sh = shift[c], mu = mean[c];
         const float rstd = 1.f / sqrtf(var[c] + eps);
-        for (int64_t b = b0 + y; b < b1; b += 8) {
-            const int l = argmax[b * C + c];
-            if (Segs::kMayBeEmpty && l < 0) continue;
-            const float yv = __ldg(Y + (segs.begin(b) + l) * ldy + c);
-            float g = __ldg(gp + b * ldg + c);
-            if (relu) g = relu_bwd(g, yv, sc, sh);
-            a1 += g;
-            a2 = fmaf(g, (yv - mu) * rstd, a2);
+        constexpr int U = Segs::kMayBeEmpty ? 4 : 8;
+        for (int64_t bg = b0 + y; bg < b1; bg += 8 * U) {
+            int l[U];
+            bool ok[U];
+            float yv[U], g[U];
+#pragma unroll
+            for (int u = 0; u < U; ++u) {
+                const int64_t b = bg + 8 * u;
+                l[u] = b < b1 ? argmax[b * C + c] : -1;
+                ok[u] = b < b1 && (!Segs::kMayBeEmpty || l[u] >= 0);
+            }
+#pragma unroll
+            for (int u = 0; u < U; ++u) {
+                const int64_t b = bg + 8 * u;
+                yv[u] = ok[u] ? __ldg(Y + (segs.begin(b) + l[u]) * ldy + c) : 0.f;
+                g[u] = ok[u] ? __ldg(gp + b * ldg + c) : 0.f;
+            }
+#pragma unroll
+            for (int u = 0; u < U; ++u) {
+                if (!ok[u]) continue;
+                float gu = g[u];
+                if (relu) gu = relu_bwd(gu, yv[u], sc, sh);
+                a1 += gu;
+                a2 = fmaf(gu, (yv[u] - mu) * rstd, a2);
+            }
         }
     }
     s1[y][x] = a1;
@@ -256,7 +273,7 @@
         m1[j] = s1[c + j] / (float)M;
         m2[j] = s2[c + j] / (float)M;
     }
-#pragma unroll 2
+#pragma unroll(Segs::kMayBeEmpty ? 2 : 4)
     for (int64_t r = (int64_t)blockIdx.y * 8 + y; r < M; r += (int64_t)gridDim.y * 8) {
         const int64_t b = segs.seg_of(r);
         const int l = (int)(r - segs.begin(b));
@@ -268,11 +285,8 @@
         const int aq[4] = {am.x, am.y, am.z, am.w};
         float d[4];
 #pragma unroll
-        for (int j = 0; j < 4; ++j) {
-            float g = (aq[j] == l) ? gv[j] : 0.f;
-            if (relu) g = relu_bwd(g, yv[j], sc[j], sh[j]);
-            d[j] = bn_bwd(g, yv[j], sc[j], mu[j], rs[j], m1[j], m2[j]);
-        }
+        for (int j = 0; j < 4; ++j)
+            d[j] = pool_bn_bwd((aq[j] == l) ? gv[j] : 0.f, yv[j], sc[j], sh[j], mu[j], rs[j], m1[j], m2[j], relu);
         *reinterpret_cast<float4*>(dY + r * lddy + c) = make_float4(d[0], d[1], d[2], d[3]);
     }
 }
@@ -440,7 +454,7 @@
                       float* workspace, int64_t B, int L, const int64_t* offsets, const int32_t* row_seg,
                       int64_t rows, int C, spg_stream_t stream) {
     if (B <= 0 || rows <= 0 || C <= 0 || !g_pooled || !argmax || !Y || !scale || !shift || !mean || !var ||
-        !s12 || !dY || !workspace)
+        !s12 || !workspace)
         return SPG_E_BADARG;
     if (offsets ? !row_seg : (L <= 0 || rows != B * L)) return SPG_E_BADARG;
     if ((C & 3) || (ldy & 3) || (lddy & 3)) return SPG_E_UNSUPPORTED;
@@ -455,7 +469,7 @@
         int rc = launch_status();
         if (rc) return rc;
         rc = colsum_merge(K_SEGMAX_BWD, workspace, chunks, 2 * C, s12, s);
-        if (rc) return rc;
+        if (rc || !dY) return rc;
         int64_t gy = ceil_div64(rows, 32);
         if (gy > 16 * kNumSMs) gy = 16 * kNumSMs;
         dim3 g2((unsigned)ceil_div64(C, 128), (unsigned)gy);
diff --git a/superpoint_graph_b200/csrc/tc_dw.cu b/superpoint_graph_b200/csrc/tc_dw.cu
--- a/superpoint_graph_b200/csrc/tc_dw.cu
+++ b/superpoint_graph_b200/csrc/tc_dw.cu
@@ -12,7 +12,7 @@
 constexpr int DW_KSTEPS = DW_PTS / 8;
 constexpr int DW_STAGES = 4;
 constexpr int DW_SMEM_LIMIT = 232448;
-constexpr int DW_STATIC_SMEM = 2048;
+constexpr int DW_STATIC_SMEM = 8192;
 
 template <int CO, int CI>
 struct DwCfg {
@@ -43,9 +43,16 @@
     float* partial;
     int64_t M;
     int64_t pts_per_cta;
+    const float* gp;
+    int64_t ldg;
+    const int* argmax;
+    int pool_L;
+    const float *y_scale, *y_shift, *y_mean, *y_var, *y_s12;
+    float y_eps;
+    int y_relu;
 };
 
-template <int CO, int CI>
+template <int CO, int CI, bool POOL>
 __global__ void __launch_bounds__(DW_THREADS, 1) tc_dw_kernel(const DwArgs p) {
     using Cfg = DwCfg<CO, CI>;
     constexpr int WM = Cfg::WM, WN = Cfg::WN, MSUB = Cfg::MSUB;
@@ -57,7 +64,9 @@
     uint8_t* smem = reinterpret_cast<uint8_t*>((reinterpret_cast<uintptr_t>(smem_raw) + 1023) & ~(uintptr_t)1023);
     __shared__ __align__(8) uint64_t bars[2 * DW_STAGES];
     __shared__ __align__(16) float sc_s[128], sh_s[128];
-    static_assert(sizeof(bars) + sizeof(sc_s) + sizeof(sh_s) <= DW_STATIC_SMEM, "static shared memory");
+    __shared__ __align__(16) float pc_s[POOL ? 6 * CO : 4];
+    static_assert(sizeof(bars) + sizeof(sc_s) + sizeof(sh_s) + sizeof(pc_s) <= DW_STATIC_SMEM,
+                  "static shared memory");
 
     const int t = threadIdx.x;
     const int warp = t >> 5, lane = t & 31;
@@ -119,6 +128,16 @@
         sc_s[t] = p.p_scale ? p.p_scale[t] : 1.f;
         sh_s[t] = p.p_shift ? p.p_shift[t] : 0.f;
     }
+    if constexpr (POOL) {
+        for (int i = t; i < CO; i += DW_THREADS) {
+            pc_s[i] = p.y_scale[i];
+            pc_s[CO + i] = p.y_shift[i];
+            pc_s[2 * CO + i] = p.y_mean[i];
+            pc_s[3 * CO + i] = 1.f / sqrtf(p.y_var[i] + p.y_eps);
+            pc_s[4 * CO + i] = p.y_s12[i] / (float)p.M;
+            pc_s[5 * CO + i] = p.y_s12[CO + i] / (float)p.M;
+        }
+    }
     __syncthreads();
 
     if (warp >= DW_CONS_WARPS) {
@@ -192,6 +211,35 @@
         for (int m = 0; m < MSUB; ++m) wg_reg_fence(acc[m]);
         const int col_g = CO >= 128 ? 0 : g * WN;
         const uint32_t smem_u = smem_u32(smem);
+        auto pool_a = [&](int kstep, float (&v)[MSUB][4]) {
+#pragma unroll
+            for (int h = 0; h < 2; ++h) {
+                const int64_t i = m_beg + (int64_t)kstep * 8 + (lane & 3) + 4 * h;
+                if (i >= m_end) continue;
+                const uint32_t b = (uint32_t)i / (uint32_t)p.pool_L;
+                const int l = (int)((uint32_t)i - b * (uint32_t)p.pool_L);
+                const int* am = p.argmax + (int64_t)b * CO + a_co;
+                const float* gr = p.gp + (int64_t)b * p.ldg + a_co;
+                int a[2 * MSUB];
+                if constexpr (MSUB == 1) {
+                    const int2 q = __ldg(reinterpret_cast<const int2*>(am));
+                    a[0] = q.x; a[1] = q.y;
+                } else {
+                    const int4 q = __ldg(reinterpret_cast<const int4*>(am));
+                    a[0] = q.x; a[1] = q.y; a[2] = q.z; a[3] = q.w;
+                }
+#pragma unroll
+                for (int m = 0; m < MSUB; ++m)
+#pragma unroll
+                    for (int k = 0; k < 2; ++k) {
+                        const int c = a_co + 2 * m + k;
+                        const float gv = a[2 * m + k] == l ? __ldg(gr + 2 * m + k) : 0.f;
+                        v[m][2 * h + k] = pool_bn_bwd(gv, v[m][2 * h + k], pc_s[c], pc_s[CO + c], pc_s[2 * CO + c],
+                                                      pc_s[3 * CO + c], pc_s[4 * CO + c], pc_s[5 * CO + c],
+                                                      p.y_relu);
+                    }
+            }
+        };
 
         int s = 0, s_prev = 0;
         uint32_t phase = 0;
@@ -212,6 +260,7 @@
                     __syncwarp();
                     if (lane == 0) mbar_arrive(bar_empty(s_prev));
                 }
+                if constexpr (POOL) pool_a(ch * DW_KSTEPS + kb, a_raw[r]);
 #pragma unroll
                 for (int m = 0; m < MSUB; ++m)
 #pragma unroll
@@ -274,12 +323,13 @@
     }
 }
 
-template <int CO, int CI>
+template <int CO, int CI, bool POOL = false>
 static int launch_dw(const DwArgs& a, int ctas, cudaStream_t s) {
     constexpr int smem = DwCfg<CO, CI>::SMEM;
-    cudaError_t e = cudaFuncSetAttribute(tc_dw_kernel<CO, CI>, cudaFuncAttributeMaxDynamicSharedMemorySize, smem);
+    cudaError_t e =
+        cudaFuncSetAttribute(tc_dw_kernel<CO, CI, POOL>, cudaFuncAttributeMaxDynamicSharedMemorySize, smem);
     if (e != cudaSuccess) return (int)e;
-    SPG_LAUNCH(K_TC_DW, s, (tc_dw_kernel<CO, CI>), (unsigned)ctas, DW_THREADS, smem, a);
+    SPG_LAUNCH(K_TC_DW, s, (tc_dw_kernel<CO, CI, POOL>), (unsigned)ctas, DW_THREADS, smem, a);
     return launch_status();
 }
 
@@ -313,6 +363,7 @@
     DwArgs a;
     a.dY = dY; a.lddy = lddy; a.P = P; a.ldp = ldp; a.p_scale = p_scale; a.p_shift = p_shift;
     a.p_relu = p_relu; a.partial = workspace; a.M = M;
+    a.gp = nullptr; a.argmax = nullptr;
     cudaStream_t s = (cudaStream_t)stream;
     a.pts_per_cta = ceil_div64(ceil_div64(M, ctas), DW_PTS) * DW_PTS;
     int rc;
@@ -326,4 +377,35 @@
     return spg_splitk_reduce(workspace, ctas, co, ci, nullptr, dW, ci, stream);
 }
 
-}
+int spg_tc_dw_pool_supported(int64_t M, int co, int ci) {
+    return (M >= DW_PTS && M < 2147483648ll && ((co == 256 && ci == 128) || (co == 128 && ci == 64))) ? 1 : 0;
+}
+
+int spg_tc_dw_pool(const float* Y, int64_t ldy, const float* g_pooled, int64_t ldg, const int32_t* argmax, int L,
+                   const float* y_scale, const float* y_shift, int y_relu, const float* y_mean,
+                   const float* y_var, const float* y_s12, float y_eps, const float* P, int64_t ldp,
+                   const float* p_scale, const float* p_shift, int p_relu, float* dW, float* workspace,
+                   int64_t M, int co, int ci, spg_stream_t stream) {
+    if (!Y || !g_pooled || !argmax || !y_scale || !y_shift || !y_mean || !y_var || !y_s12 || !P || !dW ||
+        !workspace || M <= 0 || L <= 0 || M % L != 0 || ldg < co)
+        return SPG_E_BADARG;
+    if (!spg_tc_dw_pool_supported(M, co, ci)) return SPG_E_UNSUPPORTED;
+    if ((ldy & 3) || (ldp & 3) || ldy < co || ldp < ci) return SPG_E_ALIGN;
+    if (((uintptr_t)Y | (uintptr_t)P | (uintptr_t)argmax | (uintptr_t)workspace | (uintptr_t)p_scale |
+         (uintptr_t)p_shift) & 15)
+        return SPG_E_ALIGN;
+    const int ctas = spg_tc_dw_ctas(M);
+    DwArgs a;
+    a.dY = Y; a.lddy = ldy; a.P = P; a.ldp = ldp; a.p_scale = p_scale; a.p_shift = p_shift;
+    a.p_relu = p_relu; a.partial = workspace; a.M = M;
+    a.gp = g_pooled; a.ldg = ldg; a.argmax = argmax; a.pool_L = L;
+    a.y_scale = y_scale; a.y_shift = y_shift; a.y_mean = y_mean; a.y_var = y_var; a.y_s12 = y_s12;
+    a.y_eps = y_eps; a.y_relu = y_relu;
+    a.pts_per_cta = ceil_div64(ceil_div64(M, ctas), DW_PTS) * DW_PTS;
+    cudaStream_t s = (cudaStream_t)stream;
+    const int rc = co == 256 ? launch_dw<256, 128, true>(a, ctas, s) : launch_dw<128, 64, true>(a, ctas, s);
+    if (rc) return rc;
+    return spg_splitk_reduce(workspace, ctas, co, ci, nullptr, dW, ci, stream);
+}
+
+}
diff --git a/superpoint_graph_b200/csrc/tc_gemm2.cu b/superpoint_graph_b200/csrc/tc_gemm2.cu
--- a/superpoint_graph_b200/csrc/tc_gemm2.cu
+++ b/superpoint_graph_b200/csrc/tc_gemm2.cu
@@ -18,7 +18,7 @@
 constexpr int T2_HALF_A_BYTES = T2_A_BYTES / 2;
 constexpr int T2_HALF_STAGE_BYTES = 2 * T2_HALF_A_BYTES;
 
-enum { PRO_AFFINE = 0, PRO_BNBWD = 1 };
+enum { PRO_AFFINE = 0, PRO_BNBWD = 1, PRO_POOLBWD = 2 };
 enum { EPI_NONE = 0, EPI_STATS = 1, EPI_BNRED = 2 };
 
 struct Tc2Args {
@@ -35,6 +35,10 @@
     int a_relu;
     const float *a_mean, *a_var, *a_s12;
     float a_eps;
+    const float* gp;
+    int64_t ldg;
+    const int* argmax;
+    int pool_L;
     float* dy_out;
     int64_t lddy;
     int epi;
@@ -135,7 +139,7 @@
         for (int blk = 0; blk < nk * 2; ++blk)
             tma_load_2d(wres_u + (uint32_t)blk * (NS * T2_KC * 4), &wmap, 0, blk * p.N + n0, bar_w);
     }
-    constexpr int PF = PRO == PRO_BNBWD ? 2 : 4;
+    constexpr int PF = PRO == PRO_BNBWD ? 2 : PRO == PRO_POOLBWD ? 3 : 4;
     constexpr int NOPS = PRO == PRO_BNBWD ? 2 : 1;
     float4 q[PF][NOPS][4];
     const int pt = t - T2_EPI_WARPS * 32;
@@ -173,7 +177,9 @@
     float* sh_s = sc_s + p.K;
     float* cy_s = sh_s + p.K;
     float* c0_s = cy_s + p.K;
-    float* bias_s = c0_s + p.K;
+    float* m1_s = c0_s + p.K;
+    float* m2_s = m1_s + p.K;
+    float* bias_s = c0_s + (PRO == PRO_POOLBWD ? 3 : 1) * p.K;
     float* ev_s = bias_s + NS;
     float* acc_s = ev_s + 4 * NS;
     for (int i = t; i < p.K; i += T2_THREADS) {
@@ -185,6 +191,11 @@
             const float m1 = p.a_s12[i] / (float)p.M, m2 = p.a_s12[p.K + i] / (float)p.M;
             cy_s[i] = -sc * rstd * m2;
             c0_s[i] = sc * (rstd * m2 * mu - m1);
+        } else if (PRO == PRO_POOLBWD) {
+            cy_s[i] = p.a_mean[i];
+            c0_s[i] = 1.f / sqrtf(p.a_var[i] + p.a_eps);
+            m1_s[i] = p.a_s12[i] / (float)p.M;
+            m2_s[i] = p.a_s12[p.K + i] / (float)p.M;
         }
     }
     for (int i = t; i < NS; i += T2_THREADS) {
@@ -200,7 +211,7 @@
     __syncthreads();
 
     if (warp >= T2_EPI_WARPS) {
-        const bool pro = PRO == PRO_BNBWD || p.a_scale || p.a_shift || p.a_relu;
+        const bool pro = PRO != PRO_AFFINE || p.a_scale || p.a_shift || p.a_relu;
         int64_t tile = blockIdx.x;
         int kc = 0;
         uint32_t it = 0;
@@ -209,7 +220,7 @@
 #pragma unroll
         for (int j = 0; j < 4; ++j) soff[j] = sw128_off((pq >> 3) + 16 * j, c16);
         const uint32_t ring_u = ring(ph);
-        const bool side_store = PRO == PRO_BNBWD && p.dy_out != nullptr && blockIdx.y == 0;
+        const bool side_store = PRO != PRO_AFFINE && p.dy_out != nullptr && blockIdx.y == 0;
         auto st_shared4 = [](uint32_t addr, uint4 v) {
             asm volatile("st.shared.v4.b32 [%0], {%1, %2, %3, %4};" ::"r"(addr), "r"(v.x), "r"(v.y),
                          "r"(v.z), "r"(v.w)
@@ -248,6 +259,21 @@
                         v.y = fmaf(sc.y, v.y, fmaf(cy.y, y.y, c0.y));
                         v.z = fmaf(sc.z, v.z, fmaf(cy.z, y.z, c0.z));
                         v.w = fmaf(sc.w, v.w, fmaf(cy.w, y.w, c0.w));
+                        st_global4(p.dy_out + row * p.lddy + col, v, side_store);
+                    } else if (PRO == PRO_POOLBWD) {
+                        const float4 mu = *reinterpret_cast<const float4*>(cy_s + col);
+                        const float4 rs = *reinterpret_cast<const float4*>(c0_s + col);
+                        const float4 m1 = *reinterpret_cast<const float4*>(m1_s + col);
+                        const float4 m2 = *reinterpret_cast<const float4*>(m2_s + col);
+                        const uint32_t b = (uint32_t)row / (uint32_t)p.pool_L;
+                        const int l = (int)((uint32_t)row - b * (uint32_t)p.pool_L);
+                        const int4 am = __ldg(reinterpret_cast<const int4*>(p.argmax + (int64_t)b * p.K + col));
+                        const float* gr = p.gp + (int64_t)b * p.ldg + col;
+                        const bool rl = p.a_relu;
+                        v.x = pool_bn_bwd(am.x == l ? __ldg(gr) : 0.f, v.x, sc.x, sh.x, mu.x, rs.x, m1.x, m2.x, rl);
+                        v.y = pool_bn_bwd(am.y == l ? __ldg(gr + 1) : 0.f, v.y, sc.y, sh.y, mu.y, rs.y, m1.y, m2.y, rl);
+                        v.z = pool_bn_bwd(am.z == l ? __ldg(gr + 2) : 0.f, v.z, sc.z, sh.z, mu.z, rs.z, m1.z, m2.z, rl);
+                        v.w = pool_bn_bwd(am.w == l ? __ldg(gr + 3) : 0.f, v.w, sc.w, sh.w, mu.w, rs.w, m1.w, m2.w, rl);
                         st_global4(p.dy_out + row * p.lddy + col, v, side_store);
                     } else {
                         v.x = fmaf(v.x, sc.x, sh.x);
@@ -538,12 +564,13 @@
     return r == CUDA_SUCCESS ? SPG_OK : SPG_E_BADARG;
 }
 
-static inline int fixed_smem(int NS, int K) {
-    return (K / T2_KC) * 2 * NS * T2_KC * 4 + (4 * K + NS + 4 * NS + T2_EPI_WARPS * NS * 4) * 4;
-}
-
-static inline int stages_for(int NS, int K) {
-    int nst = (232448 - 1024 - fixed_smem(NS, K)) / T2_STAGE_BYTES;
+static inline int fixed_smem(int NS, int K, int pro = PRO_AFFINE) {
+    const int kvec = pro == PRO_POOLBWD ? 6 : 4;
+    return (K / T2_KC) * 2 * NS * T2_KC * 4 + (kvec * K + NS + 4 * NS + T2_EPI_WARPS * NS * 4) * 4;
+}
+
+static inline int stages_for(int NS, int K, int pro = PRO_AFFINE) {
+    int nst = (232448 - 1024 - fixed_smem(NS, K, pro)) / T2_STAGE_BYTES;
     return nst > T2_MAX_STAGES ? T2_MAX_STAGES : nst;
 }
 
@@ -554,13 +581,13 @@
     int64_t gx = kNumSMs / slices;
     if (gx > tiles) gx = tiles;
     if (gx < 1) gx = 1;
-    const int nst = stages_for(NS, a.K);
+    const int nst = stages_for(NS, a.K, PRO);
     if (nst < 2) return SPG_E_UNSUPPORTED;
     a.nstages = nst;
     CUtensorMap map;
     int rc = make_weight_map(&map, image, a.N, a.K, NS);
     if (rc) return rc;
-    const int smem = nst * T2_STAGE_BYTES + fixed_smem(NS, a.K);
+    const int smem = nst * T2_STAGE_BYTES + fixed_smem(NS, a.K, PRO);
     cudaError_t e = cudaFuncSetAttribute(tc_gemm2_kernel<NS, PRO>, cudaFuncAttributeMaxDynamicSharedMemorySize, smem);
     if (e != cudaSuccess) return (int)e;
     dim3 grid((unsigned)gx, (unsigned)slices);
@@ -571,11 +598,38 @@
     return launch_status();
 }
 
-static inline int pick_ns(int N, int K) {
-    if (N % 128 == 0 && stages_for(128, K) >= 2) return 128;
-    if (N % 64 == 0 && stages_for(64, K) >= 2) return 64;
-    if (N % 32 == 0 && N <= 64 && stages_for(32, K) >= 2) return 32;
+static inline int pick_ns(int N, int K, int pro = PRO_AFFINE) {
+    if (N % 128 == 0 && stages_for(128, K, pro) >= 2) return 128;
+    if (N % 64 == 0 && stages_for(64, K, pro) >= 2) return 64;
+    if (N % 32 == 0 && N <= 64 && stages_for(32, K, pro) >= 2) return 32;
     return 0;
+}
+
+static int launch_pro(Tc2Args& a, const float* image, int pro, cudaStream_t s) {
+    const int ns = pick_ns(a.N, a.K, pro);
+#define SPG_TC2_CASE(NS_)                                                                               \
+    if (ns == NS_)                                                                                      \
+        return pro == PRO_POOLBWD ? launch_tc2<NS_, PRO_POOLBWD>(a, image, s)                           \
+                                  : pro == PRO_BNBWD ? launch_tc2<NS_, PRO_BNBWD>(a, image, s)          \
+                                                     : launch_tc2<NS_, PRO_AFFINE>(a, image, s);
+    SPG_TC2_CASE(128)
+    SPG_TC2_CASE(64)
+    SPG_TC2_CASE(32)
+#undef SPG_TC2_CASE
+    return SPG_E_UNSUPPORTED;
+}
+
+static int check_epilogue(const Tc2Args& a, int N) {
+    if (a.epi == EPI_STATS) {
+        if (!a.part || !a.mean_out || !a.var_out) return SPG_E_BADARG;
+        if (a.fold.enabled && !a.fold.shift) return SPG_E_BADARG;
+    } else if (a.epi == EPI_BNRED) {
+        if (!a.part || !a.e_y || !a.e_mean || !a.e_var || !a.e_s12 || (a.e_ldy & 3) || a.e_ldy < N)
+            return SPG_E_BADARG;
+    } else if (a.epi != EPI_NONE) {
+        return SPG_E_BADARG;
+    }
+    return SPG_OK;
 }
 
 }
@@ -621,28 +675,53 @@
                        momentum, M);
     a.e_y = e_y; a.e_ldy = e_ldy; a.e_scale = e_scale; a.e_shift = e_shift; a.e_mean = e_mean;
     a.e_var = e_var; a.e_eps = e_eps; a.e_relu = e_relu; a.e_s12 = e_s12; a.nstages = 0;
+    a.gp = nullptr; a.ldg = 0; a.argmax = nullptr; a.pool_L = 0;
     const bool bnbwd = a2 != nullptr;
     if (bnbwd && (!a_scale || !a_shift || !a_mean || !a_var || !a_s12 || (lda2 & 3) || lda2 < K))
         return SPG_E_BADARG;
     if (dy_out && (!bnbwd || (lddy & 3) || lddy < K)) return SPG_E_BADARG;
-    if (epilogue == EPI_STATS) {
-        if (!partials_ws || !mean_out || !var_out) return SPG_E_BADARG;
-        if (a.fold.enabled && !shift_out) return SPG_E_BADARG;
-    } else if (epilogue == EPI_BNRED) {
-        if (!partials_ws || !e_y || !e_mean || !e_var || !e_s12 || (e_ldy & 3) || e_ldy < N) return SPG_E_BADARG;
-    } else if (epilogue != EPI_NONE) {
+    const int rc = check_epilogue(a, N);
+    if (rc) return rc;
+    return launch_pro(a, weight_image, bnbwd ? PRO_BNBWD : PRO_AFFINE, (cudaStream_t)stream);
+}
+
+int spg_tc_gemm_poolbwd_supported(int64_t M, int N, int K) {
+    return (spg_tc_gemm_supported(M, N, K) && M < 2147483648ll && pick_ns(N, K, PRO_POOLBWD) != 0) ? 1 : 0;
+}
+
+int spg_tc_gemm_poolbwd(const float* Y, int64_t ldy, const float* weight_image, const float* bias, float* C,
+                        int64_t ldc, int64_t M, int N, int K, const float* g_pooled, int64_t ldg,
+                        const int32_t* argmax, int L, const float* scale, const float* shift, int relu,
+                        const float* mean, const float* var, const float* s12, float eps, float* dy_out,
+                        int64_t lddy, int epilogue, float* partials_ws,
+                        const float* e_y, int64_t e_ldy, const float* e_scale, const float* e_shift,
+                        const float* e_mean, const float* e_var, float e_eps, int e_relu, float* e_s12,
+                        spg_stream_t stream) {
+    if (M < 0 || !Y || !weight_image || !C || !g_pooled || !argmax || !scale || !shift || !mean || !var || !s12)
         return SPG_E_BADARG;
-    }
-    cudaStream_t s = (cudaStream_t)stream;
-    const int ns = pick_ns(N, K);
-#define SPG_TC2_CASE(NS_)                                                                  \
-    if (ns == NS_) return bnbwd ? launch_tc2<NS_, PRO_BNBWD>(a, weight_image, s)          \
-                                : launch_tc2<NS_, PRO_AFFINE>(a, weight_image, s);
-    SPG_TC2_CASE(128)
-    SPG_TC2_CASE(64)
-    SPG_TC2_CASE(32)
-#undef SPG_TC2_CASE
-    return SPG_E_UNSUPPORTED;
+    if (L <= 0 || M % L != 0 || ldg < K) return SPG_E_BADARG;
+    if (M == 0) return SPG_OK;
+    if (!spg_tc_gemm_poolbwd_supported(M, N, K)) return SPG_E_UNSUPPORTED;
+    if ((ldy & 3) || (ldc & 3) || ldy < K || ldc < N) return SPG_E_ALIGN;
+    if (dy_out && ((lddy & 3) || lddy < K)) return SPG_E_ALIGN;
+    if (((uintptr_t)Y | (uintptr_t)C | (uintptr_t)weight_image | (uintptr_t)argmax | (uintptr_t)dy_out |
+         (uintptr_t)e_y) & 15)
+        return SPG_E_ALIGN;
+    if (epilogue == EPI_STATS) return SPG_E_BADARG;
+    Tc2Args a;
+    a.A = Y; a.lda = ldy; a.A2 = nullptr; a.lda2 = 0; a.bias = bias; a.C = C; a.ldc = ldc; a.M = M;
+    a.N = N; a.K = K; a.a_scale = scale; a.a_shift = shift; a.a_relu = relu;
+    a.a_mean = mean; a.a_var = var; a.a_s12 = s12; a.a_eps = eps;
+    a.gp = g_pooled; a.ldg = ldg; a.argmax = argmax; a.pool_L = L;
+    a.dy_out = dy_out; a.lddy = lddy;
+    a.epi = epilogue; a.part = partials_ws;
+    a.mean_out = a.var_out = nullptr;
+    a.fold = fold_args(nullptr, nullptr, 0.f, nullptr, nullptr, nullptr, nullptr, nullptr, 0.f, M);
+    a.e_y = e_y; a.e_ldy = e_ldy; a.e_scale = e_scale; a.e_shift = e_shift; a.e_mean = e_mean;
+    a.e_var = e_var; a.e_eps = e_eps; a.e_relu = e_relu; a.e_s12 = e_s12; a.nstages = 0;
+    const int rc = check_epilogue(a, N);
+    if (rc) return rc;
+    return launch_pro(a, weight_image, PRO_POOLBWD, (cudaStream_t)stream);
 }
 
 int spg_tc_gemm(const float* A, int64_t lda, const float* weight_image, const float* bias, float* C,
diff --git a/superpoint_graph_b200/dense.py b/superpoint_graph_b200/dense.py
--- a/superpoint_graph_b200/dense.py
+++ b/superpoint_graph_b200/dense.py
@@ -197,11 +197,22 @@
             gp, ldgp, argmax, seg = pooled
             G, ldg, own_g = ops.segmax_bwd(gp, ldgp, argmax, seg, C), C, True
         lazy = None
+        pool_lazy = None
         dY, ldy = None, C
         if fused_pool:
             gp, ldgp, argmax, seg = pooled
-            s1, s2, dY = ops.segmax_bn_bwd(gp, ldgp, argmax, nxt.raw, nxt.ld, nxt.scale, nxt.shift,
-                                           mean, var, sp.bn.eps, nxt.relu, seg, C)
+            kpad = _padded_k(sp.cin, cur.ld)
+            if (ops.USE_FUSED_POOLBWD[0] and seg[2] is None and want_dx and nxt.ld % 4 == 0
+                    and nxt.scale is not None and nxt.shift is not None
+                    and ops.tc_poolbwd_supported(M, sp.cin, C, nxt.ld, sp.cin)
+                    and ops.tc_dw_pool_supported(M, C, kpad, nxt.ld, cur.ld) and (kpad == sp.cin or not cur.pending)):
+                s12 = ops.segmax_bn_sums(gp, ldgp, argmax, nxt.raw, nxt.ld, nxt.scale, nxt.shift, mean, var,
+                                         sp.bn.eps, nxt.relu, seg, C)
+                s1, s2 = s12[:C], s12[C:]
+                pool_lazy = (gp, ldgp, argmax, seg[1], nxt.scale, nxt.shift, nxt.relu, mean, var, s12, sp.bn.eps)
+            else:
+                s1, s2, dY = ops.segmax_bn_bwd(gp, ldgp, argmax, nxt.raw, nxt.ld, nxt.scale, nxt.shift,
+                                               mean, var, sp.bn.eps, nxt.relu, seg, C)
             if sp.gamma is not None:
                 grads[sp.gamma] = s2
                 grads[sp.beta] = s1
@@ -233,9 +244,13 @@
             dY, ldy = G, ldg
         red = None
 
-        def weight_grads(dY, ldy, cur=cur, nxt=nxt, mean=mean, sp=sp, Wp=Wp, C=C):
+        def weight_grads(dY, ldy, cur=cur, nxt=nxt, mean=mean, sp=sp, Wp=Wp, C=C, pool_lazy=pool_lazy):
             kpad = _padded_k(sp.cin, cur.ld)
-            if ops.tc_dw_supported(M, sp.cout, kpad, ldy, cur.ld) and (kpad == sp.cin or not cur.pending):
+            if pool_lazy is not None:
+                dW = ops.tc_dw(nxt.raw, nxt.ld, cur.raw, cur.ld, M, sp.cout, kpad, p_aff=cur.aff(), pool=pool_lazy)
+                if kpad != sp.cin:
+                    dW = dW[:, :sp.cin].contiguous()
+            elif ops.tc_dw_supported(M, sp.cout, kpad, ldy, cur.ld) and (kpad == sp.cin or not cur.pending):
                 dW = ops.tc_dw(dY, ldy, cur.raw, cur.ld, M, sp.cout, kpad, p_aff=cur.aff())
                 if kpad != sp.cin:
                     dW = dW[:, :sp.cin].contiguous()
@@ -244,7 +259,7 @@
             db = None
             if sp.b is not None:
                 if sp.bn is not None and nxt.scale is not None and mean is not None:
-                    db = _zeros(C, dY.device)
+                    db = _zeros(C, Wp.device)
                 else:
                     db = ops.colsum(dY, ldy, M, C)
             return dW.view(Wp.shape), db
@@ -256,11 +271,11 @@
                 if sp.b is not None:
                     grads[sp.b] = db
             else:
-                with side.fork(dY, saved[li]):
+                with side.fork(dY, saved[li], pool_lazy):
                     dW, db = weight_grads(dY, ldy)
                     _accumulate_grad(Wp, dW)
                     if sp.b is not None:
-                        if db is _ZEROS.get((C, dY.device.index)):
+                        if db is _ZEROS.get((C, Wp.device.index)):
                             db = db.clone()
                         _accumulate_grad(params[sp.b], db)
 
@@ -268,14 +283,18 @@
             run_weight_grads(dY, ldy)
         Gn = None
         if want_dx:
-            if lazy is not None or ops.tc_supported(M, sp.cin, sp.cout, ldy, sp.cin):
+            if lazy is not None or pool_lazy is not None or ops.tc_supported(M, sp.cin, sp.cout, ldy, sp.cin):
                 bnred = None
                 if (ops.USE_FUSED_BNBWD[0] and li > 0 and specs[li - 1].bn is not None
                         and saved[li - 1][2] is not None and saved[li - 1][1].drop is None and cur.ld % 4 == 0):
                     bnred = (cur.raw, cur.ld, cur.scale, cur.shift, saved[li - 1][2], saved[li - 1][3],
                              specs[li - 1].bn.eps, cur.relu)
-                res = ops.tc_gemm(G if lazy is not None else dY, ldg if lazy is not None else ldy,
-                                  _w2d(Wp), sp.cin, True, M, sp.cin, sp.cout, bnbwd=lazy, bnred=bnred)
+                if pool_lazy is not None:
+                    res = ops.tc_gemm(nxt.raw, nxt.ld, _w2d(Wp), sp.cin, True, M, sp.cin, sp.cout,
+                                      bnred=bnred, poolbwd=pool_lazy + (False,))
+                else:
+                    res = ops.tc_gemm(G if lazy is not None else dY, ldg if lazy is not None else ldy,
+                                      _w2d(Wp), sp.cin, True, M, sp.cin, sp.cout, bnbwd=lazy, bnred=bnred)
                 res = list(res) if isinstance(res, tuple) else [res]
                 Gn = res.pop(0)
                 if lazy is not None:
diff --git a/superpoint_graph_b200/ops.py b/superpoint_graph_b200/ops.py
--- a/superpoint_graph_b200/ops.py
+++ b/superpoint_graph_b200/ops.py
@@ -390,6 +390,7 @@
 USE_TC = [os.environ.get("SPG_TC", "1") != "0"]
 USE_FUSED_RNN = [os.environ.get("SPG_FUSED_RNN", "1") != "0"]
 USE_FUSED_BNBWD = [os.environ.get("SPG_FUSED_BNBWD", "1") != "0"]
+USE_FUSED_POOLBWD = [os.environ.get("SPG_FUSED_POOLBWD", "0") == "1"]
 USE_FUSED_EVAL = [os.environ.get("SPG_FUSED_EVAL", "1") != "0"]
 def set_pdl(mode):
     if "SPG_PDL" not in os.environ:
@@ -441,8 +442,12 @@
     return img
 
 
+def tc_poolbwd_supported(M, N, K, ldy, ldc):
+    return tc_supported(M, N, K, ldy, ldc) and bool(_lib.lib().spg_tc_gemm_poolbwd_supported(int(M), int(N), int(K)))
+
+
 def tc_gemm(A, lda, W, ldw, transpose, M, N, K, bias=None, a_aff=None, stats=False, k_valid=None,
-            fold=None, bnbwd=None, bnred=None):
+            fold=None, bnbwd=None, bnred=None, poolbwd=None):
     _need_cuda(A, W)
     dev = A.device
     kv = int(K if k_valid is None else k_valid)
@@ -478,11 +483,21 @@
         ws = workspace(MAX_TC_PARTIALS[0] * N * 3, dev, slot=1)
     GEMM_FLOPS[0] += 2 * M * N * K
     TC_FLOPS[0] += 2 * M * N * K
-    _lib.call("spg_tc_gemm_ex", A, lda, img, bias, out, N, M, N, K, a_s, a_t, int(bool(a_r)),
-              a2, lda2, a_mean, a_var, a_s12, float(a_eps), dy, lddy, epi, ws,
-              mean, var, gamma, beta, float(eps), scale, shift, rm, rv, nbt, float(mom),
-              e[0], e[1], e[2], e[3], e[4], e[5], float(e[6]), int(bool(e[7])), s12,
-              _lib.current_stream())
+    if poolbwd is not None:
+        assert not stats and bnbwd is None and a_aff is None
+        gp, ldg, argmax, L, p_s, p_t, p_r, p_mean, p_var, p_s12, p_eps, want_dy = poolbwd
+        if want_dy:
+            dy = torch.empty((M, K), dtype=torch.float32, device=dev)
+            lddy = K
+        _lib.call("spg_tc_gemm_poolbwd", A, lda, img, bias, out, N, M, N, K, gp, ldg, argmax, int(L),
+                  p_s, p_t, int(bool(p_r)), p_mean, p_var, p_s12, float(p_eps), dy, lddy, epi, ws,
+                  e[0], e[1], e[2], e[3], e[4], e[5], float(e[6]), int(bool(e[7])), s12, _lib.current_stream())
+    else:
+        _lib.call("spg_tc_gemm_ex", A, lda, img, bias, out, N, M, N, K, a_s, a_t, int(bool(a_r)),
+                  a2, lda2, a_mean, a_var, a_s12, float(a_eps), dy, lddy, epi, ws,
+                  mean, var, gamma, beta, float(eps), scale, shift, rm, rv, nbt, float(mom),
+                  e[0], e[1], e[2], e[3], e[4], e[5], float(e[6]), int(bool(e[7])), s12,
+                  _lib.current_stream())
     res = [out]
     if stats:
         res += [mean, var] + ([scale, shift] if fold is not None else [])
@@ -493,6 +508,7 @@
     return res[0] if len(res) == 1 else tuple(res)
 
 
+
 MAX_TC_PARTIALS = [132]
 
 TC_FLOPS = [0]
@@ -504,7 +520,12 @@
             and bool(_lib.lib().spg_tc_dw_supported(int(M), int(co), int(ci))))
 
 
-def tc_dw(dY, lddy, P, ldp, M, co, ci, p_aff=None):
+def tc_dw_pool_supported(M, co, ci, ldy, ldp):
+    return (tc_dw_supported(M, co, ci, ldy, ldp)
+            and bool(_lib.lib().spg_tc_dw_pool_supported(int(M), int(co), int(ci))))
+
+
+def tc_dw(dY, lddy, P, ldp, M, co, ci, p_aff=None, pool=None):
     _need_cuda(dY, P)
     dev = dY.device
     ctas = int(_lib.lib().spg_tc_dw_ctas(int(M)))
@@ -513,8 +534,13 @@
     p_s, p_t, p_r = p_aff if p_aff is not None else (None, None, False)
     GEMM_FLOPS[0] += 2 * M * co * ci
     DW_FLOPS[0] += 2 * M * co * ci
-    _lib.call("spg_tc_dw", dY, lddy, P, ldp, p_s, p_t, int(bool(p_r)), out, ws, M, co, ci,
-              _lib.current_stream())
+    if pool is not None:
+        gp, ldg, argmax, L, y_s, y_t, y_r, y_mean, y_var, y_s12, y_eps = pool
+        _lib.call("spg_tc_dw_pool", dY, lddy, gp, ldg, argmax, int(L), y_s, y_t, int(bool(y_r)), y_mean, y_var,
+                  y_s12, float(y_eps), P, ldp, p_s, p_t, int(bool(p_r)), out, ws, M, co, ci, _lib.current_stream())
+    else:
+        _lib.call("spg_tc_dw", dY, lddy, P, ldp, p_s, p_t, int(bool(p_r)), out, ws, M, co, ci,
+                  _lib.current_stream())
     return out
 
 
@@ -679,16 +705,25 @@
 
 
 def segmax_bn_bwd(g_pooled, ldg, argmax, Y, ldy, scale, shift, mean, var, eps, relu, seg, C):
+    s12, dY = _segmax_bn_bwd(g_pooled, ldg, argmax, Y, ldy, scale, shift, mean, var, eps, relu, seg, C, True)
+    return s12[:C], s12[C:], dY
+
+
+def segmax_bn_sums(g_pooled, ldg, argmax, Y, ldy, scale, shift, mean, var, eps, relu, seg, C):
+    return _segmax_bn_bwd(g_pooled, ldg, argmax, Y, ldy, scale, shift, mean, var, eps, relu, seg, C, False)[0]
+
+
+def _segmax_bn_bwd(g_pooled, ldg, argmax, Y, ldy, scale, shift, mean, var, eps, relu, seg, C, want_dy):
     _need_cuda(g_pooled, argmax, Y)
     dev = Y.device
     B, L, offsets, row_seg = seg
     M = _seg_rows(seg)
     s12 = torch.empty(2 * C, dtype=torch.float32, device=dev)
-    dY = torch.empty((M, C), dtype=torch.float32, device=dev)
+    dY = torch.empty((M, C), dtype=torch.float32, device=dev) if want_dy else None
     ws = workspace(2 * C * ((B + 255) // 256), dev)
     _lib.call("spg_segmax_bn_bwd", g_pooled, ldg, argmax, Y, ldy, scale, shift, mean, var, float(eps),
               int(bool(relu)), s12, dY, C, ws, B, L, offsets, row_seg, M, C, _lib.current_stream())
-    return s12[:C], s12[C:], dY
+    return s12, dY
 
 
 def row_segs(M):
```

New measurement: 50.06 million (median of 6 runs). 0.989x the previous value.
